# lnkloveating/MediQuery-RAG

Measured on AMD Instinct MI355X. Metric: queries/s (embed+top-k, k=5, b=256) over 1M×768 corpus; p50 single-query ms, higher is better.
Workload: dtype f32 (exact 3-way bf16 split, fp32 accumulate; exact fp32 top-k)

## Files before the change

### include/mq.h

```cpp
#ifndef MQ_H
#define MQ_H

#include <stdint.h>

#ifdef __cplusplus
extern "C" {
#endif

#define MQ_OK 0
#define MQ_EINVAL -1
#define MQ_ENOMEM -2
#define MQ_EHIP -3
#define MQ_EIO -4
#define MQ_ESTATE -5

#define MQ_DTYPE_F32 0
#define MQ_DTYPE_BF16 1
#define MQ_DTYPE_F32X6 2
#define MQ_DTYPE_F32_SCREEN 3

#define MQ_GELU_ERF 0
#define MQ_GELU_TANH 1
#define MQ_POOL_CLS 0
#define MQ_POOL_MEAN 1

#define MQ_MAX_K 64

typedef struct mq_index mq_index;
typedef struct mq_encoder mq_encoder;

const char* mq_last_error(void);
const char* mq_version(void);
const char* mq_build_source_hash(void);
int mq_device_count(void);

int mq_index_create(int device, int dim, int64_t capacity, int dtype, mq_index** out);
int mq_index_destroy(mq_index* ix);
int mq_index_size(const mq_index* ix, int64_t* n_rows);
int mq_index_dim(const mq_index* ix, int* dim);
int mq_index_add(mq_index* ix, const float* rows, int64_t n, int rows_on_device, void* stream);
int mq_index_reset(mq_index* ix);
int mq_index_search(mq_index* ix, const float* queries, int64_t nq, int k,
                    float* out_scores, int64_t* out_ids, int io_on_device, void* stream);
int mq_index_select(mq_index* src, const int64_t* rows, int64_t n, mq_index* dst);
int mq_index_get(mq_index* ix, int64_t row0, int64_t n, float* out, int out_on_device, void* stream);
int mq_index_set_precision(mq_index* ix, int dtype);
int mq_index_set_stream_threshold(mq_index* ix, int max_queries);
int mq_index_set_threshold_scan(mq_index* ix, int enabled);
int mq_index_set_int8_screen(mq_index* ix, int enabled);
int mq_index_set_async_screen(mq_index* ix, int enabled);
int mq_index_rescans(const mq_index* ix, int64_t* rescans, int64_t* remerges);
int mq_index_screen_fallbacks(const mq_index* ix, int64_t* to_direct, int64_t* to_split);
int mq_index_screen_skips(const mq_index* ix, int64_t* bf16_skips, int64_t* int8_skips);
int mq_index_data(mq_index* ix, void** device_rows);
int mq_index_set_timing(mq_index* ix, int enabled);
int mq_index_read_timing(mq_index* ix, float* ms, int n);
#define MQ_MASK_SET 0
#define MQ_MASK_AND 1
#define MQ_MASK_OR 2
#define MQ_MASK_CLEAR 3
int mq_mask_eval(const int32_t* codes, int64_t n, const uint8_t* lut, int n_lut, uint32_t* bits, int mode,
                 void* stream);
int mq_mask_eval_bits(const int32_t* codes, int64_t n, const uint64_t* lut_words, int n_lut, uint32_t* bits,
                      int mode, void* stream);
int mq_mask_combine(uint32_t* dst, const uint32_t* src, int64_t n_words, int mode, void* stream);
int mq_index_search_masked(mq_index* ix, const float* query, int k, const uint32_t* bits, float* out_scores,
                           int64_t* out_ids, int io_on_device, void* stream);
int mq_index_search_masked_batch(mq_index* ix, const float* queries, int64_t nq, int k, const uint32_t* bits,
                                 float* out_scores, int64_t* out_ids, int io_on_device, void* stream);
int mq_index_masked_gathers(const mq_index* ix, int64_t* count);
#define MQ_CONTAINS_MAX_BYTES 256
#define MQ_CONTAINS_SPAN_BYTES 16384
int mq_mask_contains(const uint8_t* text, int64_t text_bytes, const int64_t* offsets, int64_t n,
                     const uint8_t* pattern, int pattern_len, int negate, uint32_t* bits, int mode,
                     uint32_t* scratch, void* stream);

#define MQ_LEX_MAX_TERMS 128
#define MQ_LEX_NORM(fmul, fadd, c0, c1, dl) fadd((c0), fmul((c1), (dl)))
#define MQ_LEX_TERM(fmul, fadd, fdiv, w, tf, norm) fdiv(fmul((w), (tf)), fadd((tf), (norm)))
int64_t mq_lex_scratch_bytes(int64_t n, int k);
int mq_lex_df(const uint16_t* tokens, int64_t n_tokens, const int64_t* offsets, int64_t n, int ngram,
              const uint32_t* keys, int n_terms, int64_t* df, void* scratch, void* stream);
int mq_lex_topk(const uint16_t* tokens, int64_t n_tokens, const int64_t* offsets, int64_t n, int ngram,
                const uint32_t* keys, const float* w, int n_terms, float c0, float c1,
                const uint32_t* bits, int k, float* out_scores, int64_t* out_ids, int io_on_device,
                void* scratch, void* stream);

#define MQ_MMR_SCORE(fmul, fsub, lambda, s, red) \
  fsub(fmul((lambda), (s)), fmul(fsub(1.0f, (lambda)), (red)))
int mq_index_mmr_select(mq_index* ix, const float* cand_scores, const int64_t* cand_ids, int64_t nq,
                        int fetch_k, int k, float lambda, float* out_scores, int64_t* out_ids,
                        int io_on_device, void* stream);
int mq_index_search_mmr(mq_index* ix, const float* queries, int64_t nq, int k, int fetch_k,
                        float lambda, const uint32_t* bits, float* out_scores, int64_t* out_ids,
                        int io_on_device, void* stream);

int mq_index_save(mq_index* ix, const char* path);
int mq_index_load(mq_index* ix, const char* path);
int mq_index_save_rows(mq_index* ix, const char* path, int64_t row0, int64_t n);
int mq_index_load_append(mq_index* ix, const char* path);

int mq_topk_merge_host(const float* scores, const int64_t* ids, int n_lists, int64_t nq,
                       int k_in, int k_out, float* out_scores, int64_t* out_ids);
int mq_topk_merge_device(const float* scores, const int64_t* ids, int n_lists, int64_t nq,
                         int k_in, int k_out, float* out_scores, int64_t* out_ids, void* stream);

typedef struct mq_bert_config {
  int vocab_size;
  int hidden;
  int layers;
  int heads;
  int ffn;
  int max_positions;
  int type_vocab;
  float ln_eps;
  int gelu;
  int pooling;
} mq_bert_config;

int mq_encoder_create(int device, const mq_bert_config* cfg, mq_encoder** out);
int mq_encoder_destroy(mq_encoder* enc);
int64_t mq_encoder_weight_count(const mq_bert_config* cfg);
int mq_encoder_load_weights(mq_encoder* enc, const float* blob, int64_t n_floats);
int mq_encoder_set_precision(mq_encoder* enc, int dtype);
#define MQ_ENC_STAGES 8
int mq_encoder_set_graphs(mq_encoder* enc, int enabled);
#define MQ_ENC_OPT_ROWS_MAX 0
#define MQ_ENC_OPT_ROWS_SPLITS 1
#define MQ_ENC_OPT_SPLITK_MAX 2
#define MQ_ENC_OPT_FUSE_ATTN_OPROJ 4
#define MQ_ENC_OPT_SPLITK_TILES 6
#define MQ_ENC_OPT_RESIDENT_LAYERS 8
#define MQ_ENC_OPT_X6_PRESPLIT 9
#define MQ_ENC_OPT_ROWS_PLANES 10
#define MQ_ENC_OPT_LN_FOLD 11
#define MQ_ENC_OPT_CLS_KFREE 12
#define MQ_ENC_OPT_QKV_ATTN 13
#define MQ_ENC_OPT_EPI_SPLIT 14
int mq_encoder_set_option(mq_encoder* enc, int option, int value);
int mq_encoder_get_option(const mq_encoder* enc, int option, int* value);
int mq_encoder_set_timing(mq_encoder* enc, int enabled);
int mq_encoder_read_timing(mq_encoder* enc, float* ms, int n);
int mq_encoder_embed(mq_encoder* enc, const int32_t* ids, const int32_t* mask, int B, int L,
                     float* out, int io_on_device, void* stream);

#define MQ_HEAD_MAX_LABELS 8
int mq_encoder_load_head(mq_encoder* enc, const float* pooler_w, const float* pooler_b, const float* cls_w,
                         const float* cls_b, int n_labels);
int mq_encoder_score(mq_encoder* enc, const int32_t* ids, const int32_t* types, const int32_t* mask, int B,
                     int L, float* logits, int io_on_device, void* stream);

typedef struct mq_tokenizer mq_tokenizer;
int mq_tokenizer_create_wordpiece(const char* vocab_path, int lower_case, int max_length,
                                  mq_tokenizer** out);
int mq_tokenizer_create_wordpiece_tokens(const char* const* tokens, int n_tokens, int lower_case,
                                         int max_length, mq_tokenizer** out);
int mq_tokenizer_create_char(int vocab_size, int max_length, mq_tokenizer** out);
int mq_tokenizer_destroy(mq_tokenizer* tok);
int mq_tokenizer_encode_batch(mq_tokenizer* tok, const char* const* texts, int n, int pad_to,
                              int32_t* ids, int32_t* mask, int* out_len);

int mq_tokenizer_encode_pairs(mq_tokenizer* tok, const char* const* first, const char* const* second, int n,
                              int pad_to, int32_t* ids, int32_t* types, int32_t* mask, int* out_len);

int mq_debug_gemm_f32(const float* A, const float* W, const float* bias, const float* resid,
                      float* out, int M, int N, int K, int epi, int tile, void* stream);
int64_t mq_debug_w3_bytes(int N, int K);
int mq_debug_split_w3(const float* W, int N, int K, void* w3, void* stream);
int mq_debug_gemm_x6p(const float* A, const void* W3, const float* bias, const float* resid,
                      float* out, int M, int N, int K, int epi, int tile, void* stream);
int mq_debug_gemm_x6p_ln(const float* A, const void* W3, const float* bias, const float* resid,
                         float* out, int M, int N, int K, int epi, int tile, const float* stats_in,
                         float* stats_out, const float* g, const float* b, const float* s_fold,
                         float eps, void* stream);
int mq_debug_ln_fold_weight(const float* W, const float* bias, const float* g, const float* b, int N,
                            int K, float* Wg, float* s_out, float* c_out, void* stream);
int mq_debug_gemm_x6p_attn(const float* A, const void* W3, const float* bias, const int* mask,
                           float* ctx, int M, int K, int heads, float scale, int epi,
                           const float* stats_in, const float* s_fold, float eps, int max_workgroups,
                           void* stream);
int mq_debug_attention(const float* qkv, const int* mask, int B, int L, int H, int heads, float scale,
                       int variant, float* ctx, void* stream);
int mq_debug_cls_attention(const float* q, const float* x, const float* stats, const float* ln_g,
                           const float* ln_b, float eps, const int* mask, int B, int L, int H, int heads,
                           float scale, const float* Wk, const float* Wv, const float* bv, float* ctx,
                           void* stream);
int mq_debug_attn_oproj(const float* qkv, const int* mask, int B, int L, int H, int heads, float scale,
                        const float* Wo, const float* bo, const float* resid, int cls_only, int hg, int qf,
                        int acc, float* out, void* stream);
enum { MQ_ROWS_QKV = 0, MQ_ROWS_UP = 1, MQ_ROWS_OPROJ = 2, MQ_ROWS_DOWN = 3 };
int mq_debug_rows_gemm(int kind, int variant, const float* A, int lda, int64_t a_plane, int s_in, const float* W,
                       const float* bias, const float* resid, int ldr, float* out, int64_t o_plane, int M, int N,
                       int K, int splits, const float* ln_g, const float* ln_b, float eps, float* ln_out,
                       const int* ids, const int* types, int L, int vocab, const float* pos, const float* typ,
                       int type_vocab, int nt_w, float* zbuf, int64_t zn, void* stream);
int mq_debug_ln_pool(const float* hs, int planes, int64_t plane, const int* mask, int B, int L, int rows, int pooling,
                     const float* ln_g, const float* ln_b, float eps, int H, float* out, int raw, void* stream);

int mq_debug_cls_head(const float* cls, int B, int H, const float* pooler_w, const float* pooler_b,
                      const float* cls_w, const float* cls_b, int n_labels, float* logits, void* stream);

int mq_debug_int8_screen(mq_index* ix, const float* query, int kc, float* out_scores, int64_t* out_ids,
                         float* stats);

#ifdef __cplusplus
}
#endif
#endif
```

### mediquery-rag_amd/csrc/encoder.hip

```cpp
#include <algorithm>
#include <cmath>
#include <cstdlib>
#include <cstring>
#include <memory>
#include <vector>

#include "cls_head.hpp"
#include "common.hpp"
#include "gemm_epi.hpp"
#include "gemm_f32.hpp"
#include "gemm_x6p.hpp"

namespace mq {

__device__ __forceinline__ float wave_sum(float v) {
#pragma unroll
  for (int off = 32; off > 0; off >>= 1) v += __shfl_xor(v, off);
  return v;
}

template <class T, int EPI>
__global__ __launch_bounds__(T::THREADS, T::WG_PER_CU) void gemm_nt_kernel(const float* __restrict__ A, int lda,
                                                         const float* __restrict__ W,
                                                         const float* __restrict__ bias,
// ... 1297 lines not shown
  auto fetch = [&](int k0) {
    const int64_t row = row0 + min(k0 + lrow, L - 1);
#pragma unroll
    for (int j = 0; j < 4; ++j) xr[j] = *reinterpret_cast<const floatx4*>(x + row * H + (lc4 + TPR * j) * 4);
    if constexpr (FOLD) {
      const floatx4* sp = reinterpret_cast<const floatx4*>(stats + row * (2 * kLnMaxParts));
#pragma unroll
      for (int i = 0; i < kLnMaxParts / 2; ++i) sr[i] = sp[i];
    }
    mk = lane < CH && k0 + lane < L ? mask[row0 + k0 + lane] : 0;
  };
  float zacc[HEADS];
#pragma unroll
  for (int hh = 0; hh < HEADS; ++hh) zacc[hh] = 0.f;
  float m_run = -INFINITY, l_run = 0.f;
  fetch(0);
  for (int k0 = 0; k0 < L; k0 += CH) {
    if constexpr (FOLD) {
      float mu, rho;
      ln_merge(sr, eps, mu, rho);
#pragma unroll
      for (int j = 0; j < 4; ++j) xr[j] = (xr[j] - mu) * rho;
    }
#pragma unroll
    for (int j = 0; j < 4; ++j) *reinterpret_cast<floatx4*>(xs + lrow * H + (lc4 + TPR * j) * 4) = xr[j];
    const int live_key = mk;
    __syncthreads();
    if (k0 + CH < L) fetch(k0 + CH);
    float d[CH];
#pragma unroll
    for (int k = 0; k < CH; ++k) {
      float a = 0.f;
#pragma unroll
      for (int i = 0; i < VPL; ++i) {
        const floatx4 v = *reinterpret_cast<const floatx4*>(xs + k * H + (i * 64 + lane) * 4);
        a = fmaf(v.x, ur[i].x, fmaf(v.y, ur[i].y, fmaf(v.z, ur[i].z, fmaf(v.w, ur[i].w, a))));
      }
      d[k] = a;
    }
#pragma unroll
    for (int k = 0; k < CH; ++k) d[k] = wave_sum_fast(d[k]);
    float sc = -INFINITY;
#pragma unroll
    for (int k = 0; k < CH; ++k) sc = lane == k ? d[k] : sc;
    sc = live_key != 0 ? sc * scale : -INFINITY;
    float tmax = sc;
#pragma unroll
    for (int off = 8; off > 0; off >>= 1) tmax = fmaxf(tmax, __shfl_xor(tmax, off));
    tmax = __shfl(tmax, 0);
    const float m_new = fmaxf(m_run, tmax);
    const float alpha = m_new == -INFINITY ? 1.f : expf(m_run - m_new);
    const float p = sc == -INFINITY ? 0.f : expf(sc - m_new);
    float psum = p;
#pragma unroll
    for (int off = 8; off > 0; off >>= 1) psum += __shfl_xor(psum, off);
    psum = __shfl(psum, 0);
    l_run = l_run * alpha + psum;
    m_run = m_new;
    if (lane < CH) ps[lane * HEADS + h] = p;
    if (lane == 0) alpha_s[h] = alpha;
    __syncthreads();
#pragma unroll
    for (int q4 = 0; q4 < HEADS / 4; ++q4) {
      const floatx4 a = *reinterpret_cast<const floatx4*>(alpha_s + 4 * q4);
#pragma unroll
      for (int e = 0; e < 4; ++e) zacc[4 * q4 + e] *= a[e];
    }
#pragma unroll
    for (int k = 0; k < CH; ++k) {
      const float xv = xs[k * H + t];
#pragma unroll
      for (int q4 = 0; q4 < HEADS / 4; ++q4) {
        const floatx4 pp = *reinterpret_cast<const floatx4*>(ps + k * HEADS + 4 * q4);
#pragma unroll
        for (int e = 0; e < 4; ++e) zacc[4 * q4 + e] = fmaf(pp[e], xv, zacc[4 * q4 + e]);
      }
    }
    __syncthreads();
  }
  if (lane == 0) l_s[h] = l_run;
  __syncthreads();
#pragma unroll
  for (int hh = 0; hh < HEADS; ++hh) {
    const float l = l_s[hh];
    float v = l > 0.f ? zacc[hh] * (1.0f / l) : 0.f;
    if constexpr (FOLD) v = l > 0.f ? fmaf(v, g[t], be[t]) : 0.f;
    z[((int64_t)b * HEADS + hh) * H + t] = v;
  }
  if (t == 0) live[b] = l_s[0] > 0.f ? 1.f : 0.f;
}

}

using namespace mq;

namespace {

struct Buf {
  float* p = nullptr;
  size_t n = 0;
  int ensure(size_t need) {
    if (need <= n) return MQ_OK;
    if (p) (void)hipFree(p);
    p = nullptr;
    n = 0;
    if (hipMalloc((void**)&p, need * sizeof(float)) != hipSuccess)
      MQ_FAIL(MQ_ENOMEM, "hipMalloc(%zu floats) failed", need);
    n = need;
    return MQ_OK;
  }
  void release() {
    if (p) (void)hipFree(p);
    p = nullptr;
    n = 0;
  }
};

struct LayerW {
  const float *wqkv, *bqkv, *wo, *bo, *ln1g, *ln1b, *w1, *b1, *w2, *b2, *ln2g, *ln2b;
  const unsigned char *wqkv3 = nullptr, *wo3 = nullptr, *w13 = nullptr, *w23 = nullptr;
  const float *wqkvf = nullptr, *wof = nullptr, *w1f = nullptr, *w2f = nullptr;
  const unsigned char *w1g3 = nullptr, *wqkvg3 = nullptr;
  const float *w1gf = nullptr, *wqkvgf = nullptr;
  const float *w1s = nullptr, *w1c = nullptr, *wqkvs = nullptr, *wqkvc = nullptr;
};

int64_t weight_count(const mq_bert_config& c) {
  const int64_t H = c.hidden, F = c.ffn;
  const int64_t per_layer = 3 * H * H + 3 * H + H * H + H + 2 * H + F * H + F + H * F + H + 2 * H;
  return ((int64_t)c.vocab_size + c.max_positions + c.type_vocab) * H + 2 * H + c.layers * per_layer;
}

}


namespace {

struct GemmArgs {
  float* slab;
  size_t slab_floats;
  const float* A;
  int lda;
  const float* W;
  const float* bias;
  const float* resid;
  int ldr;
  float* out;
  int ldo;
  int M, N, K;
  int nt = 0;
  const void* W3 = nullptr;
  LnFold lf{};
  bool former_epi = false;
};

template <class T, int EPI>
void launch_gemm_t(const GemmArgs& g, int num_cus, hipStream_t s) {
  const int tiles = ((g.M + T::BM - 1) / T::BM) * ((g.N + T::BN - 1) / T::BN);
  const int grid = (std::min(tiles, T::WG_PER_CU * num_cus) + 7) / 8 * 8;
  const int tiles_m = (g.M + T::BM - 1) / T::BM, tiles_n = (g.N + T::BN - 1) / T::BN;
  const int rx = region_pick_rx(tiles_m, tiles_n, (double)T::BM * g.K * 4, (double)T::BN * g.K * 4, grid);
  hipLaunchKernelGGL((gemm_nt_kernel<T, EPI>), dim3(grid), dim3(T::THREADS), 0, s, g.A, g.lda, g.W,
                     g.bias, g.resid, g.ldr, g.out, g.ldo, g.M, g.N, g.K, rx, g.lf);
}

using GemmBig = F32Tile<2, 2, 2, 2>;
using GemmT96 = F32Tile<4, 1, 1, 3>;
using GemmMid = F32Tile<2, 2, 2, 1>;
using GemmSmall = F32Tile<1, 4, 1, 1>;

using X6Big = F32Tile<2, 2, 2, 2, true, 2, false, 0, false, true>;
using X6T96 = F32Tile<4, 1, 1, 3, true, 2, false, 0, false, true>;
using X6Mid = F32Tile<2, 2, 2, 1, true, 2, false, 0, false, true>;
using X6W192 = F32Tile<4, 2, 1, 3, true, 2, false, 0, false, true>;

template <int EPI>
void launch_gemm_tile(const GemmArgs& g, int tile, int num_cus, hipStream_t s) {
  switch (tile) {
    case 0: launch_gemm_t<GemmBig, EPI>(g, num_cus, s); return;
    case 1: launch_gemm_t<GemmT96, EPI>(g, num_cus, s); return;
    case 2: launch_gemm_t<GemmMid, EPI>(g, num_cus, s); return;
    case 5: launch_gemm_t<X6Big, EPI>(g, num_cus, s); return;
    case 6: launch_gemm_t<X6T96, EPI>(g, num_cus, s); return;
    case 7: launch_gemm_t<X6Mid, EPI>(g, num_cus, s); return;
    case 8: launch_gemm_t<F32Tile<4, 2, 1, 3>, EPI>(g, num_cus, s); return;
    case 9: launch_gemm_t<X6W192, EPI>(g, num_cus, s); return;
    default: launch_gemm_t<GemmSmall, EPI>(g, num_cus, s); return;
  }
}

int splitk_factor(const GemmArgs& g, int num_cus, int cap = 16, int tiles_max = 0) {
  if (!g.slab || g.N % 4 != 0) return 0;
  const int64_t tiles = (int64_t)((g.M + 31) / 32) * ((g.N + 127) / 128);
  const int64_t slots = 2 * (int64_t)num_cus;
  if (tiles > (tiles_max > 0 ? tiles_max : num_cus) || g.M > 256) return 0;
  const int slices = g.K / kBK;
  int best = 1;
  for (int s = 1; s <= slices && s <= cap; ++s)
    if (slices % s == 0 && tiles * s <= slots && (size_t)s * g.M * g.N <= g.slab_floats) best = s;
  return best >= 2 ? best : 0;
}

void launch_splitk_gemm(const GemmArgs& g, int S, hipStream_t s) {
  auto go = [&](auto tile) {
    using T = decltype(tile);
    const int tiles = ((g.M + T::BM - 1) / T::BM) * ((g.N + T::BN - 1) / T::BN);
    hipLaunchKernelGGL((gemm_splitk_kernel<T>), dim3(tiles * S), dim3(256), 0, s, g.A, g.lda, g.W, g.M, g.N, g.K,
                       S, g.slab);
  };
  if (g.nt)
    go(F32Tile<1, 4, 1, 1, false, 2, false, 0, true>{});
  else
    go(F32Tile<1, 4, 1, 1>{});
}

template <int EPI>
void launch_splitk(const GemmArgs& g, int S, hipStream_t s) {
  launch_splitk_gemm(g, S, s);
  const int64_t n4 = (int64_t)g.M * g.N / 4;
  hipLaunchKernelGGL((splitk_reduce_kernel<EPI>), dim3((unsigned)((n4 + 255) / 256)), dim3(256), 0,
                     s, g.slab, S, g.M, g.N, g.bias, g.resid, g.ldr, g.out, g.ldo);
}

int x6_tile_pick(const GemmArgs& g, int num_cus) {
  const int bns[3] = {128, 96, 64};
  const double effs[3] = {1.0, 0.96, 0.9};
  const int64_t slots = 2 * (int64_t)num_cus;
  int best = 0;
  double best_cost = 1e300;
  for (int i = 0; i < 3; ++i) {
    const int64_t tiles = (int64_t)((g.M + 127) / 128) * ((g.N + bns[i] - 1) / bns[i]);
    const double cost = (double)((tiles + slots - 1) / slots) * 128 * bns[i] / effs[i];
    if (cost < best_cost) {
      best_cost = cost;
      best = i;
    }
  }
  return best;
}

template <int EPI>
void launch_gemm_fold(const GemmArgs& g, int num_cus, hipStream_t s) {
  if (g.W3) {
    X6pArgs a{g.A, g.lda, g.W3, g.bias, g.resid, g.ldr, g.out, g.ldo, g.M, g.N, g.K};
    a.lf = g.lf;
    a.former_epi = g.former_epi;
    launch_gemm_x6p(a, EPI, -1, num_cus, s);
    return;
  }
  if constexpr (EPI == EPI_RESID_LN_STATS) {
    launch_gemm_t<X6T96, EPI>(g, num_cus, s);
  } else {
    switch (x6_tile_pick(g, num_cus)) {
      case 0: launch_gemm_t<X6Big, EPI>(g, num_cus, s); return;
      case 1: launch_gemm_t<X6T96, EPI>(g, num_cus, s); return;
      default: launch_gemm_t<X6Mid, EPI>(g, num_cus, s); return;
    }
  }
}

template <int EPI>
void launch_gemm(const GemmArgs& g, int num_cus, hipStream_t s, bool x6 = false, int splitk_cap = 16,
                 int splitk_tiles = 0) {
  const int S = splitk_factor(g, num_cus, splitk_cap, splitk_tiles);
  if (S) {
    launch_splitk<EPI>(g, S, s);
    return;
  }
  if (x6 && (int64_t)((g.M + 127) / 128) * ((g.N + 191) / 192) < num_cus) x6 = false;
  if (x6 && g.W3) {
    X6pArgs a{g.A, g.lda, g.W3, g.bias, g.resid, g.ldr, g.out, g.ldo, g.M, g.N, g.K};
    a.former_epi = g.former_epi;
    launch_gemm_x6p(a, EPI, -1, num_cus, s);
    return;
  }
  if (x6) {
    launch_gemm_tile<EPI>(g, 5 + x6_tile_pick(g, num_cus), num_cus, s);
    return;
  }
  struct Cand {
    int bm, bn;
    double eff;
  };
  const Cand cands[4] = {{128, 128, 1.0}, {128, 96, 0.96}, {128, 64, 0.9}, {32, 128, 0.55}};
  const int64_t slots = 2 * (int64_t)num_cus;
  int best = 0;
  double best_cost = 1e300;
  for (int i = 0; i < 4; ++i) {
    const int64_t tiles = (int64_t)((g.M + cands[i].bm - 1) / cands[i].bm) * ((g.N + cands[i].bn - 1) / cands[i].bn);
    const int64_t rounds = (tiles + slots - 1) / slots;
    const double cost = (double)rounds * cands[i].bm * cands[i].bn / cands[i].eff;
    if (cost < best_cost) {
      best_cost = cost;
      best = i;
    }
  }
  launch_gemm_tile<EPI>(g, best, num_cus, s);
}

#ifndef MQ_LN_FOLD_DEFAULT
#define MQ_LN_FOLD_DEFAULT 1
#endif
constexpr bool kLnFoldDefault = MQ_LN_FOLD_DEFAULT != 0;
#ifndef MQ_CLS_KFREE_DEFAULT
#define MQ_CLS_KFREE_DEFAULT 1
#endif
constexpr bool kClsKfreeDefault = MQ_CLS_KFREE_DEFAULT != 0;
#ifndef MQ_QKV_ATTN_DEFAULT
#define MQ_QKV_ATTN_DEFAULT 1
#endif
constexpr bool kQkvAttnDefault = MQ_QKV_ATTN_DEFAULT != 0;
#ifndef MQ_EPI_SPLIT_DEFAULT
#define MQ_EPI_SPLIT_DEFAULT 1
#endif
constexpr bool kEpiSplitDefault = MQ_EPI_SPLIT_DEFAULT != 0;

enum Stage { ST_EMBED = 0, ST_QKV, ST_ATTN, ST_OPROJ, ST_LN, ST_FFN_UP, ST_FFN_DOWN, ST_POOL, ST_N };


}

struct mq_encoder {
  int device = 0;
  PinBuf pin;
  mq_bert_config cfg{};
  int precision = MQ_DTYPE_F32;
  bool loaded = false;
  Buf weights;
  const float *word = nullptr, *pos = nullptr, *typ = nullptr, *eg = nullptr, *eb = nullptr;
  std::vector<LayerW> layers;
  Buf x, y, qkv, ctx, ffn, io_out, slab;
  Buf w3;
  Buf wfrag;
  int* io_ids = nullptr;
  int* io_mask = nullptr;
  size_t io_tokens = 0;
  Timeline tl;
  int num_cus = 256;
  struct Graph {
    int B = 0, L = 0, precision = 0;
    std::vector<const void*> bufs;
    hipGraphExec_t exec = nullptr;
    uint64_t last_use = 0;
  };
  std::vector<Graph> graphs;
  bool fuse_attn_oproj = true;
  int rows_max = kRowsDefault;
  int rows_splits = 0;
  int splitk_max = 16;
  int splitk_tiles = 0;
  int resident_layers = 8;
  bool x6_presplit = true;
  bool ln_fold = kLnFoldDefault;
  Buf lnst;
  Buf wfold3, wfoldf, sfold;
  bool rows_planes = false;
  bool cls_kfree = kClsKfreeDefault;
  bool qkv_attn = kQkvAttnDefault;
  bool epi_split = kEpiSplitDefault;
  Buf wkt;
  Buf cls;
  Buf head;
  int n_labels = 0;
  Buf cls_state;
  int* io_types = nullptr;
  size_t io_type_tokens = 0;
  bool use_graphs = false;
  uint64_t graph_clock = 0;
  hipStream_t cap_stream = nullptr;
  std::mutex mu;
};

namespace {

int build_w3(mq_encoder* e) {
  if (e->precision != MQ_DTYPE_F32X6 || !e->loaded || e->layers.empty() || e->layers[0].wqkv3) return MQ_OK;
  const mq_bert_config& c = e->cfg;
  const int H = c.hidden, F = c.ffn;
  const size_t per = w3_bytes(3 * H, H) + w3_bytes(H, H) + w3_bytes(F, H) + w3_bytes(H, F);
  DeviceGuard dg(e->device);
  int rc = e->w3.ensure((per * e->layers.size() + 3) / 4);
  if (rc) return rc;
  unsigned char* p = reinterpret_cast<unsigned char*>(e->w3.p);
  for (LayerW& w : e->layers) {
    auto one = [&](const float* W, int n, int k, const unsigned char*& dst) {
      launch_split_w3(W, n, k, p, nullptr);
      dst = p;
      p += w3_bytes(n, k);
    };
    one(w.wqkv, 3 * H, H, w.wqkv3);
    one(w.wo, H, H, w.wo3);
    one(w.w1, F, H, w.w13);
    one(w.w2, H, F, w.w23);
  }
  MQ_HIP(hipGetLastError());
  MQ_HIP(hipStreamSynchronize(nullptr));
  return MQ_OK;
}

int build_fold(mq_encoder* e) {
  const mq_bert_config& c = e->cfg;
  const int H = c.hidden, F = c.ffn;
  if (!e->ln_fold || e->precision != MQ_DTYPE_F32X6 || !e->loaded || e->layers.empty() ||
      H != kLnPartW * kLnMaxParts || F % 32 != 0)
    return MQ_OK;
  const bool img = e->x6_presplit;
  if (img ? e->layers[0].w1g3 != nullptr : e->layers[0].w1gf != nullptr) return MQ_OK;
  const size_t nl = e->layers.size();
  DeviceGuard dg(e->device);
  int rc = e->sfold.ensure(nl * 2 * ((size_t)F + 3 * H));
  if (rc) return rc;
  Buf tmp;
  if (img) {
    rc = e->wfold3.ensure((nl * w3_bytes(F, H) + (nl - 1) * w3_bytes(3 * H, H) + 3) / 4);
    if (!rc) rc = tmp.ensure((size_t)std::max(F, 3 * H) * H);
  } else {
    rc = e->wfoldf.ensure((nl * (size_t)F + (nl - 1) * (size_t)3 * H) * H);
  }
  if (rc) return rc;
  unsigned char* p3 = reinterpret_cast<unsigned char*>(e->wfold3.p);
  float* pf = e->wfoldf.p;
  float* ps = e->sfold.p;
  const LayerW* prev = nullptr;
  for (LayerW& w : e->layers) {
    auto one = [&](const float* W, const float* bias, const float* g, const float* b, int n, const unsigned char*& d3,
                   const float*& df, const float*& ds, const float*& dc) {
      float* wg = img ? tmp.p : pf;
      launch_ln_fold_weight(W, bias, g, b, n, H, wg, ps, ps + n, nullptr);
      ds = ps;
      dc = ps + n;
      ps += 2 * n;
      if (img) {
        launch_split_w3(wg, n, H, p3, nullptr);
        d3 = p3;
        p3 += w3_bytes(n, H);
      } else {
        df = pf;
        pf += (size_t)n * H;
      }
    };
    one(w.w1, w.b1, w.ln1g, w.ln1b, F, w.w1g3, w.w1gf, w.w1s, w.w1c);
    if (prev) one(w.wqkv, w.bqkv, prev->ln2g, prev->ln2b, 3 * H, w.wqkvg3, w.wqkvgf, w.wqkvs, w.wqkvc);
    prev = &w;
  }
  const hipError_t e1 = hipGetLastError(), e2 = hipStreamSynchronize(nullptr);
  tmp.release();
  MQ_HIP(e1);
  MQ_HIP(e2);
  return MQ_OK;
}

int build_frag16(mq_encoder* e) {
  const mq_bert_config& c = e->cfg;
  const int64_t H = c.hidden, F = c.ffn;
  const int64_t per = 3 * H * H + H * H + F * H + H * F;
  DeviceGuard dg(e->device);
  int rc = e->wfrag.ensure((size_t)(per * (int64_t)e->layers.size()));
  if (rc) return rc;
  float* p = e->wfrag.p;
  for (LayerW& w : e->layers) {
    auto one = [&](const float* W, int64_t r, int64_t k, const float*& dst) {
      const int64_t n4 = r * k / 4;
      hipLaunchKernelGGL(frag16_image_kernel, dim3((unsigned)((n4 + 255) / 256)), dim3(256), 0, nullptr, W, (int)r,
                         (int)k, reinterpret_cast<floatx4*>(p));
      dst = p;
      p += r * k;
    };
    one(w.wqkv, 3 * H, H, w.wqkvf);
    one(w.wo, H, H, w.wof);
    one(w.w1, F, H, w.w1f);
    one(w.w2, H, F, w.w2f);
  }
  MQ_HIP(hipGetLastError());
  MQ_HIP(hipStreamSynchronize(nullptr));
  return MQ_OK;
}

int build_wkt(mq_encoder* e) {
  const int H = e->cfg.hidden;
  if (e->cfg.pooling != MQ_POOL_CLS || e->layers.empty()) return MQ_OK;
  DeviceGuard dg(e->device);
  int rc = e->wkt.ensure((size_t)H * H);
  if (rc) return rc;
  hipLaunchKernelGGL(transpose_kernel, dim3(H / 32, H / 32), dim3(256), 0, nullptr,
                     e->layers.back().wqkv + (int64_t)H * H, H, H, e->wkt.p);
  MQ_HIP(hipGetLastError());
  MQ_HIP(hipStreamSynchronize(nullptr));
  return MQ_OK;
}

template <int EPI>
void gemm(mq_encoder* e, const GemmArgs& g, int stage, hipStream_t s) {
  e->tl.mark(s, stage);
  GemmArgs a = g;
  if (!e->x6_presplit) a.W3 = nullptr;
  a.former_epi = !e->epi_split;
  launch_gemm<EPI>(a, e->num_cus, s, e->precision == MQ_DTYPE_F32X6, e->splitk_max, e->splitk_tiles);
}

template <int VPL>
void gemm_resid_ln(mq_encoder* e, const GemmArgs& g, const float* lng, const float* lnb, float* x,
                   int stage, hipStream_t s) {
  const int H = VPL * 256;
  const int S = splitk_factor(g, e->num_cus, e->splitk_max, e->splitk_tiles);
  if (S && g.ldr == H && g.N == H) {
    e->tl.mark(s, stage);
    launch_splitk_gemm(g, S, s);
    e->tl.mark(s, ST_LN);
    hipLaunchKernelGGL((splitk_reduce_ln_kernel<VPL>), dim3((unsigned)g.M), dim3(256), 0, s, g.slab, S,
                       g.M, g.bias, g.resid, g.ldr, lng, lnb, e->cfg.ln_eps, x, 0);
    return;
  }
  gemm<EPI_RESID>(e, g, stage, s);
  e->tl.mark(s, ST_LN);
  constexpr int rows = 4 * kLnRowsPerWave;
  hipLaunchKernelGGL((ln_kernel<VPL, kLnRowsPerWave>), dim3((unsigned)((g.M + rows - 1) / rows)), dim3(256), 0, s,
                     g.out, g.M, lng, lnb, e->cfg.ln_eps, x);
}

struct ClsBufs {
  float *xc, *q, *u, *z, *part, *live;
  static size_t floats(int B, int H, int heads) {
    return (size_t)B * ((2 + kClsCtxSplits) * H + 2 * (size_t)heads * H + 1);
  }
  ClsBufs(float* p, int B, int H, int heads)
      : xc(p), q(xc + (size_t)B * H), u(q + (size_t)B * H), z(u + (size_t)B * heads * H),
        part(z + (size_t)B * heads * H), live(part + (size_t)kClsCtxSplits * B * H) {}
};

void launch_cls_u(int B, int H, int heads, const float* q, const float* wkt, float* u, hipStream_t s) {
  using T = F32Tile<1, 4, 1, 1>;
  const int tiles = ((B + T::BM - 1) / T::BM) * ((H + T::BN - 1) / T::BN);
  hipLaunchKernelGGL((gemm_heads_kernel<T>), dim3(tiles * heads), dim3(256), 0, s, q, H, kDh, wkt, H, kDh, nullptr,
                     nullptr, B, H, kDh, u, heads * H, H, 1, (int64_t)0);
}

void launch_cls_ctx(int B, int L, int H, int heads, float scale, const float* x, const float* stats,
                    const float* g, const float* be, float eps, const float* u, const int* mask, const float* wv,
                    const float* bv, float* z, float* part, float* live, float* ctx, hipStream_t s) {
  auto pass = [&](auto vpl) {
    constexpr int VPL = decltype(vpl)::value;
    if (stats)
      hipLaunchKernelGGL((cls_pass_kernel<VPL, true>), dim3(B), dim3(256 * VPL), 0, s, x, stats, g, be, eps, u, mask, L,
                         scale, z, live);
    else
      hipLaunchKernelGGL((cls_pass_kernel<VPL, false>), dim3(B), dim3(256 * VPL), 0, s, x, stats, g, be, eps, u, mask, L,
                         scale, z, live);
  };
  if (H == 256)
    pass(IC<1>{});
  else if (H == 512)
    pass(IC<2>{});
  else
    pass(IC<3>{});
  using T = F32Tile<2, 2, 1, 1>;
  const int tiles = (B + T::BM - 1) / T::BM;
  hipLaunchKernelGGL((gemm_heads_kernel<T>), dim3(tiles * heads * kClsCtxSplits), dim3(256), 0, s, z, heads * H, H, wv, H,
                     kDh * H, nullptr, nullptr, B, kDh, H, part, H, kDh, kClsCtxSplits, (int64_t)B * H);
  hipLaunchKernelGGL(cls_ctx_reduce_kernel, dim3((unsigned)(((int64_t)B * H / 4 + 255) / 256)), dim3(256), 0, s, part, B,
                     H, bv, live, ctx);
}

template <int VPL>
void gemm_resid_ln_pool(mq_encoder* e, const GemmArgs& g, const float* lng, const float* lnb, const int* mask,
                        float* out, int raw, int stage, hipStream_t s) {
  const int H = VPL * 256;
  const int S = splitk_factor(g, e->num_cus, e->splitk_max, e->splitk_tiles);
  if (S && g.ldr == H && g.N == H) {
    e->tl.mark(s, stage);
    launch_splitk_gemm(g, S, s);
    e->tl.mark(s, ST_POOL);
    hipLaunchKernelGGL((splitk_reduce_ln_kernel<VPL, true>), dim3((unsigned)g.M), dim3(256), 0, s, g.slab, S, g.M,
                       g.bias, g.resid, g.ldr, lng, lnb, e->cfg.ln_eps, out, raw);
    return;
  }
  gemm<EPI_RESID>(e, g, stage, s);
  e->tl.mark(s, ST_POOL);
  hipLaunchKernelGGL((ln_pool_kernel<VPL>), dim3((unsigned)((g.M + 3) / 4)), dim3(256), 0, s, g.out, 1, (int64_t)0, mask,
                     g.M, 1, 1, MQ_POOL_CLS, lng, lnb, e->cfg.ln_eps, out, raw);
}

template <int VPL>
int forward_vpl(mq_encoder* e, const int* ids, const int* types, const int* mask, int B, int L, float* out,
                int raw_cls, hipStream_t s) {
  const mq_bert_config& c = e->cfg;
  const int M = B * L, H = c.hidden, F = c.ffn;
  const unsigned row_blocks = (unsigned)((M + 3) / 4);
  const float scale = 1.0f / sqrtf((float)(H / c.heads));
  const int q_tiles = (L + 31) / 32;
  e->tl.mark(s, ST_EMBED);
  hipLaunchKernelGGL((embed_ln_kernel<VPL>), dim3(row_blocks), dim3(256), 0, s, ids, M, L,
                     c.vocab_size, e->word, e->pos, e->typ, types, c.type_vocab, e->eg, e->eb, c.ln_eps, e->x.p);
  const LayerW* prev = nullptr;
  const int nt = H / kLnPartW;
  const LayerW w0 = e->layers.empty() ? LayerW{} : e->layers[0];
  const bool fold = e->ln_fold && e->precision == MQ_DTYPE_F32X6 && M > 256 && H == kLnPartW * kLnMaxParts &&
                    F % 32 == 0 && (int64_t)((M + 127) / 128) * ((H + 191) / 192) >= e->num_cus &&
                    e->lnst.n >= (size_t)4 * M * nt && (e->x6_presplit ? w0.w1g3 != nullptr : w0.w1gf != nullptr);
  float* fst1 = e->lnst.p;
  float* fst2 = e->lnst.p + (size_t)2 * M * nt;
  bool raw = false;
  bool pooled = false;
  const bool attn_shape = e->qkv_attn && e->precision == MQ_DTYPE_F32X6 && L == 32 && H == 64 * c.heads &&
                          H % 192 == 0 && H % 32 == 0 && M > 256 &&
                          (int64_t)((M + 127) / 128) * ((3 * H + 191) / 192) >= e->num_cus &&
                          x6p_pick_tile(M, 3 * H, e->num_cus) == 0 && (int64_t)M * H < (1ll << 29);
  const bool qkv_attn = attn_shape && e->x6_presplit;
  auto fold_gemm = [&](auto epi, GemmArgs g, int stage) {
    e->tl.mark(s, stage);
    if (!e->x6_presplit) g.W3 = nullptr;
    g.former_epi = !e->epi_split;
    g.lf.eps = c.ln_eps;
    launch_gemm_fold<decltype(epi)::value>(g, e->num_cus, s);
  };
  for (size_t li = 0; li < e->layers.size(); ++li) {
    const LayerW& w = e->layers[li];
    const bool cls_only = c.pooling == MQ_POOL_CLS && li + 1 == e->layers.size();
    const int rows = cls_only ? B : M;
    int stride = cls_only ? L * H : H;
    const float* resid = e->x.p;
    int ldr = stride;
    const bool kfree = cls_only && L > 1 && e->cls_kfree && VPL <= 3 && e->wkt.p != nullptr &&
                       e->cls.n >= ClsBufs::floats(B, H, c.heads);
    const int lnt = M <= 256 && (int)li >= e->resident_layers ? 1 : 0;
    const bool fold_layer = fold && !(cls_only && L > 1);
    bool attn_done = false;
    bool attn_after = false;
    auto qkv_fold = [&](GemmArgs g, int row0) {
      g.W = w.wqkvgf ? w.wqkvgf + (int64_t)row0 * H : nullptr;
      g.W3 = w.wqkvg3 ? w.wqkvg3 + w3_row_offset(row0, H) : nullptr;
      g.bias = w.wqkvc + row0;
      g.lf.s = w.wqkvs + row0;
      g.lf.stats_in = fst2;
      fold_gemm(IC<EPI_BIAS_LNFOLD>{}, g, ST_QKV);
    };
    auto qkv_gemm = [&](GemmArgs g) {
      g.nt = lnt;
      if (raw)
        qkv_fold(g, (int)(g.W - w.wqkv) / H);
      else
        gemm<EPI_BIAS>(e, g, ST_QKV, s);
    };
    if (kfree) {
      const ClsBufs cb(e->cls.p, B, H, c.heads);
      const float* xin = e->x.p;
      const float* xst = raw ? fst2 : nullptr;
      if (xst) {
        e->tl.mark(s, ST_LN);
        hipLaunchKernelGGL((ln_rows_kernel<VPL>), dim3((unsigned)((B + 3) / 4)), dim3(256), 0, s, xin, B, (int64_t)L * H,
                           prev->ln2g, prev->ln2b, c.ln_eps, cb.xc);
        resid = cb.xc;
        ldr = H;
      }
      GemmArgs q{e->slab.p, e->slab.n, resid, ldr, w.wqkv, w.bqkv, nullptr, 0, cb.q, H, B, H, H, lnt};
      q.W3 = w.wqkv3;
      gemm<EPI_BIAS>(e, q, ST_QKV, s);
      launch_cls_u(B, H, c.heads, cb.q, e->wkt.p, cb.u, s);
      e->tl.mark(s, ST_ATTN);
      launch_cls_ctx(B, L, H, c.heads, scale, xin, xst, xst ? prev->ln2g : nullptr, xst ? prev->ln2b : nullptr,
                     c.ln_eps, cb.u, mask, w.wqkv + (int64_t)2 * H * H, w.bqkv + 2 * H, cb.z, cb.part, cb.live, e->ctx.p, s);
      stride = H;
    } else if (cls_only && L > 1) {
      GemmArgs kv{e->slab.p, e->slab.n, e->x.p, H, w.wqkv + (int64_t)H * H, w.bqkv + H, nullptr, 0, e->qkv.p + H,
                  3 * H, M, 2 * H, H};
      if (w.wqkv3) kv.W3 = w.wqkv3 + w3_row_offset(H, H);
      qkv_gemm(kv);
      if (raw) {
        e->tl.mark(s, ST_LN);
        hipLaunchKernelGGL((ln_rows_inplace_kernel<VPL>), dim3((unsigned)((B + 3) / 4)), dim3(256), 0, s, e->x.p, B,
                           (int64_t)L * H, prev->ln2g, prev->ln2b, c.ln_eps);
      }
      GemmArgs q{e->slab.p, e->slab.n, e->x.p, L * H, w.wqkv, w.bqkv, nullptr, 0, e->qkv.p, L * 3 * H, B, H, H, lnt};
      q.W3 = w.wqkv3;
      gemm<EPI_BIAS>(e, q, ST_QKV, s);
    } else if (qkv_attn && (raw ? w.wqkvg3 != nullptr : w.wqkv3 != nullptr)) {
      X6pArgs a{e->x.p, H, raw ? w.wqkvg3 : w.wqkv3, raw ? w.wqkvc : w.bqkv, nullptr, 0, e->ctx.p, H, M, 3 * H, H};
      if (raw) {
        a.lf.s = w.wqkvs;
        a.lf.stats_in = fst2;
        a.lf.eps = c.ln_eps;
      }
      a.at.mask = mask;
      a.at.scale = scale;
      e->tl.mark(s, ST_QKV);
      launch_gemm_x6p(a, raw ? EPI_ATTN_LNFOLD : EPI_ATTN_BIAS, 0, e->num_cus, s);
      attn_done = true;
    } else {
      GemmArgs qkv{e->slab.p, e->slab.n, e->x.p, H, w.wqkv, w.bqkv, nullptr, 0, e->qkv.p, 3 * H, M, 3 * H, H};
      qkv.W3 = w.wqkv3;
      qkv_gemm(qkv);
      attn_after = attn_shape;
    }
    const bool resid_raw = raw && fold_layer;
    raw = false;
    if (!kfree && !attn_done) {
      e->tl.mark(s, ST_ATTN);
      const int qt = cls_only ? 1 : q_tiles;
      if (attn_after)
        launch_attn32(e->qkv.p, mask, e->ctx.p, M, H, scale, s);
      else
        launch_attention(B, L, c.heads, qt, H, scale, e->qkv.p, mask, e->ctx.p, s);
    }
    GemmArgs oproj{e->slab.p, e->slab.n, e->ctx.p, stride, w.wo, w.bo, resid, ldr, e->y.p, H, rows, H, H, lnt};
    oproj.W3 = w.wo3;
    if (fold_layer) {
      oproj.lf.stats_out = fst1;
      if (resid_raw) {
        oproj.lf.stats_in = fst2;
        oproj.lf.g = prev->ln2g;
        oproj.lf.b = prev->ln2b;
      }
      fold_gemm(IC<EPI_RESID_LN_STATS>{}, oproj, ST_OPROJ);
    } else {
      gemm_resid_ln<VPL>(e, oproj, w.ln1g, w.ln1b, e->x.p, ST_OPROJ, s);
    }
    GemmArgs up{e->slab.p, e->slab.n, e->x.p, H, w.w1, w.b1, nullptr, 0, e->ffn.p, F, rows, F, H, lnt};
    up.W3 = w.w13;
    if (fold_layer) {
      up.A = e->y.p;
      up.W = w.w1gf;
      up.W3 = w.w1g3;
      up.bias = w.w1c;
      up.lf.s = w.w1s;
      up.lf.stats_in = fst1;
      if (c.gelu == MQ_GELU_TANH)
        fold_gemm(IC<EPI_GELU_TANH_LNFOLD>{}, up, ST_FFN_UP);
      else
        fold_gemm(IC<EPI_GELU_ERF_LNFOLD>{}, up, ST_FFN_UP);
    } else if (c.gelu == MQ_GELU_TANH) {
      gemm<EPI_GELU_TANH>(e, up, ST_FFN_UP, s);
    } else {
      gemm<EPI_GELU_ERF>(e, up, ST_FFN_UP, s);
    }
    GemmArgs down{e->slab.p, e->slab.n, e->ffn.p, F, w.w2, w.b2, e->x.p, H, e->y.p, H, rows, H, F, lnt};
    down.W3 = w.w23;
    if (fold_layer) {
      const bool last = li + 1 == e->layers.size();
      down.resid = e->y.p;
      down.lf.stats_in = fst1;
      down.lf.g = w.ln1g;
      down.lf.b = w.ln1b;
      down.lf.stats_out = fst2;
      down.out = last ? e->ctx.p : e->x.p;
      fold_gemm(IC<EPI_RESID_LN_STATS>{}, down, ST_FFN_DOWN);
      if (last) {
        e->tl.mark(s, ST_LN);
        constexpr int wg_rows = 4 * kLnRowsPerWave;
        hipLaunchKernelGGL((ln_kernel<VPL, kLnRowsPerWave>), dim3((unsigned)((M + wg_rows - 1) / wg_rows)), dim3(256),
                           0, s, e->ctx.p, M, w.ln2g, w.ln2b, c.ln_eps, e->x.p);
      } else {
        raw = true;
      }
    } else if (kfree) {
      gemm_resid_ln_pool<VPL>(e, down, w.ln2g, w.ln2b, mask, out, raw_cls, ST_FFN_DOWN, s);
      pooled = true;
    } else {
      gemm_resid_ln<VPL>(e, down, w.ln2g, w.ln2b, e->x.p, ST_FFN_DOWN, s);
    }
    prev = &w;
  }
  if (!pooled) {
    e->tl.mark(s, ST_POOL);
    const bool pruned = c.pooling == MQ_POOL_CLS;
    hipLaunchKernelGGL((pool_kernel<VPL>), dim3((B + 3) / 4), dim3(256), 0, s, e->x.p, mask, B,
                       pruned ? 1 : L, c.pooling, out, raw_cls);
  }
  e->tl.close(s);
  MQ_HIP(hipGetLastError());
  return MQ_OK;
}

struct RowsArgs {
  const float* A;
  int lda;
  int64_t a_plane;
  const float* W;
  int ldw;
  const float* bias;
  const float* resid;
  int ldr;
  float* out;
  int ldo;
  int64_t o_plane;
  int M, N, K;
  int splits;
  const int* ids = nullptr;
  int L = 1, vocab = 0;
  const float* pos = nullptr;
  const float* typ = nullptr;
  const int* types = nullptr;
  int type_vocab = 1;
  int nt_w = 0;
  float* zbuf = nullptr;
  int64_t zn = 0;
};

template <int EPI, bool LN_IN, int VPL, int NB, int S_IN, int RT, int FL>
void launch_rows_rt(const RowsArgs& g, const float* lng, const float* lnb, float eps, float* ln_out,
                    hipStream_t s) {
  hipLaunchKernelGGL((rows_gemm_kernel<EPI, LN_IN, VPL, NB, S_IN, RT, FL>),
                     dim3(g.N / kRT, (g.M + kRT * RT - 1) / (kRT * RT), g.splits), dim3(64 * kRWaves), 0, s,
                     g.A, g.lda, g.a_plane, g.M, lng, lnb, eps, ln_out, g.W, g.ldw, g.bias, g.resid, g.ldr,
                     g.out, g.ldo, g.o_plane, g.ids, g.L, g.vocab, g.pos, g.typ, g.types, g.type_vocab, g.nt_w, g.zbuf,
                     g.zn);
}

template <int EPI, bool LN_IN, int VPL, int NB, int S_IN, int FL = 0>
void launch_rows_nb(const RowsArgs& g, const float* lng, const float* lnb, float eps, float* ln_out,
                    hipStream_t s) {
  constexpr bool two_fit = LN_IN && (size_t)(2 * kRT * (NB * 256 + 4) + kRWaves * 2 * kRT * kRT) * 4 <= 160 * 1024;
  if constexpr (two_fit) {
    if (g.M > kRT) {
      launch_rows_rt<EPI, LN_IN, VPL, NB, S_IN, 2, FL>(g, lng, lnb, eps, ln_out, s);
      return;
    }
  }
  launch_rows_rt<EPI, LN_IN, VPL, NB, S_IN, 1, FL>(g, lng, lnb, eps, ln_out, s);
}

bool rows_nb_ok(int nb) { return nb >= 1 && (nb <= 4 || nb == 6 || nb == 8 || nb == 12 || nb == 16); }

int rows_splits(int K, int forced = 0) {
  const int nb = K / 256;
  if (forced >= 1 && forced <= 4 && nb % forced == 0 && rows_nb_ok(nb / forced)) return forced;
  for (int sp = 1; sp <= 4; ++sp)
    if (nb % sp == 0 && nb / sp <= 6 && rows_nb_ok(nb / sp)) return sp;
  return 1;
}

template <int EPI, int NB, int FL>
void launch_rows_plain(const RowsArgs& g, hipStream_t s) {
  launch_rows_nb<EPI, false, 1, NB, 1, FL>(g, nullptr, nullptr, 0.f, nullptr, s);
}

template <int EPI, int FL = 0>
void launch_rows(const RowsArgs& g, hipStream_t s) {
// ... 568 lines not shown
    g.zbuf = zn ? zbuf : nullptr;
    g.zn = zn;
    if (ln_kind && s_in == 0) {
      g.ids = ids;
      g.L = L;
      g.vocab = vocab;
      g.pos = pos;
      g.typ = typ;
      g.types = types;
      g.type_vocab = type_vocab;
    }
    if (ln_kind) {
      switch (K) {
        case 256: debug_rows_ln<1>(kind, variant, g, s_in, ln_g, ln_b, eps, ln_out, s); break;
        case 512: debug_rows_ln<2>(kind, variant, g, s_in, ln_g, ln_b, eps, ln_out, s); break;
        case 768: debug_rows_ln<3>(kind, variant, g, s_in, ln_g, ln_b, eps, ln_out, s); break;
        default: debug_rows_ln<4>(kind, variant, g, s_in, ln_g, ln_b, eps, ln_out, s); break;
      }
    } else if (kind == MQ_ROWS_OPROJ) {
      launch_rows<EPI_RESID>(g, s);
    } else if (acc) {
      launch_rows<EPI_RESID, FL_A | FL_ACC>(g, s);
    } else {
      launch_rows<EPI_RESID, FL_A>(g, s);
    }
    err = hipGetLastError();
  }
  const hipError_t serr = hipStreamSynchronize(s);
  (void)hipFree(wimg);
  if (err == hipSuccess) err = serr;
  if (err != hipSuccess) MQ_FAIL(MQ_EHIP, "few-row GEMM failed: %s", hipGetErrorString(err));
  return MQ_OK;
}

int mq_debug_ln_pool(const float* hs, int planes, int64_t plane, const int* mask, int B, int L, int rows, int pooling,
                     const float* ln_g, const float* ln_b, float eps, int H, float* out, int raw, void* stream) {
  clear_error();
  MQ_CHECK_ARG(hs && ln_g && ln_b && out, "NULL buffer");
  MQ_CHECK_ARG(H == 256 || H == 512 || H == 768 || H == 1024, "hidden must be 256/512/768/1024 (got %d)", H);
  MQ_CHECK_ARG(B >= 1 && L >= 1, "bad shape B=%d L=%d", B, L);
  MQ_CHECK_ARG(planes >= 1 && planes <= 4, "planes must be in [1, 4] (got %d)", planes);
  MQ_CHECK_ARG(planes == 1 || (plane > 0 && plane % 4 == 0), "plane must be a positive multiple of 4 (got %lld)",
               (long long)plane);
  MQ_CHECK_ARG(pooling == MQ_POOL_CLS || pooling == MQ_POOL_MEAN, "bad pooling %d", pooling);
  MQ_CHECK_ARG(rows == L || (rows == 1 && pooling == MQ_POOL_CLS),
               "rows per sequence must be L, or 1 with CLS pooling (rows %d, L %d)", rows, L);
  MQ_CHECK_ARG(pooling == MQ_POOL_CLS || mask, "mean pooling needs the mask");
  MQ_CHECK_ARG(raw == 0 || raw == 1, "raw must be 0 or 1 (got %d)", raw);
  MQ_CHECK_ARG(aligned16(hs) && aligned16(ln_g) && aligned16(ln_b) && aligned16(out), "buffers must be 16-byte aligned");
  hipStream_t s = (hipStream_t)stream;
  const dim3 grid((unsigned)((B + 3) / 4));
  auto go = [&](auto kern) {
    hipLaunchKernelGGL(kern, grid, dim3(256), 0, s, hs, planes, plane, mask, B, L, rows, pooling, ln_g, ln_b, eps, out,
                       raw);
  };
  switch (H) {
    case 256: go(ln_pool_kernel<1>); break;
    case 512: go(ln_pool_kernel<2>); break;
    case 768: go(ln_pool_kernel<3>); break;
    default: go(ln_pool_kernel<4>); break;
  }
  MQ_HIP(hipGetLastError());
  return MQ_OK;
}

int mq_debug_cls_attention(const float* q, const float* x, const float* stats, const float* ln_g,
                           const float* ln_b, float eps, const int* mask, int B, int L, int H, int heads,
                           float scale, const float* Wk, const float* Wv, const float* bv, float* ctx,
                           void* stream) {
  clear_error();
  MQ_CHECK_ARG(q && x && mask && Wk && Wv && bv && ctx, "NULL buffer");
  MQ_CHECK_ARG(B > 0 && L > 0 && heads > 0 && H == heads * kDh, "bad shape B=%d L=%d H=%d heads=%d", B, L, H, heads);
  MQ_CHECK_ARG(H == 256 || H == 512 || H == 768, "hidden must be 256 / 512 / 768 (got %d)", H);
  MQ_CHECK_ARG(!stats || (ln_g && ln_b && H == kLnPartW * kLnMaxParts), "stats need ln_g, ln_b and H = %d",
               kLnPartW * kLnMaxParts);
  hipStream_t s = (hipStream_t)stream;
  float* scratch = nullptr;
  const size_t wkt_floats = (size_t)H * H;
  if (hipMalloc((void**)&scratch, (wkt_floats + ClsBufs::floats(B, H, heads)) * 4) != hipSuccess)
    MQ_FAIL(MQ_ENOMEM, "scratch allocation failed");
  const ClsBufs cb(scratch + wkt_floats, B, H, heads);
  hipLaunchKernelGGL(transpose_kernel, dim3(H / 32, H / 32), dim3(256), 0, s, Wk, H, H, scratch);
  launch_cls_u(B, H, heads, q, scratch, cb.u, s);
  launch_cls_ctx(B, L, H, heads, scale, x, stats, ln_g, ln_b, eps, cb.u, mask, Wv, bv, cb.z, cb.part, cb.live, ctx, s);
  hipError_t err = hipGetLastError();
  const hipError_t serr = hipStreamSynchronize(s);
  (void)hipFree(scratch);
  if (err == hipSuccess) err = serr;
  if (err != hipSuccess) MQ_FAIL(MQ_EHIP, "CLS attention failed: %s", hipGetErrorString(err));
  return MQ_OK;
}

int mq_encoder_set_graphs(mq_encoder* e, int enabled) {
  clear_error();
  MQ_CHECK_ARG(e, "NULL encoder");
  std::lock_guard<std::mutex> lk(e->mu);
  e->use_graphs = enabled != 0;
  return MQ_OK;
}

int mq_encoder_set_option(mq_encoder* e, int option, int value) {
  clear_error();
  MQ_CHECK_ARG(e, "NULL encoder");
  std::lock_guard<std::mutex> lk(e->mu);
  switch (option) {
    case MQ_ENC_OPT_ROWS_MAX:
      MQ_CHECK_ARG(value >= 0 && value <= kRowsMax, "rows_max must be in [0, %d] (got %d)", kRowsMax, value);
      e->rows_max = value;
      break;
    case MQ_ENC_OPT_ROWS_SPLITS:
      MQ_CHECK_ARG(value >= 0 && value <= 4, "rows_splits must be in [0, 4] (got %d)", value);
      e->rows_splits = value;
      break;
    case MQ_ENC_OPT_SPLITK_MAX:
      MQ_CHECK_ARG(value >= 2 && value <= 64, "splitk_max must be in [2, 64] (got %d)", value);
      e->splitk_max = value;
      break;
    case MQ_ENC_OPT_FUSE_ATTN_OPROJ:
      MQ_CHECK_ARG(value == 0 || value == 1, "fuse_attn_oproj must be 0 or 1 (got %d)", value);
      e->fuse_attn_oproj = value != 0;
      break;
    case MQ_ENC_OPT_RESIDENT_LAYERS:
      MQ_CHECK_ARG(value >= 0 && value <= 1024, "resident_layers must be in [0, 1024] (got %d)", value);
      e->resident_layers = value;
      break;
    case MQ_ENC_OPT_SPLITK_TILES:
      MQ_CHECK_ARG(value >= 0 && value <= 4096, "splitk_tiles must be in [0, 4096] (got %d)", value);
      e->splitk_tiles = value;
      break;
    case MQ_ENC_OPT_X6_PRESPLIT:
      MQ_CHECK_ARG(value == 0 || value == 1, "x6_presplit must be 0 or 1 (got %d)", value);
      e->x6_presplit = value != 0;
      break;
    case MQ_ENC_OPT_ROWS_PLANES:
      MQ_CHECK_ARG(value == 0 || value == 1, "rows_planes must be 0 or 1 (got %d)", value);
      e->rows_planes = value != 0;
      break;
    case MQ_ENC_OPT_LN_FOLD:
      MQ_CHECK_ARG(value == 0 || value == 1, "ln_fold must be 0 or 1 (got %d)", value);
      e->ln_fold = value != 0;
      break;
    case MQ_ENC_OPT_CLS_KFREE:
      MQ_CHECK_ARG(value == 0 || value == 1, "cls_kfree must be 0 or 1 (got %d)", value);
      e->cls_kfree = value != 0;
      break;
    case MQ_ENC_OPT_QKV_ATTN:
      MQ_CHECK_ARG(value == 0 || value == 1, "qkv_attn must be 0 or 1 (got %d)", value);
      e->qkv_attn = value != 0;
      break;
    case MQ_ENC_OPT_EPI_SPLIT:
      MQ_CHECK_ARG(value == 0 || value == 1, "epi_split must be 0 or 1 (got %d)", value);
      e->epi_split = value != 0;
      break;
    default:
      MQ_FAIL(MQ_EINVAL, "unknown encoder option %d", option);
  }
  for (auto& g : e->graphs) (void)hipGraphExecDestroy(g.exec);
  e->graphs.clear();
  return MQ_OK;
}

int mq_encoder_get_option(const mq_encoder* e, int option, int* value) {
  clear_error();
  MQ_CHECK_ARG(e && value, "NULL argument");
  switch (option) {
    case MQ_ENC_OPT_ROWS_MAX: *value = e->rows_max; break;
    case MQ_ENC_OPT_ROWS_SPLITS: *value = e->rows_splits; break;
    case MQ_ENC_OPT_SPLITK_MAX: *value = e->splitk_max; break;
    case MQ_ENC_OPT_FUSE_ATTN_OPROJ: *value = e->fuse_attn_oproj ? 1 : 0; break;
    case MQ_ENC_OPT_RESIDENT_LAYERS: *value = e->resident_layers; break;
    case MQ_ENC_OPT_SPLITK_TILES: *value = e->splitk_tiles; break;
    case MQ_ENC_OPT_X6_PRESPLIT: *value = e->x6_presplit ? 1 : 0; break;
    case MQ_ENC_OPT_ROWS_PLANES: *value = e->rows_planes ? 1 : 0; break;
    case MQ_ENC_OPT_LN_FOLD: *value = e->ln_fold ? 1 : 0; break;
    case MQ_ENC_OPT_CLS_KFREE: *value = e->cls_kfree ? 1 : 0; break;
    case MQ_ENC_OPT_QKV_ATTN: *value = e->qkv_attn ? 1 : 0; break;
    case MQ_ENC_OPT_EPI_SPLIT: *value = e->epi_split ? 1 : 0; break;
    default: MQ_FAIL(MQ_EINVAL, "unknown encoder option %d", option);
  }
  return MQ_OK;
}

int mq_encoder_set_timing(mq_encoder* e, int enabled) {
  clear_error();
  MQ_CHECK_ARG(e, "NULL encoder");
  std::lock_guard<std::mutex> lk(e->mu);
  DeviceGuard dg(e->device);
  e->tl.drain();
  e->tl.on = enabled != 0;
  return MQ_OK;
}

int mq_encoder_read_timing(mq_encoder* e, float* ms, int n) {
  clear_error();
  MQ_CHECK_ARG(e && ms && n >= 0, "bad argument");
  std::lock_guard<std::mutex> lk(e->mu);
  DeviceGuard dg(e->device);
  e->tl.read(ms, n);
  return MQ_OK;
}

}

namespace {

int ensure_forward_bufs(mq_encoder* e, int B, int L) {
  const mq_bert_config& c = e->cfg;
  const size_t M = (size_t)B * L;
  if (e->tl.used > 4096) e->tl.drain();
  int rc = MQ_OK;
  rc = e->slab.ensure((size_t)2 * e->num_cus * 32 * 128);
  if (rc) return rc;
  rc = build_fold(e);
  if (rc) return rc;
  const size_t ln_parts = e->ln_fold && M > 256 ? (size_t)4 * M * std::max(1, c.hidden / kLnPartW) : 0;
  const size_t cls_floats = e->cls_kfree && c.pooling == MQ_POOL_CLS && L > 1 ? ClsBufs::floats(B, c.hidden, c.heads) : 0;
  for (auto bn : {std::make_pair(&e->x, M * c.hidden), std::make_pair(&e->y, (M <= (size_t)kRowsMax ? 4 : 1) * M * c.hidden),
                  std::make_pair(&e->ctx, M * c.hidden), std::make_pair(&e->qkv, M * 3 * c.hidden),
                  std::make_pair(&e->ffn, (M + 15) / 16 * 16 * c.ffn), std::make_pair(&e->lnst, ln_parts),
                  std::make_pair(&e->cls, cls_floats)}) {
    rc = bn.first->ensure(bn.second);
    if (rc) return rc;
  }
  return MQ_OK;
}

int ensure_io(mq_encoder* e, size_t M, int B) {
  if (e->io_tokens < M) {
    if (e->io_ids) (void)hipFree(e->io_ids);
    if (e->io_mask) (void)hipFree(e->io_mask);
    e->io_ids = e->io_mask = nullptr;
    e->io_tokens = 0;
    if (hipMalloc((void**)&e->io_ids, M * 4) != hipSuccess ||
        hipMalloc((void**)&e->io_mask, M * 4) != hipSuccess)
      MQ_FAIL(MQ_ENOMEM, "hipMalloc(io) failed");
    e->io_tokens = M;
  }
  return e->io_out.ensure((size_t)B * e->cfg.hidden);
}

}

extern "C" {

int mq_encoder_embed(mq_encoder* e, const int32_t* ids, const int32_t* mask, int B, int L,
                     float* out, int io_on_device, void* stream) {
  clear_error();
  MQ_CHECK_ARG(e, "NULL encoder");
  MQ_CHECK_ARG(B >= 0 && L >= 1, "bad shape B=%d L=%d", B, L);
  MQ_CHECK_ARG(L <= e->cfg.max_positions, "L=%d exceeds max_positions %d", L, e->cfg.max_positions);
  if (B == 0) return MQ_OK;
  MQ_CHECK_ARG(ids && mask && out, "NULL buffer");
  MQ_CHECK_ARG((int64_t)B * L < (1ll << 31) / 4096, "batch too large");
  if (!e->loaded) MQ_FAIL(MQ_ESTATE, "encoder weights not loaded");
  std::lock_guard<std::mutex> lk(e->mu);
  DeviceGuard dg(e->device);
  hipStream_t s = (hipStream_t)stream;
  const mq_bert_config& c = e->cfg;
  const size_t M = (size_t)B * L;
  int rc = ensure_forward_bufs(e, B, L);
  if (rc) return rc;
  const bool graph = e->use_graphs && !e->tl.on;
  const int* dids = ids;
  const int* dmask = mask;
  float* dout = out;
  if (!io_on_device || graph) {
    rc = ensure_io(e, M, B);
    if (rc) return rc;
    const hipMemcpyKind kind = io_on_device ? hipMemcpyDeviceToDevice : hipMemcpyHostToDevice;
    if (!io_on_device && M * 8 + (size_t)B * c.hidden * 4 <= (1u << 20)) {
      rc = e->pin.ensure(M * 8 + (size_t)B * c.hidden * 4);
      if (rc) return rc;
      memcpy(e->pin.as<unsigned char>(), ids, M * 4);
      memcpy(e->pin.as<unsigned char>() + M * 4, mask, M * 4);
      MQ_HIP(hipMemcpyAsync(e->io_ids, e->pin.p, M * 4, kind, s));
      MQ_HIP(hipMemcpyAsync(e->io_mask, e->pin.as<unsigned char>() + M * 4, M * 4, kind, s));
    } else {
      MQ_HIP(hipMemcpyAsync(e->io_ids, ids, M * 4, kind, s));
      MQ_HIP(hipMemcpyAsync(e->io_mask, mask, M * 4, kind, s));
    }
    dids = e->io_ids;
    dmask = e->io_mask;
    dout = e->io_out.p;
  }
  if (graph) {
    rc = launch_graph(e, B, L, s);
  } else {
    rc = forward(e, dids, nullptr, dmask, B, L, dout, 0, s);
  }
  if (rc) return rc;
  if (io_on_device && dout != out)
    MQ_HIP(hipMemcpyAsync(out, dout, (size_t)B * c.hidden * 4, hipMemcpyDeviceToDevice, s));
  if (!io_on_device) {
    const size_t ob = (size_t)B * c.hidden * 4;
    if (M * 8 + ob <= (1u << 20)) {
      unsigned char* hp = e->pin.as<unsigned char>() + M * 8;
      MQ_HIP(hipMemcpyAsync(hp, dout, ob, hipMemcpyDeviceToHost, s));
      MQ_HIP(hipStreamSynchronize(s));
      memcpy(out, hp, ob);
    } else {
      MQ_HIP(hipMemcpyAsync(out, dout, ob, hipMemcpyDeviceToHost, s));
      MQ_HIP(hipStreamSynchronize(s));
    }
  }
  return MQ_OK;
}

int mq_encoder_load_head(mq_encoder* e, const float* pooler_w, const float* pooler_b, const float* cls_w,
                         const float* cls_b, int n_labels) {
  clear_error();
  MQ_CHECK_ARG(n_labels >= 1 && n_labels <= MQ_HEAD_MAX_LABELS, "n_labels must be in [1, %d] (got %d)",
               MQ_HEAD_MAX_LABELS, n_labels);
  MQ_CHECK_ARG(e, "NULL encoder");
  MQ_CHECK_ARG(pooler_w && pooler_b && cls_w && cls_b, "NULL argument");
  if (!e->loaded) MQ_FAIL(MQ_ESTATE, "encoder weights not loaded");
  std::lock_guard<std::mutex> lk(e->mu);
  DeviceGuard dg(e->device);
  const size_t H = (size_t)e->cfg.hidden;
  e->n_labels = 0;
  const int rc = e->head.ensure(H * H + H + (size_t)MQ_HEAD_MAX_LABELS * (H + 1));
  if (rc) return rc;
  float* p = e->head.p;
  MQ_HIP(hipMemcpy(p, pooler_w, H * H * 4, hipMemcpyHostToDevice));
  MQ_HIP(hipMemcpy(p + H * H, pooler_b, H * 4, hipMemcpyHostToDevice));
  MQ_HIP(hipMemcpy(p + H * H + H, cls_w, (size_t)n_labels * H * 4, hipMemcpyHostToDevice));
  MQ_HIP(hipMemcpy(p + H * H + H + (size_t)MQ_HEAD_MAX_LABELS * H, cls_b, (size_t)n_labels * 4, hipMemcpyHostToDevice));
  e->n_labels = n_labels;
  return MQ_OK;
}

// ... 79 lines not shown
```

### mediquery-rag_amd/csrc/gemm_epi.hpp

```cpp
#pragma once

#include "gemm_f32.hpp"
#include "gemm_x6p.hpp"

namespace mq {

enum Epi {
  EPI_BIAS = 0,
  EPI_GELU_ERF = 1,
  EPI_GELU_TANH = 2,
  EPI_RESID = 3,
  EPI_RESID_LN_STATS = 5,
  EPI_BIAS_LNFOLD = 6,
  EPI_GELU_ERF_LNFOLD = 7,
  EPI_GELU_TANH_LNFOLD = 8,
  EPI_ATTN_BIAS = 9,
  EPI_ATTN_LNFOLD = 10
};
constexpr bool epi_is_lnfold(int epi) { return epi >= EPI_BIAS_LNFOLD && epi <= EPI_GELU_TANH_LNFOLD; }
constexpr bool epi_is_attn(int epi) { return epi == EPI_ATTN_BIAS || epi == EPI_ATTN_LNFOLD; }

__device__ __forceinline__ float gelu_erf(float x) {
  const float z = fabsf(x) * 0.70710678118654752f;
  const float t = __builtin_amdgcn_rcpf(fmaf(0.5f, z, 1.0f));
// ... 126 lines not shown
                                                           const LnFold& lf, const unsigned char* tl = nullptr) {
  static_assert(NB * 16 == kLnPartW && MB <= 4, "partials are per kLnPartW-column wave tile");
  static_assert(!HAND || ER == 1, "the hand-off form finishes a row at a time");
  const int c = lane & 15, g = lane >> 4;
  const bool ln_r = lf.stats_in != nullptr;
  float own_mu = 0.f, own_rho = 1.0f;
  if constexpr (!HAND) {
    if (ln_r) ln_row_own<MB>(lf.stats_in, wr0, M, lf.eps, lane, own_mu, own_rho);
  }
  float gv[NB];
#pragma unroll
  for (int n = 0; n < NB; ++n) {
    const int col = wc0 + n * 16 + c;
    const float bb = bias[col] + (ln_r ? lf.b[col] : 0.f);
    gv[n] = ln_r ? lf.g[col] : 1.0f;
#pragma unroll
    for (int m = 0; m < MB; ++m)
#pragma unroll
      for (int e = 0; e < 4; ++e) acc[m][n][e] += bb;
  }
  const __amdgpu_buffer_rsrc_t rr =
      __builtin_amdgcn_make_buffer_rsrc((void*)(resid + wc0), (short)0, 0x7fffffff, 0x00020000);
  const __amdgpu_buffer_rsrc_t ro =
      __builtin_amdgcn_make_buffer_rsrc((void*)(out + wc0), (short)0, 0x7fffffff, 0x00020000);
  const __amdgpu_buffer_rsrc_t rs = __builtin_amdgcn_make_buffer_rsrc(
      (void*)(lf.stats_out + 2 * (wc0 / kLnPartW)), (short)0, 0x7fffffff, 0x00020000);
#pragma unroll
  for (int m = 0; m < MB; ++m) {
    floatx4 tv[NB];
    if constexpr (HAND) {
#pragma unroll
      for (int n = 0; n < NB; ++n)
        tv[n] = *reinterpret_cast<const floatx4*>(tl + (m * NB + n) * 1024 + ln_t_slot(lane));
    }
#pragma unroll
    for (int eh = 0; eh < 4; eh += ER) {
      float v[ER][NB];
      if constexpr (!HAND) {
#pragma unroll
        for (int e2 = 0; e2 < ER; ++e2) {
          const int lo = (min(wr0 + m * 16 + 4 * g + eh + e2, M - 1) * ldr + c) * 4;
#pragma unroll
          for (int n = 0; n < NB; ++n)
            v[e2][n] = __uint_as_float(__builtin_amdgcn_raw_buffer_load_b32(rr, lo, n * 64, 0));
        }
      }
#pragma unroll
      for (int e2 = 0; e2 < ER; ++e2) {
        const int e = eh + e2, row = wr0 + m * 16 + 4 * g + e;
        float mu = 0.f, rho = 1.0f;
        if constexpr (!HAND) {
          mu = ln_row_bcast(own_mu, lane, m, e);
          rho = ln_row_bcast(own_rho, lane, m, e);
        }
        const int so = (row * ldo + c) * 4;
        float sum = 0.f;
#pragma unroll
        for (int n = 0; n < NB; ++n) {
          if constexpr (HAND)
            v[e2][n] = __fmaf_rn(tv[n][e], gv[n], acc[m][n][e]);
          else
            v[e2][n] = __fmaf_rn((v[e2][n] - mu) * rho, gv[n], acc[m][n][e]);
          sum += v[e2][n];
          if (row < M) __builtin_amdgcn_raw_buffer_store_b32(__float_as_uint(v[e2][n]), ro, so, n * 64, 0);
        }
        const float mean = row16_sum(sum) * (1.0f / (float)kLnPartW);
        float m2 = 0.f;
#pragma unroll
        for (int n = 0; n < NB; ++n) {
          const float d = v[e2][n] - mean;
          m2 = __fmaf_rn(d, d, m2);
        }
        m2 = row16_sum(m2);
        if (c == 0 && row < M) {
          uint2v_t pr;
          pr.x = __float_as_uint(mean);
          pr.y = __float_as_uint(m2);
          __builtin_amdgcn_raw_buffer_store_b64(pr, rs, row * (kLnMaxParts * 8), 0, 0);
        }
      }
    }
  }
}

template <int MB, int NB>
struct LnTileRegs {
  floatx4 r[MB][NB];
  floatx4 p[kLnMaxParts / 2];
};
template <int Q>
__device__ __forceinline__ float quad_bcast(float v) {
  return __int_as_float(__builtin_amdgcn_update_dpp(0, __float_as_int(v), Q * 0x55, 0xF, 0xF, false));
}
template <int MB, int NB>
__device__ __forceinline__ void ln_tile_load(LnTileRegs<MB, NB>& q, const float* __restrict__ resid, int ldr,
                                             int wr0, int wc0, int M, const LnFold& lf, int lane) {
  const __amdgpu_buffer_rsrc_t rr =
      __builtin_amdgcn_make_buffer_rsrc((void*)(resid + wc0), (short)0, 0x7fffffff, 0x00020000);
#pragma unroll
  for (int m = 0; m < MB; ++m) {
    const int row = min(wr0 + m * 16 + (lane >> 2), M - 1);
    const int lo = (row * ldr + 4 * (lane & 3)) * 4;
#pragma unroll
    for (int n = 0; n < NB; ++n)
      q.r[m][n] = __builtin_bit_cast(floatx4, __builtin_amdgcn_raw_buffer_load_b128(rr, lo, n * 64, 0));
  }
  if (lf.stats_in != nullptr) {
    const int row = min(wr0 + (lane & 3) * 16 + (lane >> 2), M - 1);
    const floatx4* src = reinterpret_cast<const floatx4*>(lf.stats_in + (int64_t)row * (2 * kLnMaxParts));
#pragma unroll
    for (int i = 0; i < kLnMaxParts / 2; ++i) q.p[i] = src[i];
  }
}
template <int MB, int NB>
__device__ __forceinline__ void ln_tile_write(const LnTileRegs<MB, NB>& q, unsigned char* tl, const LnFold& lf,
                                              int lane) {
  static_assert(MB == 4, "a quad's lanes share out the block rows");
  const int g = lane >> 4, e = (lane >> 2) & 3;
  unsigned off[4];
#pragma unroll
  for (int i = 0; i < 4; ++i) off[i] = (unsigned)(256 * g + 16 * ((4 * (lane & 3) + i) ^ g) + 4 * e);
  float own_mu = 0.f, own_rho = 1.0f;
  if (lf.stats_in != nullptr) ln_merge(q.p, lf.eps, own_mu, own_rho);
  const float mus[4] = {quad_bcast<0>(own_mu), quad_bcast<1>(own_mu), quad_bcast<2>(own_mu), quad_bcast<3>(own_mu)};
  const float rhos[4] = {quad_bcast<0>(own_rho), quad_bcast<1>(own_rho), quad_bcast<2>(own_rho),
                         quad_bcast<3>(own_rho)};
#pragma unroll
  for (int m = 0; m < MB; ++m) {
    const float mu = mus[m], rho = rhos[m];
#pragma unroll
    for (int n = 0; n < NB; ++n)
#pragma unroll
      for (int i = 0; i < 4; ++i)
        *reinterpret_cast<float*>(tl + (m * NB + n) * 1024 + off[i]) = (q.r[m][n][i] - mu) * rho;
  }
}

template <int NB>
struct EpiPre {
  float bv[NB], sv[NB];
  float own_mu = 0.f, own_rho = 0.f;
};
template <int EPI, int MB, int NB>
__device__ __forceinline__ void epi_pre_load(EpiPre<NB>& p, int wr0, int wc0, int M, int N,
                                             const float* __restrict__ bias, const LnFold& lf, int lane) {
#pragma unroll
  for (int n = 0; n < NB; ++n) {
    const int col = min(wc0 + n * 16 + (lane & 15), N - 1);
    p.bv[n] = bias[col];
    p.sv[n] = epi_is_lnfold(EPI) ? lf.s[col] : 0.f;
  }
  if constexpr (epi_is_lnfold(EPI)) ln_row_own<MB>(lf.stats_in, wr0, M, lf.eps, lane, p.own_mu, p.own_rho);
}
template <int EPI, int MB, int NB, int M_LO = 0, int M_HI = MB, bool PRE = false>
__device__ __forceinline__ void store_wave_tile16(floatx4 (&acc)[MB][NB], int wr0, int wc0, int M, int N,
                                                  const float* __restrict__ bias, const float* __restrict__ resid,
                                                  int ldr, float* __restrict__ out, int ldo, int lane,
                                                  const LnFold& lf = LnFold{}, const EpiPre<NB>* pre = nullptr) {
  static_assert(!PRE || (EPI != EPI_RESID && EPI != EPI_RESID_LN_STATS), "preloads: the kinds without a residual");
  static_assert(0 <= M_LO && M_LO < M_HI && M_HI <= MB, "block-row range");
  static_assert(EPI != EPI_RESID_LN_STATS || (M_LO == 0 && M_HI == MB), "the producer finishes whole wave tiles");
  const int c = lane & 15, g = lane >> 4;
  if constexpr (EPI == EPI_RESID_LN_STATS) {
    store_wave_tile16_ln_stats<1>(acc, wr0, wc0, M, bias, resid, ldr, out, ldo, lane, lf);
    return;
  }
  constexpr bool FOLD = epi_is_lnfold(EPI);
  static_assert(!FOLD || MB <= 4, "one lane of a 16-lane row group per row of the wave tile");
  float own_mu = 0.f, own_rho = 0.f;
  if constexpr (PRE) {
    own_mu = pre->own_mu;
    own_rho = pre->own_rho;
  } else if constexpr (FOLD) {
    ln_row_own<MB>(lf.stats_in, wr0, M, lf.eps, lane, own_mu, own_rho);
  }
  if (wr0 + MB * 16 <= M && wc0 + NB * 16 <= N) {
    float bv[NB], sv[NB];
#pragma unroll
    for (int n = 0; n < NB; ++n) {
      if constexpr (PRE)
        bv[n] = pre->bv[n];
      else
        bv[n] = bias[wc0 + n * 16 + c];
    }
    if constexpr (FOLD) {
#pragma unroll
      for (int n = 0; n < NB; ++n) {
        if constexpr (PRE)
          sv[n] = pre->sv[n];
        else
          sv[n] = lf.s[wc0 + n * 16 + c];
      }
    }
    const __amdgpu_buffer_rsrc_t rr = __builtin_amdgcn_make_buffer_rsrc(
        (void*)(resid + (EPI == EPI_RESID ? (int64_t)wr0 * ldr + wc0 : 0)), (short)0, 0x7fffffff, 0x00020000);
    const int rl = (4 * g * ldr + c) * 4;
    const __amdgpu_buffer_rsrc_t ro = __builtin_amdgcn_make_buffer_rsrc(
        (void*)(out + (int64_t)wr0 * ldo + wc0), (short)0, 0x7fffffff, 0x00020000);
    const int ol = (4 * g * ldo + c) * 4;
#pragma unroll
    for (int m = M_LO; m < M_HI; ++m) {
      float rv[NB][4];
      if constexpr (EPI == EPI_RESID) {
#pragma unroll
        for (int n = 0; n < NB; ++n)
#pragma unroll
          for (int e = 0; e < 4; ++e)
            rv[n][e] = __uint_as_float(
                __builtin_amdgcn_raw_buffer_load_b32(rr, rl, ((m * 16 + e) * ldr + n * 16) * 4, 0));
      }
      if constexpr (FOLD) {
#pragma unroll
        for (int e = 0; e < 4; ++e) {
          const float mu = ln_row_bcast(own_mu, lane, m, e), rho = ln_row_bcast(own_rho, lane, m, e);
#pragma unroll
          for (int n = 0; n < NB; ++n) {
            const float v = epi_apply<EPI>(__fmaf_rn(rho, __fmaf_rn(-mu, sv[n], acc[m][n][e]), bv[n]));
            __builtin_amdgcn_raw_buffer_store_b32(__float_as_uint(v), ro, ol, ((m * 16 + e) * ldo + n * 16) * 4, 0);
          }
        }
      } else {
#pragma unroll
        for (int n = 0; n < NB; ++n)
#pragma unroll
          for (int e = 0; e < 4; ++e) {
            float v = epi_apply<EPI>(acc[m][n][e] + bv[n]);
            if constexpr (EPI == EPI_RESID) v += rv[n][e];
            __builtin_amdgcn_raw_buffer_store_b32(__float_as_uint(v), ro, ol, ((m * 16 + e) * ldo + n * 16) * 4, 0);
          }
      }
    }
    return;
  }
  if constexpr (FOLD) {
#pragma unroll
    for (int m = M_LO; m < M_HI; ++m) {
      float mu[4], rho[4];
#pragma unroll
      for (int e = 0; e < 4; ++e) {
        mu[e] = ln_row_bcast(own_mu, lane, m, e);
        rho[e] = ln_row_bcast(own_rho, lane, m, e);
      }
#pragma unroll
      for (int n = 0; n < NB; ++n) {
        const int col = wc0 + n * 16 + c;
        if (col < N) {
          float b, sn;
          if constexpr (PRE) {
            b = pre->bv[n];
            sn = pre->sv[n];
          } else {
            b = bias[col];
            sn = lf.s[col];
          }
#pragma unroll
          for (int e = 0; e < 4; ++e) {
            const int row = wr0 + m * 16 + 4 * g + e;
            if (row < M)
              out[(int64_t)row * ldo + col] = epi_apply<EPI>(__fmaf_rn(rho[e], __fmaf_rn(-mu[e], sn, acc[m][n][e]), b));
          }
        }
      }
    }
    return;
  }
#pragma unroll
  for (int n = 0; n < NB; ++n) {
    const int col = wc0 + n * 16 + c;
    if (col >= N) continue;
    float b;
    if constexpr (PRE)
      b = pre->bv[n];
    else
      b = bias[col];
#pragma unroll
    for (int m = M_LO; m < M_HI; ++m)
#pragma unroll
      for (int e = 0; e < 4; ++e) {
        const int row = wr0 + m * 16 + 4 * g + e;
        if (row >= M) continue;
        float v = epi_apply<EPI>(acc[m][n][e] + b);
        if constexpr (EPI == EPI_RESID) v += resid[(int64_t)row * ldr + col];
        out[(int64_t)row * ldo + col] = v;
      }
  }
}

constexpr int kAttnSt = 36;
constexpr int kAttnStage = 64 * kAttnSt * 4;
template <bool FOLD, bool PRE = false>
__device__ __forceinline__ void attn_wave_tile(floatx4 (&acc)[4][6], int wr0, int head, int wn, int M, int H,
                                               const float* __restrict__ bias, const LnFold& lf,
                                               const int* __restrict__ mask, float scale,
                                               float* __restrict__ ctx, int lane, unsigned char* stg,
                                               const unsigned char* partner) {
  static_assert(kAttnStage >= 8 * 1024, "the partials of two sequences fit the staging");
  const int c = lane & 15, g = lane >> 4;
  const unsigned long long kbits = __ballot(mask[min(wr0 + lane, M - 1)] != 0);
  float own_mu = 0.f, own_rho = 0.f;
  if constexpr (FOLD) ln_row_own<4>(lf.stats_in, wr0, M, lf.eps, lane, own_mu, own_rho);
  if constexpr (PRE) {
#pragma unroll
    for (int m = 0; m < 4; ++m)
#pragma unroll
      for (int n = 0; n < 2; ++n)
#pragma unroll
        for (int e = 0; e < 4; ++e) acc[m][n][e] = acc[m][n][e] * scale;
  } else {
    float bv[6], sv[6];
#pragma unroll
    for (int n = 0; n < 6; ++n) {
      const int col = (n >> 1) * H + 64 * head + 32 * wn + 16 * (n & 1) + c;
      bv[n] = bias[col];
      if constexpr (FOLD) sv[n] = lf.s[col];
    }
#pragma unroll
    for (int m = 0; m < 4; ++m)
#pragma unroll
      for (int e = 0; e < 4; ++e) {
        float mu = 0.f, rho = 0.f;
        if constexpr (FOLD) {
          mu = ln_row_bcast(own_mu, lane, m, e);
          rho = ln_row_bcast(own_rho, lane, m, e);
        }
#pragma unroll
        for (int n = 0; n < 6; ++n) {
          float v;
          if constexpr (FOLD)
            v = __fmaf_rn(rho, __fmaf_rn(-mu, sv[n], acc[m][n][e]), bv[n]);
          else
            v = acc[m][n][e] + bv[n];
          acc[m][n][e] = n < 2 ? v * scale : v;
        }
      }
  }
  float* sf = reinterpret_cast<float*>(stg);
  floatx4 sp[2][2][2];
#pragma unroll
  for (int s = 0; s < 2; ++s) {
#pragma unroll
    for (int t = 0; t < 2; ++t)
#pragma unroll
      for (int mb = 0; mb < 2; ++mb)
#pragma unroll
        for (int nd = 0; nd < 2; ++nd)
#pragma unroll
          for (int e = 0; e < 4; ++e)
            sf[(32 * t + 16 * mb + 4 * g + e) * kAttnSt + 16 * nd + c] = acc[2 * s + mb][2 * t + nd][e];
    floatx4 qf[2][2], kf[2][2];
#pragma unroll
    for (int blk = 0; blk < 2; ++blk)
#pragma unroll
      for (int hf = 0; hf < 2; ++hf) {
        qf[blk][hf] = *reinterpret_cast<const floatx4*>(&sf[(16 * blk + c) * kAttnSt + 16 * hf + 4 * g]);
        kf[blk][hf] = *reinterpret_cast<const floatx4*>(&sf[(32 + 16 * blk + c) * kAttnSt + 16 * hf + 4 * g]);
      }
#pragma unroll
    for (int kb = 0; kb < 2; ++kb)
#pragma unroll
      for (int qb = 0; qb < 2; ++qb) {
        floatx4 st = {0.f, 0.f, 0.f, 0.f};
#pragma unroll
        for (int i = 0; i < 8; ++i)
          st = __builtin_amdgcn_mfma_f32_16x16x4f32(kf[kb][i >> 2][i & 3], qf[qb][i >> 2][i & 3], st, 0, 0, 0);
        sp[s][kb][qb] = st;
      }
  }
#pragma unroll
  for (int i = 0; i < 8; ++i)
    *reinterpret_cast<floatx4*>(stg + i * 1024 + lane * 16) = sp[i >> 2][(i >> 1) & 1][i & 1];
  asm volatile("s_waitcnt lgkmcnt(0)\n\ts_barrier" ::: "memory");
#pragma unroll
  for (int i = 0; i < 8; ++i)
    sp[i >> 2][(i >> 1) & 1][i & 1] += *reinterpret_cast<const floatx4*>(partner + i * 1024 + lane * 16);
#pragma unroll
  for (int s = 0; s < 2; ++s) {
    const unsigned kb32 = (unsigned)(kbits >> (32 * s));
    float inv[2];
#pragma unroll
    for (int qb = 0; qb < 2; ++qb) {
      float mx = -INFINITY;
#pragma unroll
      for (int kb = 0; kb < 2; ++kb)
#pragma unroll
        for (int e = 0; e < 4; ++e) {
          const bool live = (kb32 >> (16 * kb + 4 * g + e)) & 1u;
          sp[s][kb][qb][e] = live ? sp[s][kb][qb][e] : -INFINITY;
          mx = fmaxf(mx, sp[s][kb][qb][e]);
        }
      mx = fmaxf(mx, __shfl_xor(mx, 16));
      mx = fmaxf(mx, __shfl_xor(mx, 32));
      float l = 0.f;
#pragma unroll
      for (int kb = 0; kb < 2; ++kb)
#pragma unroll
        for (int e = 0; e < 4; ++e) {
          const float v = sp[s][kb][qb][e];
          const float p = v == -INFINITY ? 0.f : expf(v - mx);
          sp[s][kb][qb][e] = p;
          l += p;
        }
      l += __shfl_xor(l, 16);
      l += __shfl_xor(l, 32);
      inv[qb] = l > 0.f ? 1.0f / l : 0.f;
    }
#pragma unroll
    for (int qb = 0; qb < 2; ++qb) {
      floatx4 o[2] = {{0.f, 0.f, 0.f, 0.f}, {0.f, 0.f, 0.f, 0.f}};
#pragma unroll
      for (int kb = 0; kb < 2; ++kb)
#pragma unroll
        for (int e = 0; e < 4; ++e)
#pragma unroll
          for (int nd = 0; nd < 2; ++nd)
            o[nd] = __builtin_amdgcn_mfma_f32_16x16x4f32(sp[s][kb][qb][e], acc[2 * s + kb][4 + nd][e], o[nd], 0, 0, 0);
#pragma unroll
      for (int e = 0; e < 4; ++e) {
        const float iq = __shfl(inv[qb], 4 * g + e);
        const int row = wr0 + 32 * s + 16 * qb + 4 * g + e;
        if (row < M) {
          float* dst = ctx + (int64_t)row * H + 64 * head + 32 * wn + c;
          dst[0] = o[0][e] * iq;
          dst[16] = o[1][e] * iq;
        }
      }
    }
  }
}

}
```

### mediquery-rag_amd/csrc/gemm_x6p.hip

```cpp
#include <algorithm>

#include "gemm_epi.hpp"
#include "gemm_x6p.hpp"

namespace mq {
namespace {

typedef __attribute__((address_space(3))) void x6p_lds_t;

__device__ __forceinline__ void x6p_glds(const void* base, unsigned voff, unsigned lds_dst) {
  const uint64_t b64 = (uint64_t)(uintptr_t)base;
  base = (const void*)(uintptr_t)(((uint64_t)__builtin_amdgcn_readfirstlane((unsigned)(b64 >> 32)) << 32) |
                                  (unsigned)__builtin_amdgcn_readfirstlane((unsigned)b64));
  unsigned keep;
  asm volatile("s_mov_b32 %0, m0\n\ts_mov_b32 m0, %3\n\ts_nop 0\n\tglobal_load_lds_dwordx4 %1, %2\n\ts_mov_b32 m0, %0"
               : "=&s"(keep)
               : "v"(voff), "s"(base), "s"(__builtin_amdgcn_readfirstlane(lds_dst))
               : "memory");
}

__device__ __forceinline__ int a_swz(int q) { return q ^ (q >> 1); }

typedef __bf16 bf16x2_t __attribute__((ext_vector_type(2)));
typedef float float2_t __attribute__((ext_vector_type(2)));
__device__ __forceinline__ unsigned cvt_pk_bf16(float lo, float hi) {
  float2_t v;
  v.x = lo;
  v.y = hi;
  return __builtin_bit_cast(unsigned, __builtin_convertvector(v, bf16x2_t));
}
__device__ __forceinline__ void split3v(floatx4 x, uint2 (&pl)[3]) {
#pragma unroll
  for (int p = 0; p < 3; ++p) {
    const unsigned a = cvt_pk_bf16(x.x, x.y), b = cvt_pk_bf16(x.z, x.w);
    pl[p] = make_uint2(a, b);
    if (p < 2) {
      x.x -= bf16_lo(a);
      x.y -= bf16_hi(a);
      x.z -= bf16_lo(b);
      x.w -= bf16_hi(b);
    }
  }
}

#if defined(MQ_X6P_DBG) && !defined(MQ_MEASUREMENT_BUILD)
#error "MQ_X6P_DBG computes wrong results: only a measurement build (-DMQ_MEASUREMENT_BUILD) may set it"
#endif

template <int WAVES_M_, int WAVES_N_, int TM_, int TN_, int NBUF_, int KS_ = 1, int DMAW_ = 8, bool SCHED_ = false,
          int DBG_ = 0, int DSTEP_ = 1, int BR0_ = 0, int PS_ = 4, bool LDR_ = false, bool M16_ = false,
          bool DEEP_ = false>
struct X6pTile {
  static constexpr int WAVES_M = WAVES_M_, WAVES_N = WAVES_N_, TM = TM_, TN = TN_, NBUF = NBUF_;
  static constexpr int KS = KS_;
  static constexpr int DMAW = DMAW_;
  static constexpr bool SCHED = SCHED_;
  static constexpr int DSTEP = DSTEP_, BR0 = BR0_, PS = PS_;
  static constexpr int DBG = DBG_;
  static constexpr bool LDR = LDR_;
  static constexpr bool M16 = M16_, DEEP = DEEP_;
  static constexpr int NW = WAVES_M * WAVES_N, THREADS = (LDR ? 2 * NW : NW) * 64;
  static constexpr int WM = TM * 32, WN = TN * 32, BM = WAVES_M * WM, BN = WAVES_N * WN;
  static constexpr int A_SUB = BM * 64;
  static constexpr int B_SUB = BN * 96;
  static constexpr int STAGE = KS * (A_SUB + B_SUB);
  static constexpr int NA = BM / 16, NB = BN / 32 * 3;
  static constexpr int NI = KS * (NA + NB);
  static constexpr int CNT_LO = NI / DMAW, REM = NI % DMAW, CNT_HI = CNT_LO + (REM ? 1 : 0);
  static_assert(DMAW == 8 || DMAW == 4, "DMA waves");
  static_assert(!LDR || DMAW == 4, "loader mode: the 4 loader waves issue every DMA");
  static constexpr int AHEAD = KS == 1 || (M16 && DEEP) ? NBUF : NBUF - 1;
  static_assert(!M16 || (KS == 2 && SCHED), "16x16x32 body: slot-scheduled 32-deep stages");
  static_assert(!DEEP || M16, "DEEP is a 16x16x32 option");
#ifndef MQ_X6P_GM
#define MQ_X6P_GM 4
#endif
  static constexpr int GM = MQ_X6P_GM;
  static_assert(LDR ? NW == 4 : NW == 8, "8-wave workgroups");
  static_assert(!SCHED || (CNT_HI - 1) * DSTEP < TM * TN * 6 * (M16 ? 4 : 1), "DMAs per k-step slots");
  static_assert(AHEAD >= 2 && NBUF * STAGE <= 160 * 1024, "LDS ring");
};

#ifndef MQ_X6P_HS
#define MQ_X6P_HS 2
#endif
#ifndef MQ_X6P_SPLIT_BIAS
#define MQ_X6P_SPLIT_BIAS 0
#endif
constexpr bool epi_is_split(int epi) {
  return epi == EPI_GELU_ERF || epi == EPI_GELU_TANH || epi == EPI_GELU_ERF_LNFOLD || epi == EPI_GELU_TANH_LNFOLD ||
         (MQ_X6P_SPLIT_BIAS != 0 && (epi == EPI_BIAS || epi == EPI_BIAS_LNFOLD));
}

template <class T, int EPI, bool FORMER = false>
__global__ __launch_bounds__(T::THREADS, 1) void gemm_x6p_kernel(const float* __restrict__ A, int lda,
                                                             const unsigned char* __restrict__ W3,
                                                             const float* __restrict__ bias,
                                                             const float* __restrict__ resid, int ldr,
                                                             float* __restrict__ out, int ldo, int M, int N,
                                                             int K, int rx, LnFold lf, AttnEpi at) {
  __shared__ __attribute__((aligned(1024))) unsigned char lds[T::NBUF * T::STAGE];
  const unsigned lds0 = (unsigned)(uintptr_t)(x6p_lds_t*)lds;
  constexpr bool HAND = EPI == EPI_RESID_LN_STATS && T::LDR && T::M16 && !T::DEEP && T::NBUF == 3 && !FORMER;
  constexpr bool ATTN = epi_is_attn(EPI);
  static_assert(!ATTN || (T::LDR && T::M16 && !T::DEEP && T::NBUF == 3 && T::WAVES_M == 2 && T::WAVES_N == 2 &&
                          T::TM == 2 && T::TN == 3 && 4 * kAttnStage <= T::STAGE),
                "attention epilogue: the 128 x 192 loader-wave tile");
  static_assert(!HAND || (T::NW == 4 && 2 * T::WM * T::WN * 4 <= T::STAGE && T::WN == kLnPartW && T::STAGE % 1024 == 0),
                "hand-off: two wave tiles of t per ring slot");
  constexpr int HS = MQ_X6P_HS;
  constexpr bool SPLIT = epi_is_split(EPI) && !FORMER && T::LDR && T::M16 && !T::DEEP && T::NBUF == 3 && T::TM == 2 &&
                         T::TN == 3;
  static_assert(!SPLIT || ((HS == 1 || HS == 2) && 4 * HS * 2 * T::TN * 1024 <= T::STAGE),
                "split epilogue: the handed blocks of the four compute waves fit one ring slot");
  const int lane = threadIdx.x & 63;
  const int wave = __builtin_amdgcn_readfirstlane(threadIdx.x >> 6);
  const int cw = T::LDR ? wave % T::NW : wave;
  const int wm = cw / T::WAVES_N, wn = cw % T::WAVES_N;
  const int tiles_m = (M + T::BM - 1) / T::BM, tiles_n = (N + T::BN - 1) / T::BN;
  const int total = tiles_m * tiles_n;
  const int G = gridDim.x, per_xcd = G >> 3;
  const int xslot = (blockIdx.x & 7) * per_xcd + (blockIdx.x >> 3);
  int m_lo = 0, rm = tiles_m, n_lo = 0, rn = tiles_n, loc = xslot, wstep = G, rtiles = total;
  if (rx > 0) {
    const Region rg = region_of(rx, blockIdx.x & 7, tiles_m, tiles_n);
    m_lo = rg.m_lo;
    rm = rg.rm;
    n_lo = rg.n_lo;
    rn = rg.rn;
    loc = blockIdx.x >> 3;
    wstep = per_xcd;
    rtiles = rm * rn;
  }
  const int n_tiles = loc < rtiles ? (rtiles - loc + wstep - 1) / wstep : 0;
  if (n_tiles == 0) return;
  const int nk = K >> 4;
  const int nst = nk / T::KS;
  const int S = n_tiles * nst;
  const int nbw = (N + 31) >> 5;
  const int band_tiles = T::GM * rn;
  auto coords = [&](int i, int& m0, int& n0) {
    const int t = i * wstep + loc;
    const int band = t / band_tiles;
    const int gm = min(T::GM, rm - band * T::GM);
    const int w = t - band * band_tiles;
    const int tc = w / gm;
    m0 = (m_lo + band * T::GM + (w - tc * gm)) * T::BM;
    n0 = (n_lo + tc) * T::BN;
  };

  int is_j = 0, is_i = 0, is_kt = 0, is_m0, is_n0;
  coords(0, is_m0, is_n0);
  const unsigned a_chunk = (unsigned)(((lane & 3) ^ a_swz((lane >> 4) & 3)) * 16);
  auto issue_one = [&](int buf, int t) __attribute__((always_inline)) {
    if constexpr (T::DBG & 1) return;
    if constexpr (T::DBG & 64) {
      if (is_j >= T::AHEAD) return;
    }
    const int dw = T::LDR ? wave - T::NW : wave;
    if (dw < 0 || dw >= T::DMAW || (T::REM && t == T::CNT_HI - 1 && dw >= T::REM)) return;
    const unsigned dst = lds0 + (unsigned)(buf * T::STAGE);
    const int ins = dw + t * T::DMAW;
    const int ks = ins / (T::NA + T::NB), in = ins - ks * (T::NA + T::NB);
    const int kt = is_kt + ks;
    if (in < T::NA) {
      if constexpr (T::DBG & 16) return;
      const float* abase = A + (int64_t)is_m0 * lda + kt * 16;
      const unsigned voff = (unsigned)min(16 * in + (lane >> 2), M - 1 - is_m0) * (unsigned)lda * 4u + a_chunk;
      x6p_glds(abase, voff, dst + ks * T::A_SUB + in * 1024);
    } else {
      if constexpr (T::DBG & 32) return;
      const int b = in - T::NA, nbl = b / 3, p = b - nbl * 3;
      int nbg = min((is_n0 >> 5) + nbl, nbw - 1);
      if constexpr (ATTN) nbg = (nbl % 3) * (N / 96) + 2 * (is_n0 / T::BN) + nbl / 3;
      const unsigned char* wbase = W3 + ((size_t)(nbg * nk + kt) * 3 + p) * 1024;
      x6p_glds(wbase, (unsigned)lane * 16u, dst + T::KS * T::A_SUB + ks * T::B_SUB + b * 1024);
    }
  };
  auto advance = [&]() __attribute__((always_inline)) {
    if (is_j + 1 < S) {
      ++is_j;
      is_kt += T::KS;
      if (is_kt == nk) {
        is_kt = 0;
        ++is_i;
        coords(is_i, is_m0, is_n0);
      }
    }
  };
  auto issue = [&](int buf) __attribute__((always_inline)) {
#pragma unroll
    for (int t = 0; t < T::CNT_HI; ++t) issue_one(buf, t);
    advance();
  };

  const int r = lane & 31, h = lane >> 5, sw = a_swz((r >> 2) & 3);
  const unsigned a_lo = (unsigned)((((2 * h) ^ sw) * 16)), a_hi = (unsigned)((((2 * h + 1) ^ sw) * 16));
  struct Frags {
    floatx4 raw[T::TM][2];
    bf16x8 a[T::TM][3], b[T::TN][3];
  };
  auto read_frags = [&](int buf, int ks, Frags& f) __attribute__((always_inline)) {
    if constexpr (T::DBG & 8) return;
    const unsigned char* st = lds + buf * T::STAGE;
#pragma unroll
    for (int tm = 0; tm < T::TM; ++tm) {
      const unsigned char* ar = st + ks * T::A_SUB + (wm * T::WM + tm * 32 + r) * 64;
      f.raw[tm][0] = *reinterpret_cast<const floatx4*>(ar + a_lo);
      f.raw[tm][1] = *reinterpret_cast<const floatx4*>(ar + a_hi);
    }
    const unsigned char* bs = st + T::KS * T::A_SUB + ks * T::B_SUB + lane * 16;
#pragma unroll
    for (int tn = 0; tn < T::TN; ++tn)
#pragma unroll
      for (int p = 0; p < 3; ++p)
        f.b[tn][p] = __builtin_bit_cast(bf16x8, *reinterpret_cast<const uintx4*>(bs + ((wn * T::TN + tn) * 3 + p) * 1024));
  };
  auto split_frags = [&](Frags& f) __attribute__((always_inline)) {
#pragma unroll
    for (int tm = 0; tm < T::TM; ++tm) {
      if constexpr (T::DBG & 2) {
        f.a[tm][0] = __builtin_bit_cast(bf16x8, f.raw[tm][0]);
        f.a[tm][1] = __builtin_bit_cast(bf16x8, f.raw[tm][1]);
        f.a[tm][2] = f.a[tm][0];
        continue;
      }
      uint2 pl[3], ph[3];
      split3v(f.raw[tm][0], pl);
      split3v(f.raw[tm][1], ph);
#pragma unroll
      for (int p = 0; p < 3; ++p) {
        uintx4 v;
        v.x = pl[p].x;
        v.y = pl[p].y;
        v.z = ph[p].x;
        v.w = ph[p].y;
        f.a[tm][p] = __builtin_bit_cast(bf16x8, v);
      }
    }
  };
  floatx16 acc[T::TM][T::TN];
  auto mma = [&](const Frags& f, auto&& hook) __attribute__((always_inline)) {
#pragma unroll
    for (int tm = 0; tm < T::TM; ++tm)
#pragma unroll
      for (int tn = 0; tn < T::TN; ++tn) {
        acc[tm][tn] = __builtin_amdgcn_mfma_f32_32x32x16_bf16(f.a[tm][2], f.b[tn][0], acc[tm][tn], 0, 0, 0);
        acc[tm][tn] = __builtin_amdgcn_mfma_f32_32x32x16_bf16(f.a[tm][1], f.b[tn][1], acc[tm][tn], 0, 0, 0);
        acc[tm][tn] = __builtin_amdgcn_mfma_f32_32x32x16_bf16(f.a[tm][0], f.b[tn][2], acc[tm][tn], 0, 0, 0);
        acc[tm][tn] = __builtin_amdgcn_mfma_f32_32x32x16_bf16(f.a[tm][1], f.b[tn][0], acc[tm][tn], 0, 0, 0);
        acc[tm][tn] = __builtin_amdgcn_mfma_f32_32x32x16_bf16(f.a[tm][0], f.b[tn][1], acc[tm][tn], 0, 0, 0);
        acc[tm][tn] = __builtin_amdgcn_mfma_f32_32x32x16_bf16(f.a[tm][0], f.b[tn][0], acc[tm][tn], 0, 0, 0);
        hook(tm * T::TN + tn);
      }
  };
  auto mma_one = [&](const Frags& f, int i) __attribute__((always_inline)) {
    const int g = i / 6, tm = g / T::TN, tn = g % T::TN, term = i % 6;
    const int pa = term == 0 ? 2 : term == 1 || term == 3 ? 1 : 0;
    const int pb = term == 0 || term >= 3 ? (term == 4 ? 1 : 0) : term == 1 ? 1 : 2;
    acc[tm][tn] = __builtin_amdgcn_mfma_f32_32x32x16_bf16(f.a[tm][pa], f.b[tn][pb], acc[tm][tn], 0, 0, 0);
  };
  auto read_a = [&](int buf, int ks, Frags& f) __attribute__((always_inline)) {
    if constexpr ((T::DBG & 8) || (T::DBG & 512)) {
#pragma unroll
      for (int tm = 0; tm < T::TM; ++tm) asm volatile("" : "+v"(f.raw[tm][0]), "+v"(f.raw[tm][1]));
      return;
    }
    const unsigned char* st = lds + buf * T::STAGE;
#pragma unroll
    for (int tm = 0; tm < T::TM; ++tm) {
      const unsigned char* ar = st + ks * T::A_SUB + (wm * T::WM + tm * 32 + r) * 64;
      f.raw[tm][0] = *reinterpret_cast<const floatx4*>(ar + a_lo);
      f.raw[tm][1] = *reinterpret_cast<const floatx4*>(ar + a_hi);
    }
  };
  auto read_b = [&](int buf, int ks, Frags& f, int q) __attribute__((always_inline)) {
    if constexpr ((T::DBG & 8) || (T::DBG & 256)) {
      asm volatile("" : "+v"(f.b[q / 3][q % 3]));
      return;
    }
    const unsigned char* bs = lds + buf * T::STAGE + T::KS * T::A_SUB + ks * T::B_SUB + lane * 16;
    f.b[q / 3][q % 3] = __builtin_bit_cast(bf16x8, *reinterpret_cast<const uintx4*>(bs + ((wn * T::TN) * 3 + q) * 1024));
  };
  unsigned pk[T::TM][2][3][2];
  auto piece = [&](Frags& f, int q) __attribute__((always_inline)) {
    const int tm = q / 12, half = (q / 6) % 2, p = (q % 6) / 2, part = q % 2;
    floatx4& x = f.raw[tm][half];
    unsigned u;
    if (part == 0) {
      u = cvt_pk_bf16(x.x, x.y);
      if (p < 2) {
        x.x -= bf16_lo(u);
        x.y -= bf16_hi(u);
      }
    } else {
      u = cvt_pk_bf16(x.z, x.w);
      if (p < 2) {
        x.z -= bf16_lo(u);
        x.w -= bf16_hi(u);
      }
    }
    asm volatile("" : "+v"(u), "+v"(x));
    pk[tm][half][p][part] = u;
  };
  auto assemble = [&](Frags& f) __attribute__((always_inline)) {
#pragma unroll
    for (int tm = 0; tm < T::TM; ++tm)
#pragma unroll
      for (int p = 0; p < 3; ++p) {
        uintx4 v;
        v.x = pk[tm][0][p][0];
        v.y = pk[tm][0][p][1];
        v.z = pk[tm][1][p][0];
        v.w = pk[tm][1][p][1];
        f.a[tm][p] = __builtin_bit_cast(bf16x8, v);
        asm volatile("" : "+v"(f.a[tm][p]));
      }
  };
  int c_i = 0, c_st = 0;
  auto tile_end = [&]() __attribute__((always_inline)) {
    if (++c_st == nst) {
      c_st = 0;
      int m0, n0;
      coords(c_i, m0, n0);
      if constexpr (!(T::DBG & 4))
        store_wave_tile<EPI, T::TM, T::TN>(acc, m0 + wm * T::WM, n0 + wn * T::WN, M, N, bias, resid, ldr, out, ldo,
                                           lane);
      zero_acc<T>(acc);
      ++c_i;
    }
  };
  auto wait_stages = [&](auto stages) __attribute__((always_inline)) {
    constexpr int n = decltype(stages)::value;
    const int dwi = T::LDR ? wave - T::NW : wave;
    if constexpr (T::DBG & 128) {
      if (T::REM && dwi >= 0 && dwi < T::REM)
        asm volatile("s_waitcnt vmcnt(%0)\n\ts_waitcnt lgkmcnt(0)" ::"n"(T::CNT_HI * n) : "memory");
      else
        asm volatile("s_waitcnt vmcnt(%0)\n\ts_waitcnt lgkmcnt(0)" ::"n"(T::CNT_LO * n) : "memory");
      return;
    }
    if (T::REM && dwi >= 0 && dwi < T::REM)
      asm volatile("s_waitcnt vmcnt(%0)" ::"n"(T::CNT_HI * n) : "memory");
    else
      asm volatile("s_waitcnt vmcnt(%0)" ::"n"(T::CNT_LO * n) : "memory");
    __builtin_amdgcn_s_waitcnt(0xC07F);
    asm volatile("s_barrier" ::: "memory");
  };
  zero_acc<T>(acc);

  if constexpr (T::LDR) {
    if (wave >= T::NW) {
#pragma unroll
      for (int d = 0; d < T::AHEAD; ++d) issue(d);
      wait_stages(IC<T::AHEAD - 1>{});
      if constexpr (HAND) {
        static_assert(T::AHEAD == 2, "hand-off: the ring two stages ahead");
        for (int j = 0; j + 2 < S; ++j) {
          wait_stages(IC<0>{});
          issue((j + 2) % T::NBUF);
        }
        if (S >= 2) wait_stages(IC<0>{});
        int m0, n0;
        coords(n_tiles - 1, m0, n0);
        LnTileRegs<2 * T::TM, 2 * T::TN> q;
        ln_tile_load(q, resid, ldr, m0 + wm * T::WM, n0 + wn * T::WN, M, lf, lane);
        wait_stages(IC<0>{});
        const int ts = (S + (cw >> 1)) % T::NBUF;
        ln_tile_write(q, lds + ts * T::STAGE + (cw & 1) * (T::WM * T::WN * 4), lf, lane);
        __builtin_amdgcn_s_waitcnt(0xC07F);
        asm volatile("s_barrier" ::: "memory");
        return;
      }
      int l_st = 0;
      [[maybe_unused]] int l_i = 0;
      for (int j = 0; j < S; ++j) {
        wait_stages(IC<T::AHEAD - 2>{});
        issue((j + T::AHEAD) % T::NBUF);
        if constexpr (ATTN) {
          if (++l_st == nst) {
            l_st = 0;
            asm volatile("s_barrier" ::: "memory");
          }
        }
        if constexpr (SPLIT) {
          if (++l_st == nst) {
            l_st = 0;
            static_assert(T::AHEAD == 2, "split epilogue: the ring two stages ahead");
            constexpr int MB = 2 * T::TM, NB16 = 2 * T::TN;
            int m0, n0;
            coords(l_i++, m0, n0);
            const int wr0 = m0 + wm * T::WM, wc0 = n0 + wn * T::WN;
            EpiPre<NB16> pre;
            epi_pre_load<EPI, MB, NB16>(pre, wr0, wc0, M, N, bias, lf, lane);
            asm volatile("s_barrier" ::: "memory");
            const unsigned char* hs = lds + (j % T::NBUF) * T::STAGE + cw * (HS * NB16 * 1024) + lane * 16;
            floatx4 hacc[MB][NB16];
#pragma unroll
            for (int m = 0; m < HS; ++m)
#pragma unroll
              for (int n = 0; n < NB16; ++n)
                hacc[MB - HS + m][n] = *reinterpret_cast<const floatx4*>(hs + (m * NB16 + n) * 1024);
            store_wave_tile16<EPI, MB, NB16, MB - HS, MB, true>(hacc, wr0, wc0, M, N, bias, resid, ldr, out, ldo, lane,
                                                                lf, &pre);
          }
        }
      }
      asm volatile("s_waitcnt vmcnt(0)" ::: "memory");
      return;
    }
  } else {
#pragma unroll
    for (int d = 0; d < T::AHEAD; ++d) issue(d);
  }
  if constexpr (T::M16) {
    constexpr int MB = 2 * T::TM, NB16 = 2 * T::TN, RS = NB16 * 6, NM16 = MB * RS, NSUB = 28;
    static_assert(RS >= NSUB + 4, "a region holds one block's split and its raw reads");
    const int c = lane & 15, kq = lane >> 4, hq = kq & 1, sw16 = a_swz((c >> 2) & 3);
    const unsigned a_base = (unsigned)((kq >> 1) * T::A_SUB + (wm * T::WM + c) * 64);
    const unsigned a_lo16 = a_base + (unsigned)(((2 * hq) ^ sw16) * 16);
    const unsigned a_hi16 = a_base + (unsigned)(((2 * hq + 1) ^ sw16) * 16);
    const unsigned b_base =
        (unsigned)(T::KS * T::A_SUB + (kq >> 1) * T::B_SUB + wn * T::TN * 3 * 1024 + hq * 512 + c * 16);
    floatx4 acc4[MB][NB16];
    uintx4 au[MB][3];
    bf16x8 bw[NB16][3];
    floatx4 raw[2];
    auto rd_raw = [&](const unsigned char* st, int m, int half) __attribute__((always_inline)) {
      raw[half] = *reinterpret_cast<const floatx4*>(st + m * 1024 + (half ? a_hi16 : a_lo16));
    };
    auto rd_b = [&](const unsigned char* st, int n, int p) __attribute__((always_inline)) {
      bw[n][p] = __builtin_bit_cast(
          bf16x8, *reinterpret_cast<const uintx4*>(st + b_base + ((n >> 1) * 3 + p) * 1024 + (n & 1) * 256));
    };
    auto sub = [&](int m, int q) __attribute__((always_inline)) {
      const int half = q / 14, rq = q % 14;
      const int p = rq < 12 ? rq / 6 : 2, part = rq < 12 ? (rq % 6) / 3 : rq - 12, op = rq < 12 ? rq % 3 : 0;
      floatx4& x = raw[half];
      if (op == 0) {
        unsigned u = cvt_pk_bf16(x[2 * part], x[2 * part + 1]);
        asm volatile("" : "+v"(u));
        au[m][p][2 * half + part] = u;
      } else {
        const unsigned u = au[m][p][2 * half + part];
        if (op == 1)
          x[2 * part] -= bf16_lo(u);
        else
          x[2 * part + 1] -= bf16_hi(u);
        asm volatile("" : "+v"(x));
      }
    };
    auto zero4 = [&]() __attribute__((always_inline)) {
#pragma unroll
      for (int m = 0; m < MB; ++m)
#pragma unroll
        for (int n = 0; n < NB16; ++n) acc4[m][n] = floatx4{0.f, 0.f, 0.f, 0.f};
    };
    zero4();
    wait_stages(IC<T::AHEAD - 1>{});
    auto load_ops = [&](const unsigned char* st) __attribute__((always_inline)) {
#pragma unroll
      for (int m = 0; m < MB; ++m) {
        rd_raw(st, m, 0);
        rd_raw(st, m, 1);
        if (m < MB - 1) {
#pragma unroll
          for (int q = 0; q < NSUB; ++q) sub(m, q);
        }
      }
#pragma unroll
      for (int n = 0; n < NB16; ++n)
#pragma unroll
        for (int p = 0; p < 3; ++p) rd_b(st, n, p);
    };
    load_ops(lds);
    int rb = 1 % T::NBUF;
    int ib = T::AHEAD % T::NBUF;
    for (int j = 0; j < S; ++j) {
      if constexpr (!T::LDR) {
        wait_stages(IC<T::AHEAD - 2>{});
      } else {
        if constexpr (T::DEEP) __builtin_amdgcn_s_waitcnt(0xC07F);
        if constexpr (ATTN || SPLIT) {
          if (c_st == nst - 1) __builtin_amdgcn_s_waitcnt(0xC07F);
        }
        asm volatile("s_barrier" ::: "memory");
      }
      const unsigned char* st = lds + rb * T::STAGE;
      static_for<NM16>([&](auto ic) {
        constexpr int i = decltype(ic)::value;
        constexpr int m = i / RS, w = i % RS, n = w / 6, term = w % 6;
        constexpr int pa = term == 0 ? 2 : term == 1 || term == 3 ? 1 : 0;
        constexpr int pb = term == 0 || term >= 3 ? (term == 4 ? 1 : 0) : term == 1 ? 1 : 2;
        acc4[m][n] = __builtin_amdgcn_mfma_f32_16x16x32_bf16(__builtin_bit_cast(bf16x8, au[m][pa]), bw[n][pb],
                                                             acc4[m][n], 0, 0, 0);
        if constexpr (w >= 2 && w < 2 + NSUB) sub((m + MB - 1) % MB, w - 2);
        if constexpr (w == 2 + NSUB || w == 3 + NSUB) rd_raw(st, m, w - 2 - NSUB);
        if constexpr (m == MB - 1 && term == 2) rd_b(st, n, 2);
        if constexpr (m == MB - 1 && term == 4) rd_b(st, n, 1);
        if constexpr (m == MB - 1 && term == 5) rd_b(st, n, 0);
        if constexpr (!T::LDR && i % T::DSTEP == 0 && i / T::DSTEP < T::CNT_HI) issue_one(ib, i / T::DSTEP);
        __builtin_amdgcn_sched_barrier(0);
      });
      if constexpr (!T::LDR) {
        advance();
        ib = ib + 1 == T::NBUF ? 0 : ib + 1;
      }
      rb = rb + 1 == T::NBUF ? 0 : rb + 1;
      if (++c_st == nst) {
        if constexpr (HAND) {
          if (j == S - 1) break;
        }
        c_st = 0;
        int m0, n0;
        coords(c_i, m0, n0);
        if constexpr (ATTN) {
          unsigned char* fs = lds + (j % T::NBUF) * T::STAGE;
          attn_wave_tile<EPI == EPI_ATTN_LNFOLD>(acc4, m0 + wm * T::WM, n0 / T::BN, wn, M, N / 3, bias, lf, at.mask,
                                                 at.scale, out, lane, fs + cw * kAttnStage,
                                                 fs + (cw ^ 1) * kAttnStage);
          load_ops(st);
        } else if constexpr (SPLIT) {
          unsigned char* hs = lds + (j % T::NBUF) * T::STAGE + cw * (HS * NB16 * 1024) + lane * 16;
#pragma unroll
          for (int m = 0; m < HS; ++m)
#pragma unroll
            for (int n = 0; n < NB16; ++n)
              *reinterpret_cast<floatx4*>(hs + (m * NB16 + n) * 1024) = acc4[MB - HS + m][n];
          __builtin_amdgcn_s_waitcnt(0xC07F);
          asm volatile("s_barrier" ::: "memory");
          store_wave_tile16<EPI, MB, NB16, 0, MB - HS>(acc4, m0 + wm * T::WM, n0 + wn * T::WN, M, N, bias, resid, ldr,
                                                       out, ldo, lane, lf);
        } else {
          store_wave_tile16<EPI, MB, NB16>(acc4, m0 + wm * T::WM, n0 + wn * T::WN, M, N, bias, resid, ldr, out, ldo,
                                           lane, lf);
        }
        zero4();
        ++c_i;
      }
    }
    if constexpr (HAND) {
      asm volatile("s_barrier" ::: "memory");
      int m0, n0;
      coords(n_tiles - 1, m0, n0);
      const int ts = (S + (cw >> 1)) % T::NBUF;
      store_wave_tile16_ln_stats<1, MB, NB16, true>(acc4, m0 + wm * T::WM, n0 + wn * T::WN, M, bias, resid, ldr, out,
                                                    ldo, lane, lf,
                                                    lds + ts * T::STAGE + (cw & 1) * (T::WM * T::WN * 4));
      return;
    }
    if constexpr (!T::LDR) asm volatile("s_waitcnt vmcnt(0)" ::: "memory");
    return;
  }
  wait_stages(IC<T::AHEAD - 1>{});
  Frags f0 = {}, f1 = {};
  read_frags(0, 0, f0);
  split_frags(f0);
  auto step = [&](int j, Frags& fa, Frags& fb) __attribute__((always_inline)) {
    wait_stages(IC<T::AHEAD - 2>{});
    const int buf = (j + T::AHEAD) % T::NBUF;
    if constexpr (!T::SCHED && !T::LDR) issue(buf);
    static_for<T::KS>([&](auto kc) {
      constexpr int ks = decltype(kc)::value;
      Frags& cur = ks % 2 == 0 ? fa : fb;
      Frags& nxt = ks % 2 == 0 ? fb : fa;
      if constexpr (T::SCHED) {
        constexpr int NM = T::TM * T::TN * 6, NBR = 3 * T::TN, PS = T::PS, NP = 12 * T::TM;
        constexpr int PER = (NP + (NM - PS) - 1) / (NM - PS);
        const int rbuf = ks + 1 < T::KS ? j % T::NBUF : (j + 1) % T::NBUF;
        constexpr int rks = ks + 1 < T::KS ? ks + 1 : 0;
        read_a(rbuf, rks, nxt);
        __builtin_amdgcn_sched_barrier(0);
        static_for<NM>([&](auto ic) {
          constexpr int i = decltype(ic)::value;
          mma_one(cur, i);
          constexpr bool dma_slot = !T::LDR && ks == 0 && i % T::DSTEP == 0 && i / T::DSTEP < T::CNT_HI;
          constexpr int bslot = [] {
            int n = 0;
            for (int k = T::BR0; k < i; ++k)
              if (!(!T::LDR && ks == 0 && k % T::DSTEP == 0 && k / T::DSTEP < T::CNT_HI) || T::DSTEP == 1) ++n;
            return n;
          }();
          if constexpr (i >= T::BR0 && (!dma_slot || T::DSTEP == 1)) {
            if constexpr (2 * bslot < NBR) read_b(rbuf, rks, nxt, 2 * bslot);
            if constexpr (2 * bslot + 1 < NBR) read_b(rbuf, rks, nxt, 2 * bslot + 1);
          }
          if constexpr (dma_slot) issue_one(buf, i / T::DSTEP);
          if constexpr (i >= PS) {
            static_for<PER>([&](auto pc) {
              constexpr int q = (i - PS) * PER + decltype(pc)::value;
              if constexpr (q < NP) piece(nxt, q);
            });
          }
          __builtin_amdgcn_sched_barrier(0);
        });
        assemble(nxt);
      } else {
        if constexpr (ks + 1 < T::KS)
          read_frags(j % T::NBUF, ks + 1, nxt);
        else
          read_frags((j + 1) % T::NBUF, 0, nxt);
        mma(cur, [](int) {});
        split_frags(nxt);
      }
    });
    if constexpr (T::SCHED && !T::LDR) advance();
    tile_end();
  };
  if constexpr (T::KS % 2 == 0) {
    for (int j = 0; j < S; ++j) step(j, f0, f1);
  } else {
    for (int j = 0; j < S; j += 2) {
      step(j, f0, f1);
      if (j + 1 >= S) break;
      step(j + 1, f1, f0);
    }
  }
  asm volatile("s_waitcnt vmcnt(0)" ::: "memory");
}

__global__ __launch_bounds__(256) void attn32_kernel(const float* __restrict__ qkv, const int* __restrict__ mask,
                                                     float* __restrict__ ctx, int M, int H, float scale) {
  __shared__ __attribute__((aligned(16))) unsigned char stg[4 * kAttnStage];
  const int lane = threadIdx.x & 63, c = lane & 15, g = lane >> 4;
  const int cw = __builtin_amdgcn_readfirstlane(threadIdx.x >> 6), wm = cw >> 1, wn = cw & 1;
  const int heads = H / 64, head = blockIdx.x % heads, wr0 = (blockIdx.x / heads) * 128 + 64 * wm;
  floatx4 acc[4][6];
#pragma unroll
  for (int m = 0; m < 4; ++m)
#pragma unroll
    for (int e = 0; e < 4; ++e) {
      const float* row = qkv + (int64_t)min(wr0 + 16 * m + 4 * g + e, M - 1) * (3 * H) + 64 * head + 32 * wn + c;
#pragma unroll
      for (int n = 0; n < 6; ++n) acc[m][n][e] = row[(n >> 1) * H + 16 * (n & 1)];
    }
  attn_wave_tile<false, true>(acc, wr0, head, wn, M, H, nullptr, LnFold{}, mask, scale, ctx, lane,
                              stg + cw * kAttnStage, stg + (cw ^ 1) * kAttnStage);
}

__global__ __launch_bounds__(256) void split_w3_kernel(const float* __restrict__ W, int N, int K,
                                                       uintx4* __restrict__ w3) {
  const int k8n = K >> 3, np = (N + 31) & ~31;
  const int64_t idx = (int64_t)blockIdx.x * 256 + threadIdx.x;
  if (idx >= (int64_t)np * k8n) return;
  const int n = (int)(idx / k8n), k8 = (int)(idx - (int64_t)n * k8n);
  floatx4 lo = {0.f, 0.f, 0.f, 0.f}, hi = lo;
  if (n < N) {
    lo = *reinterpret_cast<const floatx4*>(W + (int64_t)n * K + 8 * k8);
    hi = *reinterpret_cast<const floatx4*>(W + (int64_t)n * K + 8 * k8 + 4);
  }
  uint2 pl[3], ph[3];
  split3(lo, pl);
  split3(hi, ph);
  const int kb = k8 >> 1, hh = k8 & 1, nb = n >> 5, rr = n & 31;
#pragma unroll
  for (int p = 0; p < 3; ++p) {
    uintx4 v;
    v.x = pl[p].x;
    v.y = pl[p].y;
    v.z = ph[p].x;
    v.w = ph[p].y;
    w3[((int64_t)(nb * (K >> 4) + kb) * 3 + p) * 64 + hh * 32 + rr] = v;
  }
}

using X6p0 = X6pTile<2, 2, 2, 3, 3, 2, 4, true, 0, 1, 0, 6, true, true>;
using X6p1 = X6pTile<4, 1, 2, 3, 3, 2, 4, true, 0, 1, 0, 6, true, true>;
using X6p2 = X6pTile<4, 2, 1, 3, 3, 2, 4, true, 0, 2, 1, 6, false, true>;
using X6p3 = X6pTile<4, 2, 2, 3, 2, 2, 8, true, 0, 6, 1, 8, false, true, true>;
using X6p4 = X6pTile<2, 2, 2, 3, 3, 2, 4, true, 0, 1, 0, 6, true, true, true>;
using X6p5 = X6pTile<2, 2, 1, 3, 3, 2, 4, true, 0, 1, 0, 6, true, true, true>;
using X6p6 = X6pTile<4, 1, 2, 3, 3, 2, 4, true, 0, 1, 0, 6, true, true, true>;
using X6p7 = X6pTile<2, 2, 1, 3, 3, 2, 4, true, 0, 1, 0, 6, true, true>;
using X6p16 = X6pTile<2, 2, 2, 3, 4, 1, 4, true, 0, 1, 0, 6, true>;
using X6p17 = X6pTile<2, 2, 1, 3, 4, 1, 4, true, 0, 1, 0, 6, true>;

template <class T, int EPI, bool FORMER = false>
void launch_t(const X6pArgs& g, int num_cus, hipStream_t s) {
  if constexpr (EPI < EPI_RESID_LN_STATS) {
    if (g.K % (16 * T::KS) != 0) {
      launch_t<X6pTile<4, 2, 1, 3, 4>, EPI>(g, num_cus, s);
      return;
    }
  }
  const int tiles = ((g.M + T::BM - 1) / T::BM) * ((g.N + T::BN - 1) / T::BN);
  int grid = (std::min(tiles, num_cus) + 7) / 8 * 8;
  if (g.max_wg > 0) grid = std::min(grid, g.max_wg);
  const int tiles_m = (g.M + T::BM - 1) / T::BM, tiles_n = (g.N + T::BN - 1) / T::BN;
  int rx = g.rx;
  if (rx < 0) rx = region_pick_rx(tiles_m, tiles_n, (double)T::BM * g.K * 4, (double)T::BN * g.K * 6, grid);
  if (rx > 0 && (8 % rx != 0 || rx > tiles_n || 8 / rx > tiles_m || grid < 8)) rx = 0;
  hipLaunchKernelGGL((gemm_x6p_kernel<T, EPI, FORMER>), dim3(grid), dim3(T::THREADS), 0, s, g.A, g.lda,
                     static_cast<const unsigned char*>(g.W3), g.bias, g.resid, g.ldr, g.out, g.ldo, g.M, g.N, g.K, rx,
                     g.lf, g.at);
}

template <int EPI>
void launch_tile(const X6pArgs& g, int tile, int num_cus, hipStream_t s) {
#ifdef MQ_X6P_DBG
  if (tile >= 8) {
    switch (tile) {
      case 8: launch_t<X6pTile<2, 2, 2, 3, 4, 1, 4, true, 64, 1, 0, 6, true>, EPI>(g, num_cus, s); return;
      case 9: launch_t<X6pTile<2, 2, 2, 3, 4, 1, 4, true, 66, 1, 0, 6, true>, EPI>(g, num_cus, s); return;
      case 10: launch_t<X6pTile<2, 2, 2, 3, 4, 1, 4, true, 8, 1, 0, 6, true>, EPI>(g, num_cus, s); return;
      case 11: launch_t<X6pTile<2, 2, 2, 3, 4, 1, 4, true, 74, 1, 0, 6, true>, EPI>(g, num_cus, s); return;
      case 12: launch_t<X6pTile<2, 2, 2, 3, 4, 1, 4, true, 2, 1, 0, 6, true>, EPI>(g, num_cus, s); return;
      case 13: launch_t<X6pTile<2, 2, 2, 3, 4, 1, 4, true, 256, 1, 0, 6, true>, EPI>(g, num_cus, s); return;
      case 14: launch_t<X6pTile<2, 2, 2, 3, 4, 1, 4, true, 512, 1, 0, 6, true>, EPI>(g, num_cus, s); return;
      default: launch_t<X6pTile<2, 2, 2, 3, 4, 1, 4, true, 128, 1, 0, 6, true>, EPI>(g, num_cus, s); return;
    }
  }
#endif
  switch (tile) {
    case 1: launch_t<X6p1, EPI>(g, num_cus, s); return;
    case 2: launch_t<X6p2, EPI>(g, num_cus, s); return;
    case 3: launch_t<X6p3, EPI>(g, num_cus, s); return;
    case 4: launch_t<X6p4, EPI>(g, num_cus, s); return;
    case 5: launch_t<X6p5, EPI>(g, num_cus, s); return;
    case 6: launch_t<X6p6, EPI>(g, num_cus, s); return;
    case 7: launch_t<X6p7, EPI>(g, num_cus, s); return;
    case 16: launch_t<X6p16, EPI>(g, num_cus, s); return;
    case 17: launch_t<X6p17, EPI>(g, num_cus, s); return;
    case 20: launch_t<X6p0, EPI, epi_is_split(EPI)>(g, num_cus, s); return;
    case 21: launch_t<X6p1, EPI, epi_is_split(EPI)>(g, num_cus, s); return;
    default: launch_t<X6p0, EPI>(g, num_cus, s); return;
  }
}

template <int EPI>
void launch_tile_fold(const X6pArgs& g, int tile, int num_cus, hipStream_t s) {
  constexpr bool HAS_FORMER = EPI == EPI_RESID_LN_STATS || epi_is_split(EPI);
  switch (tile) {
    case 1: launch_t<X6p1, EPI>(g, num_cus, s); return;
    case 20: launch_t<X6p0, EPI, HAS_FORMER>(g, num_cus, s); return;
    case 21: launch_t<X6p1, EPI, HAS_FORMER>(g, num_cus, s); return;
    default: launch_t<X6p0, EPI>(g, num_cus, s); return;
  }
}

__global__ __launch_bounds__(256) void ln_fold_weight_kernel(const float* __restrict__ W,
                                                             const float* __restrict__ bias,
                                                             const float* __restrict__ g,
                                                             const float* __restrict__ b, int N, int K,
                                                             float* __restrict__ Wg, float* __restrict__ s_out,
                                                             float* __restrict__ c_out) {
  const int lane = threadIdx.x & 63;
  const int n = blockIdx.x * 4 + (threadIdx.x >> 6);
  if (n >= N) return;
  double sg = 0.0, sb = 0.0;
  for (int k = lane; k < K; k += 64) {
    const float w = W[(int64_t)n * K + k];
    const float wg = g[k] * w;
    Wg[(int64_t)n * K + k] = wg;
    sg += (double)wg;
    sb += (double)b[k] * (double)w;
  }
#pragma unroll
  for (int off = 32; off > 0; off >>= 1) {
    sg += __shfl_xor(sg, off);
    sb += __shfl_xor(sb, off);
  }
  if (lane == 0) {
    s_out[n] = (float)sg;
    c_out[n] = (float)((double)bias[n] + sb);
  }
}

}

void launch_ln_fold_weight(const float* W, const float* bias, const float* g, const float* b, int N, int K, float* Wg,
                           float* s_out, float* c_out, hipStream_t s) {
  hipLaunchKernelGGL(ln_fold_weight_kernel, dim3((unsigned)((N + 3) / 4)), dim3(256), 0, s, W, bias, g, b, N, K, Wg,
                     s_out, c_out);
}

void launch_attn32(const float* qkv, const int* mask, float* ctx, int M, int H, float scale, hipStream_t s) {
  hipLaunchKernelGGL(attn32_kernel, dim3((unsigned)(((M + 127) / 128) * (H / 64))), dim3(256), 0, s, qkv, mask, ctx, M,
                     H, scale);
}

void launch_split_w3(const float* W, int N, int K, void* w3, hipStream_t s) {
  const int64_t n = (int64_t)((N + 31) & ~31) * (K >> 3);
  hipLaunchKernelGGL(split_w3_kernel, dim3((unsigned)((n + 255) / 256)), dim3(256), 0, s, W, N, K,
                     static_cast<uintx4*>(w3));
}

int x6p_pick_tile(int M, int N, int num_cus) {
  auto rounds = [&](int bm, int bn) {
    const int64_t tiles = (int64_t)((M + bm - 1) / bm) * ((N + bn - 1) / bn);
    return (tiles + num_cus - 1) / num_cus;
  };
  return rounds(256, 96) < rounds(128, 192) ? 1 : 0;
}

void launch_gemm_x6p(const X6pArgs& g, int epi, int tile, int num_cus, hipStream_t s) {
  if (tile < 0) {
    tile = x6p_pick_tile(g.M, g.N, num_cus);
  }
  if (g.former_epi && epi_is_split(epi) && (tile == 0 || tile == 1)) tile += 20;
  switch (epi) {
    case EPI_GELU_ERF: launch_tile<EPI_GELU_ERF>(g, tile, num_cus, s); return;
    case EPI_GELU_TANH: launch_tile<EPI_GELU_TANH>(g, tile, num_cus, s); return;
    case EPI_RESID: launch_tile<EPI_RESID>(g, tile, num_cus, s); return;
    case EPI_RESID_LN_STATS: launch_tile_fold<EPI_RESID_LN_STATS>(g, tile, num_cus, s); return;
    case EPI_BIAS_LNFOLD: launch_tile_fold<EPI_BIAS_LNFOLD>(g, tile, num_cus, s); return;
    case EPI_GELU_ERF_LNFOLD: launch_tile_fold<EPI_GELU_ERF_LNFOLD>(g, tile, num_cus, s); return;
    case EPI_GELU_TANH_LNFOLD: launch_tile_fold<EPI_GELU_TANH_LNFOLD>(g, tile, num_cus, s); return;
    case EPI_ATTN_BIAS: launch_t<X6p0, EPI_ATTN_BIAS>(g, num_cus, s); return;
    case EPI_ATTN_LNFOLD: launch_t<X6p0, EPI_ATTN_LNFOLD>(g, num_cus, s); return;
    default: launch_tile<EPI_BIAS>(g, tile, num_cus, s); return;
  }
}

}

extern "C" {

int64_t mq_debug_w3_bytes(int N, int K) { return N > 0 && K > 0 && K % 16 == 0 ? (int64_t)mq::w3_bytes(N, K) : -1; }

int mq_debug_split_w3(const float* W, int N, int K, void* w3, void* stream) {
  using namespace mq;
  clear_error();
  MQ_CHECK_ARG(W && w3, "NULL buffer");
  MQ_CHECK_ARG(N > 0 && K > 0 && K % 16 == 0, "bad shape N=%d K=%d", N, K);
  launch_split_w3(W, N, K, w3, (hipStream_t)stream);
  MQ_HIP(hipGetLastError());
  return MQ_OK;
}

int mq_debug_gemm_x6p(const float* A, const void* W3, const float* bias, const float* resid, float* out, int M,
                      int N, int K, int epi, int tile, void* stream) {
  using namespace mq;
  clear_error();
  MQ_CHECK_ARG(A && W3 && bias && out && (epi != EPI_RESID || resid), "NULL buffer");
  MQ_CHECK_ARG(M > 0 && N > 0 && K > 0 && K % 32 == 0, "bad shape M=%d N=%d K=%d", M, N, K);
  const int rx = tile >= 100 ? tile / 100 - 1 : -1;
  if (tile >= 100) tile %= 100;
  MQ_CHECK_ARG(epi >= 0 && epi <= 3 && tile >= -1 && (tile <= 17 || tile == 20 || tile == 21) && rx <= 8,
               "bad epi/tile");
  int dev = 0, cus = 256;
  (void)hipGetDevice(&dev);
  (void)hipDeviceGetAttribute(&cus, hipDeviceAttributeMultiprocessorCount, dev);
  X6pArgs g{A, K, W3, bias, resid, N, out, N, M, N, K};
  g.rx = rx;
  launch_gemm_x6p(g, epi, tile, cus, (hipStream_t)stream);
  MQ_HIP(hipGetLastError());
  return MQ_OK;
}

int mq_debug_ln_fold_weight(const float* W, const float* bias, const float* g, const float* b, int N, int K,
                            float* Wg, float* s_out, float* c_out, void* stream) {
  using namespace mq;
  clear_error();
  MQ_CHECK_ARG(W && bias && g && b && Wg && s_out && c_out, "NULL buffer");
  MQ_CHECK_ARG(N > 0 && K > 0, "bad shape N=%d K=%d", N, K);
  launch_ln_fold_weight(W, bias, g, b, N, K, Wg, s_out, c_out, (hipStream_t)stream);
  MQ_HIP(hipGetLastError());
  return MQ_OK;
}

int mq_debug_gemm_x6p_ln(const float* A, const void* W3, const float* bias, const float* resid, float* out, int M,
                         int N, int K, int epi, int tile, const float* stats_in, float* stats_out, const float* g,
                         const float* b, const float* s_fold, float eps, void* stream) {
  using namespace mq;
  clear_error();
  MQ_CHECK_ARG(A && W3 && bias && out, "NULL buffer");
  MQ_CHECK_ARG(M > 0 && N > 0 && K > 0 && K % 32 == 0, "bad shape M=%d N=%d K=%d", M, N, K);
  MQ_CHECK_ARG((tile >= -1 && tile <= 1) || tile == 20 || tile == 21,
               "the LayerNorm-fold epilogues run on tiles 0 and 1 (20 / 21: their former epilogues; got %d)", tile);
  if (epi == EPI_RESID_LN_STATS) {
    MQ_CHECK_ARG(resid && stats_out && (!stats_in || (g && b)), "producer: NULL buffer");
    MQ_CHECK_ARG(N == kLnPartW * kLnMaxParts, "producer: N must be %d (got %d)", kLnPartW * kLnMaxParts, N);
    MQ_CHECK_ARG((int64_t)M * N < (1ll << 29), "producer: M * N must stay below 2^29 (32-bit byte offsets)");
  } else {
    MQ_CHECK_ARG(epi_is_lnfold(epi), "epi must be a LayerNorm-fold kind (got %d)", epi);
    MQ_CHECK_ARG(stats_in && s_fold, "consumer: NULL buffer");
  }
  int dev = 0, cus = 256;
  (void)hipGetDevice(&dev);
  (void)hipDeviceGetAttribute(&cus, hipDeviceAttributeMultiprocessorCount, dev);
  X6pArgs a{A, K, W3, bias, resid, N, out, N, M, N, K};
  a.lf.stats_in = stats_in;
  a.lf.stats_out = stats_out;
  a.lf.g = g;
  a.lf.b = b;
  a.lf.s = s_fold;
  a.lf.eps = eps;
  launch_gemm_x6p(a, epi, tile, cus, (hipStream_t)stream);
  MQ_HIP(hipGetLastError());
  return MQ_OK;
}

int mq_debug_gemm_x6p_attn(const float* A, const void* W3, const float* bias, const int* mask, float* ctx, int M,
                           int K, int heads, float scale, int epi, const float* stats_in, const float* s_fold,
                           float eps, int max_workgroups, void* stream) {
  using namespace mq;
  clear_error();
  MQ_CHECK_ARG(A && W3 && bias && mask && ctx, "NULL buffer");
  MQ_CHECK_ARG(M > 0 && M % 32 == 0 && K > 0 && K % 32 == 0 && heads > 0 && heads <= 1024,
               "bad shape M=%d K=%d heads=%d (M and K must be multiples of 32)", M, K, heads);
  MQ_CHECK_ARG((int64_t)M * heads * 64 < (1ll << 31) && (int64_t)M * K < (1ll << 29), "M too large");
  MQ_CHECK_ARG(epi == EPI_ATTN_BIAS || epi == EPI_ATTN_LNFOLD, "epi must be an attention kind (got %d)", epi);
  MQ_CHECK_ARG(epi != EPI_ATTN_LNFOLD || (stats_in && s_fold), "fold: NULL buffer");
  MQ_CHECK_ARG(max_workgroups >= 0 && max_workgroups % 8 == 0,
               "max_workgroups must be 0 or a multiple of 8 (got %d)", max_workgroups);
  int dev = 0, cus = 256;
  (void)hipGetDevice(&dev);
  (void)hipDeviceGetAttribute(&cus, hipDeviceAttributeMultiprocessorCount, dev);
  const int H = 64 * heads;
  X6pArgs a{A, K, W3, bias, nullptr, 0, ctx, H, M, 3 * H, K};
  a.lf.stats_in = stats_in;
  a.lf.s = s_fold;
  a.lf.eps = eps;
  a.at.mask = mask;
  a.at.scale = scale;
  a.max_wg = max_workgroups;
  launch_gemm_x6p(a, epi, 0, cus, (hipStream_t)stream);
  MQ_HIP(hipGetLastError());
  return MQ_OK;
}

}
```

### mediquery-rag_amd/csrc/gemm_x6p.hpp

```cpp
#pragma once

#include <hip/hip_runtime.h>

#include <cstddef>
#include <cstdint>

namespace mq {

inline size_t w3_bytes(int64_t N, int64_t K) { return (size_t)((N + 31) / 32) * (size_t)(K / 16) * 3 * 1024; }
inline size_t w3_row_offset(int64_t row0, int64_t K) { return (size_t)(row0 / 32) * (size_t)(K / 16) * 3 * 1024; }

inline int region_pick_rx(int64_t tiles_m, int64_t tiles_n, double a_bytes_per_row_tile,
                          double w_bytes_per_col_tile, int64_t grid) {
  if (tiles_m * tiles_n <= grid || grid < 8) return 0;
  const double l2 = 4.0 * 1024 * 1024;
  const int64_t per_xcd = grid / 8;
  int best = 0;
  double best_b = 0;
  for (int rx = 1; rx <= 8; rx *= 2) {
    const int ry = 8 / rx;
    if (rx > tiles_n || ry > tiles_m) continue;
    const int64_t rm = (tiles_m + ry - 1) / ry, rn = (tiles_n + rx - 1) / rx;
    const int64_t rounds = (rm * rn + per_xcd - 1) / per_xcd;
    const double w = (double)rn * w_bytes_per_col_tile;
    const double b = (double)rm * a_bytes_per_row_tile + (w <= l2 ? w : w * (double)rounds);
    if (best == 0 || b < best_b) {
      best = rx;
      best_b = b;
    }
  }
  return best;
}
struct Region {
  int m_lo, rm, n_lo, rn;
};
__host__ __device__ inline Region region_of(int rx, int xc, int tiles_m, int tiles_n) {
  const int ry = 8 / rx, ri = xc / rx, rj = xc - ri * rx;
  Region r;
  r.m_lo = ri * tiles_m / ry;
  r.rm = (ri + 1) * tiles_m / ry - r.m_lo;
  r.n_lo = rj * tiles_n / rx;
  r.rn = (rj + 1) * tiles_n / rx - r.n_lo;
  return r;
}

void launch_split_w3(const float* W, int N, int K, void* w3, hipStream_t s);

constexpr int kLnPartW = 96;
constexpr int kLnMaxParts = 8;
struct LnFold {
  const float* stats_in = nullptr;
  float* stats_out = nullptr;
  const float* g = nullptr;
  const float* b = nullptr;
  const float* s = nullptr;
  float eps = 0.f;
};
void launch_ln_fold_weight(const float* W, const float* bias, const float* g, const float* b, int N, int K, float* Wg,
                           float* s_out, float* c_out, hipStream_t s);

struct AttnEpi {
  const int* mask = nullptr;
  float scale = 0.f;
};

struct X6pArgs {
  const float* A;
  int lda;
  const void* W3;
  const float* bias;
  const float* resid;
  int ldr;
  float* out;
  int ldo;
  int M, N, K;
  int rx = -1;
  LnFold lf{};
  AttnEpi at{};
  int max_wg = 0;
  bool former_epi = false;
};

void launch_attn32(const float* qkv, const int* mask, float* ctx, int M, int H, float scale, hipStream_t s);

int x6p_pick_tile(int M, int N, int num_cus);
void launch_gemm_x6p(const X6pArgs& g, int epi, int tile, int num_cus, hipStream_t s);

}
```

### mediquery-rag_amd/mediquery_hip/_lib.py

```python
import ctypes
import hashlib
import os

try:
    import torch
except Exception:
    torch = None

LIB_PATH = os.environ.get("MQ_LIB_PATH") or os.path.join(os.path.dirname(os.path.abspath(__file__)),
                                                          "libmqhip.so")

MQ_OK = 0
MQ_DTYPE_F32, MQ_DTYPE_BF16, MQ_DTYPE_F32X6, MQ_DTYPE_F32_SCREEN = 0, 1, 2, 3
MQ_GELU_ERF, MQ_GELU_TANH = 0, 1
MQ_POOL_CLS, MQ_POOL_MEAN = 0, 1
MQ_MAX_K = 64
MQ_HEAD_MAX_LABELS = 8
MQ_MASK_SET, MQ_MASK_AND, MQ_MASK_OR, MQ_MASK_CLEAR = 0, 1, 2, 3
MQ_CONTAINS_MAX_BYTES = 256
MQ_CONTAINS_SPAN_BYTES = 16384
MQ_LEX_MAX_TERMS = 128
MQ_ENC_OPT_ROWS_MAX, MQ_ENC_OPT_ROWS_SPLITS, MQ_ENC_OPT_SPLITK_MAX = 0, 1, 2
MQ_ENC_OPT_FUSE_ATTN_OPROJ = 4
MQ_ENC_OPT_SPLITK_TILES = 6
MQ_ENC_OPT_RESIDENT_LAYERS = 8
MQ_ENC_OPT_X6_PRESPLIT = 9
MQ_ENC_OPT_ROWS_PLANES = 10
MQ_ENC_OPT_LN_FOLD = 11
MQ_ENC_OPT_CLS_KFREE = 12
MQ_ENC_OPT_QKV_ATTN = 13
MQ_ENC_OPT_EPI_SPLIT = 14
MQ_ROWS_QKV, MQ_ROWS_UP, MQ_ROWS_OPROJ, MQ_ROWS_DOWN = 0, 1, 2, 3


class MQError(RuntimeError):

    def __init__(self, fn, code, msg):
        super().__init__("%s failed (status %d): %s" % (fn, code, msg))
        self.code = code


class BertConfigC(ctypes.Structure):
    _fields_ = [("vocab_size", ctypes.c_int), ("hidden", ctypes.c_int), ("layers", ctypes.c_int),
                ("heads", ctypes.c_int), ("ffn", ctypes.c_int), ("max_positions", ctypes.c_int),
                ("type_vocab", ctypes.c_int), ("ln_eps", ctypes.c_float), ("gelu", ctypes.c_int),
                ("pooling", ctypes.c_int)]

    @classmethod
    def from_config(cls, cfg):
        return cls(cfg.vocab_size, cfg.hidden, cfg.layers, cfg.heads, cfg.ffn, cfg.max_positions,
                   cfg.type_vocab, cfg.ln_eps, cfg.gelu, cfg.pooling)


_P = ctypes.c_void_p
_I = ctypes.c_int
_I64 = ctypes.c_int64
_PP = ctypes.POINTER(ctypes.c_void_p)

SIGNATURES = {
    "mq_last_error": (ctypes.c_char_p, []),
    "mq_version": (ctypes.c_char_p, []),
    "mq_build_source_hash": (ctypes.c_char_p, []),
    "mq_device_count": (_I, []),
    "mq_index_create": (_I, [_I, _I, _I64, _I, _PP]),
    "mq_index_destroy": (_I, [_P]),
    "mq_index_size": (_I, [_P, ctypes.POINTER(_I64)]),
    "mq_index_dim": (_I, [_P, ctypes.POINTER(_I)]),
    "mq_index_add": (_I, [_P, _P, _I64, _I, _P]),
    "mq_index_reset": (_I, [_P]),
    "mq_index_search": (_I, [_P, _P, _I64, _I, _P, _P, _I, _P]),
    "mq_index_get": (_I, [_P, _I64, _I64, _P, _I, _P]),
    "mq_index_select": (_I, [_P, _P, _I64, _P]),
    "mq_index_data": (_I, [_P, _PP]),
    "mq_index_set_precision": (_I, [_P, _I]),
    "mq_index_set_stream_threshold": (_I, [_P, _I]),
    "mq_index_set_threshold_scan": (_I, [_P, _I]),
    "mq_index_set_int8_screen": (_I, [_P, _I]),
    "mq_index_set_async_screen": (_I, [_P, _I]),
    "mq_index_rescans": (_I, [_P, _P, _P]),
    "mq_index_screen_fallbacks": (_I, [_P, _P, _P]),
    "mq_index_screen_skips": (_I, [_P, _P, _P]),
    "mq_index_set_timing": (_I, [_P, _I]),
    "mq_index_read_timing": (_I, [_P, _P, _I]),
    "mq_index_save": (_I, [_P, ctypes.c_char_p]),
    "mq_index_load": (_I, [_P, ctypes.c_char_p]),
    "mq_index_save_rows": (_I, [_P, ctypes.c_char_p, ctypes.c_int64, ctypes.c_int64]),
    "mq_index_load_append": (_I, [_P, ctypes.c_char_p]),
    "mq_mask_eval": (_I, [_P, _I64, _P, _I, _P, _I, _P]),
    "mq_mask_eval_bits": (_I, [_P, _I64, _P, _I, _P, _I, _P]),
    "mq_mask_combine": (_I, [_P, _P, _I64, _I, _P]),
    "mq_mask_contains": (_I, [_P, _I64, _P, _I64, _P, _I, _I, _P, _I, _P, _P]),
    "mq_lex_scratch_bytes": (_I64, [_I64, _I]),
    "mq_lex_df": (_I, [_P, _I64, _P, _I64, _I, _P, _I, _P, _P, _P]),
    "mq_lex_topk": (_I, [_P, _I64, _P, _I64, _I, _P, _P, _I, ctypes.c_float, ctypes.c_float, _P, _I, _P, _P, _I,
                         _P, _P]),
    "mq_index_search_masked": (_I, [_P, _P, _I, _P, _P, _P, _I, _P]),
    "mq_index_search_masked_batch": (_I, [_P, _P, _I64, _I, _P, _P, _P, _I, _P]),
    "mq_index_masked_gathers": (_I, [_P, ctypes.POINTER(_I64)]),
    "mq_index_mmr_select": (_I, [_P, _P, _P, _I64, _I, _I, ctypes.c_float, _P, _P, _I, _P]),
    "mq_index_search_mmr": (_I, [_P, _P, _I64, _I, _I, ctypes.c_float, _P, _P, _P, _I, _P]),
    "mq_topk_merge_host": (_I, [_P, _P, _I, _I64, _I, _I, _P, _P]),
    "mq_topk_merge_device": (_I, [_P, _P, _I, _I64, _I, _I, _P, _P, _P]),
    "mq_encoder_create": (_I, [_I, ctypes.POINTER(BertConfigC), _PP]),
    "mq_encoder_destroy": (_I, [_P]),
    "mq_encoder_weight_count": (_I64, [ctypes.POINTER(BertConfigC)]),
    "mq_encoder_load_weights": (_I, [_P, _P, _I64]),
    "mq_encoder_set_precision": (_I, [_P, _I]),
    "mq_encoder_set_graphs": (_I, [_P, _I]),
    "mq_encoder_set_option": (_I, [_P, _I, _I]),
    "mq_encoder_get_option": (_I, [_P, _I, ctypes.POINTER(ctypes.c_int)]),
    "mq_encoder_set_timing": (_I, [_P, _I]),
    "mq_encoder_read_timing": (_I, [_P, _P, _I]),
    "mq_encoder_embed": (_I, [_P, _P, _P, _I, _I, _P, _I, _P]),
    "mq_encoder_load_head": (_I, [_P, _P, _P, _P, _P, _I]),
    "mq_encoder_score": (_I, [_P, _P, _P, _P, _I, _I, _P, _I, _P]),
    "mq_tokenizer_create_wordpiece": (_I, [ctypes.c_char_p, _I, _I, _PP]),
    "mq_tokenizer_create_wordpiece_tokens": (_I, [ctypes.POINTER(ctypes.c_char_p), _I, _I, _I, _PP]),
    "mq_tokenizer_create_char": (_I, [_I, _I, _PP]),
    "mq_tokenizer_destroy": (_I, [_P]),
    "mq_tokenizer_encode_batch": (_I, [_P, ctypes.POINTER(ctypes.c_char_p), _I, _I, _P, _P,
                                       ctypes.POINTER(_I)]),
    "mq_tokenizer_encode_pairs": (_I, [_P, ctypes.POINTER(ctypes.c_char_p), ctypes.POINTER(ctypes.c_char_p), _I, _I,
                                       _P, _P, _P, ctypes.POINTER(_I)]),
    "mq_debug_cls_head": (_I, [_P, _I, _I, _P, _P, _P, _P, _I, _P, _P]),
    "mq_debug_gemm_f32": (_I, [_P, _P, _P, _P, _P, _I, _I, _I, _I, _I, _P]),
    "mq_debug_w3_bytes": (_I64, [_I, _I]),
    "mq_debug_split_w3": (_I, [_P, _I, _I, _P, _P]),
    "mq_debug_gemm_x6p": (_I, [_P, _P, _P, _P, _P, _I, _I, _I, _I, _I, _P]),
    "mq_debug_gemm_x6p_ln": (_I, [_P, _P, _P, _P, _P, _I, _I, _I, _I, _I, _P, _P, _P, _P, _P, ctypes.c_float, _P]),
    "mq_debug_ln_fold_weight": (_I, [_P, _P, _P, _P, _I, _I, _P, _P, _P, _P]),
    "mq_debug_gemm_x6p_attn": (_I, [_P, _P, _P, _P, _P, _I, _I, _I, ctypes.c_float, _I, _P, _P, ctypes.c_float, _I, _P]),
    "mq_debug_attention": (_I, [_P, _P, _I, _I, _I, _I, ctypes.c_float, _I, _P, _P]),
    "mq_debug_cls_attention": (_I, [_P, _P, _P, _P, _P, ctypes.c_float, _P, _I, _I, _I, _I, ctypes.c_float, _P, _P, _P,
                                    _P, _P]),
    "mq_debug_attn_oproj": (_I, [_P, _P, _I, _I, _I, _I, ctypes.c_float, _P, _P, _P, _I, _I, _I, _I, _P, _P]),
    "mq_debug_rows_gemm": (_I, [_I, _I, _P, _I, _I64, _I, _P, _P, _P, _I, _P, _I64, _I, _I, _I, _I, _P, _P,
                                ctypes.c_float, _P, _P, _P, _I, _I, _P, _P, _I, _I, _P, _I64, _P]),
    "mq_debug_ln_pool": (_I, [_P, _I, _I64, _P, _I, _I, _I, _I, _P, _P, ctypes.c_float, _I, _P, _I, _P]),
    "mq_debug_int8_screen":(_I, [_P, _P, _I, _P, _P, _P]),
}

_lib = None


def lib():
    global _lib
    if _lib is None:
        if not os.path.exists(LIB_PATH):
            raise ImportError("libmqhip.so not found at %s - build it with "
                              "`make -C mediquery-rag_amd/csrc` or __graft_entry__.build()" % LIB_PATH)
        h = ctypes.CDLL(LIB_PATH)
        allow_missing = os.environ.get("MQ_LIB_ALLOW_MISSING") == "1"
        for name, (res, args) in SIGNATURES.items():
            if allow_missing and not hasattr(h, name):
                continue
            fn = getattr(h, name)
            fn.restype = res
            fn.argtypes = args
        _lib = h
    return _lib


def check(fn_name, rc):
    if rc != MQ_OK:
        raise MQError(fn_name, rc, lib().mq_last_error().decode("utf-8", "replace"))
    return rc


def call(fn_name, *args):
    return check(fn_name, getattr(lib(), fn_name)(*args))


CSRC = os.path.join(os.path.dirname(os.path.dirname(os.path.abspath(__file__))), "csrc")
_STAMPED_EXT = (".hip", ".cpp", ".hpp", ".inc")


def tree_source_hash(csrc=CSRC):
    names = sorted(f for f in os.listdir(csrc) if f.endswith(_STAMPED_EXT))
    paths = [os.path.join(csrc, f) for f in names]
    paths += [os.path.join(csrc, "Makefile"), os.path.join(csrc, "..", "..", "include", "mq.h")]
    h = hashlib.sha256()
    for p in paths:
        with open(p, "rb") as f:
            h.update(f.read())
    return h.hexdigest()[:16]


def built_source_hash():
    return lib().mq_build_source_hash().decode()


def check_build_fresh():
    if not os.path.isdir(CSRC):
        return
    built, tree = built_source_hash(), tree_source_hash()
    if built != tree:
        raise ImportError("libmqhip.so at %s was built from sources %s, the tree holds %s: "
                          "rebuild with `make -C mediquery-rag_amd/csrc`" % (LIB_PATH, built, tree))


def device_count():
    return lib().mq_device_count()


def ptr(a):
    if a is None:
        return None
    if isinstance(a, int):
        return ctypes.c_void_p(a)
    if hasattr(a, "data_ptr"):
        return ctypes.c_void_p(a.data_ptr())
    return ctypes.c_void_p(a.ctypes.data)


class device_scope:

    def __init__(self, device):
        self._ctx = None
        if device is not None and torch is not None and torch.cuda.is_available():
            self._ctx = torch.cuda.device(int(device))

    def __enter__(self):
        if self._ctx is not None:
            self._ctx.__enter__()
        return self

    def __exit__(self, *exc):
        if self._ctx is not None:
            return self._ctx.__exit__(*exc)
        return False


def stream_handle(stream=None):
    if stream is None:
        if torch is None or not torch.cuda.is_available():
            return None
        stream = torch.cuda.current_stream()
    if isinstance(stream, int):
        return ctypes.c_void_p(stream)
    return ctypes.c_void_p(stream.cuda_stream)
```

### mediquery-rag_amd/mediquery_hip/native.py

```python
import ctypes

import numpy as np

from . import _lib
from .config import BertConfig
from .weights import head_from_state_dict, state_dict_to_blob, synthetic_state_dict


class FlatIndex:

    def __init__(self, dim=768, capacity=0, device=0, dtype=_lib.MQ_DTYPE_F32):
        h = ctypes.c_void_p()
        _lib.call("mq_index_create", device, dim, capacity, dtype, ctypes.byref(h))
        self._h = h
        self.dim = dim
        self.device = device

    def close(self):
        h, self._h = getattr(self, "_h", None), None
        if h:
            try:
                _lib.lib().mq_index_destroy(h)
            except Exception:
                pass
# ... 84 lines not shown
    @property
    def screen_passdowns(self):
        n = ctypes.c_int64()
        _lib.call("mq_index_screen_fallbacks", self._h, None, ctypes.byref(n))
        return n.value

    @property
    def screen_skips(self):
        n = ctypes.c_int64()
        _lib.call("mq_index_screen_skips", self._h, ctypes.byref(n), None)
        return n.value

    @property
    def int8_skips(self):
        n = ctypes.c_int64()
        _lib.call("mq_index_screen_skips", self._h, None, ctypes.byref(n))
        return n.value

    def set_timing(self, enabled=True):
        _lib.call("mq_index_set_timing", self._h, int(bool(enabled)))

    def read_timing(self):
        ms = np.zeros(len(self.STAGES), dtype=np.float32)
        _lib.call("mq_index_read_timing", self._h, _lib.ptr(ms), len(ms))
        return dict(zip(self.STAGES, ms.tolist()))

    def save(self, path):
        _lib.call("mq_index_save", self._h, str(path).encode())

    def load(self, path):
        _lib.call("mq_index_load", self._h, str(path).encode())

    def _check_bits(self, bits):
        check_mask_words(bits, len(self), self.device)

    def search_masked(self, queries, k, bits):
        q = np.ascontiguousarray(queries, dtype=np.float32).reshape(-1, self.dim)
        self._check_bits(bits)
        scores = np.empty((q.shape[0], k), dtype=np.float32)
        ids = np.empty((q.shape[0], k), dtype=np.int64)
        with _lib.device_scope(self.device):
            _lib.call("mq_index_search_masked_batch", self._h, _lib.ptr(q), q.shape[0], k, _lib.ptr(bits),
                      _lib.ptr(scores), _lib.ptr(ids), 0, _lib.stream_handle(None))
        return scores, ids

    def mmr_select(self, cand_scores, cand_ids, k, lambda_mult=0.5):
        s = np.ascontiguousarray(cand_scores, dtype=np.float32)
        i = np.ascontiguousarray(cand_ids, dtype=np.int64)
        s = s.reshape(1, -1) if s.ndim == 1 else s
        i = i.reshape(s.shape)
        scores = np.empty((s.shape[0], k), dtype=np.float32)
        ids = np.empty((s.shape[0], k), dtype=np.int64)
        with _lib.device_scope(self.device):
            _lib.call("mq_index_mmr_select", self._h, _lib.ptr(s), _lib.ptr(i), s.shape[0], s.shape[1], k,
                      float(lambda_mult), _lib.ptr(scores), _lib.ptr(ids), 0, _lib.stream_handle(None))
        return scores, ids

    def mmr_select_device(self, cand_scores, cand_ids, k, lambda_mult, out_scores, out_ids, stream=None):
        _lib.call("mq_index_mmr_select", self._h, _lib.ptr(cand_scores), _lib.ptr(cand_ids),
                  cand_scores.shape[0], cand_scores.shape[1], k, float(lambda_mult), _lib.ptr(out_scores),
                  _lib.ptr(out_ids), 1, _lib.stream_handle(stream))

    def search_mmr(self, queries, k, fetch_k, lambda_mult=0.5, bits=None):
        q = np.ascontiguousarray(queries, dtype=np.float32).reshape(-1, self.dim)
        if bits is not None:
            self._check_bits(bits)
        scores = np.empty((q.shape[0], k), dtype=np.float32)
        ids = np.empty((q.shape[0], k), dtype=np.int64)
        with _lib.device_scope(self.device):
            _lib.call("mq_index_search_mmr", self._h, _lib.ptr(q), q.shape[0], k, fetch_k, float(lambda_mult),
                      _lib.ptr(bits), _lib.ptr(scores), _lib.ptr(ids), 0, _lib.stream_handle(None))
        return scores, ids

    @property
    def masked_gathers(self):
        n = ctypes.c_int64()
        _lib.call("mq_index_masked_gathers", self._h, ctypes.byref(n))
        return n.value

    def save_rows(self, path, row0, n):
        _lib.call("mq_index_save_rows", self._h, str(path).encode(), int(row0), int(n))

    def load_append(self, path):
        _lib.call("mq_index_load_append", self._h, str(path).encode())


def merge_topk_host(scores, ids, k_out):
    scores = np.ascontiguousarray(scores, dtype=np.float32)
    ids = np.ascontiguousarray(ids, dtype=np.int64)
    n_lists, nq, k_in = scores.shape
    os_ = np.empty((nq, k_out), dtype=np.float32)
    oi = np.empty((nq, k_out), dtype=np.int64)
    _lib.call("mq_topk_merge_host", _lib.ptr(scores), _lib.ptr(ids), n_lists, nq, k_in, k_out,
              _lib.ptr(os_), _lib.ptr(oi))
    return os_, oi


def merge_topk_device(scores, ids, k_out, out_scores, out_ids, stream=None):
    n_lists, nq, k_in = scores.shape
    _lib.call("mq_topk_merge_device", _lib.ptr(scores), _lib.ptr(ids), n_lists, nq, k_in, k_out,
              _lib.ptr(out_scores), _lib.ptr(out_ids), _lib.stream_handle(stream))


class Encoder:

    def __init__(self, cfg: BertConfig, weights=None, seed=0, device=0):
        self.cfg = cfg
        self.device = device
        self._ccfg = _lib.BertConfigC.from_config(cfg)
        h = ctypes.c_void_p()
        _lib.call("mq_encoder_create", device, ctypes.byref(self._ccfg), ctypes.byref(h))
        self._h = h
        sd = weights if weights is not None else synthetic_state_dict(cfg, seed)
        blob = state_dict_to_blob(cfg, sd)
        n = _lib.lib().mq_encoder_weight_count(ctypes.byref(self._ccfg))
        if n != blob.size:
            raise ValueError("weight blob %d floats, library expects %d" % (blob.size, n))
        _lib.call("mq_encoder_load_weights", self._h, _lib.ptr(blob), blob.size)
        self.n_labels = 0

    def close(self):
        h, self._h = getattr(self, "_h", None), None
        if h:
            try:
                _lib.lib().mq_encoder_destroy(h)
            except Exception:
                pass

    __del__ = close

    STAGES = ("embed_ln", "qkv_gemm", "attention", "out_proj_gemm", "layernorm", "ffn_up_gemm",
              "ffn_down_gemm", "pool")

    def set_timing(self, enabled=True):
        _lib.call("mq_encoder_set_timing", self._h, int(bool(enabled)))

    def read_timing(self):
        ms = np.zeros(len(self.STAGES), dtype=np.float32)
        _lib.call("mq_encoder_read_timing", self._h, _lib.ptr(ms), len(ms))
        return dict(zip(self.STAGES, ms.tolist()))

    def set_precision(self, dtype):
        _lib.call("mq_encoder_set_precision", self._h, dtype)

    def set_graphs(self, enabled=True):
        _lib.call("mq_encoder_set_graphs", self._h, int(bool(enabled)))

    OPTIONS = {"rows_max": _lib.MQ_ENC_OPT_ROWS_MAX, "rows_splits": _lib.MQ_ENC_OPT_ROWS_SPLITS,
               "splitk_max": _lib.MQ_ENC_OPT_SPLITK_MAX, "fuse_attn_oproj": _lib.MQ_ENC_OPT_FUSE_ATTN_OPROJ,
               "splitk_tiles": _lib.MQ_ENC_OPT_SPLITK_TILES,
               "resident_layers": _lib.MQ_ENC_OPT_RESIDENT_LAYERS, "x6_presplit": _lib.MQ_ENC_OPT_X6_PRESPLIT,
               "rows_planes": _lib.MQ_ENC_OPT_ROWS_PLANES, "ln_fold": _lib.MQ_ENC_OPT_LN_FOLD,
               "cls_kfree": _lib.MQ_ENC_OPT_CLS_KFREE, "qkv_attn": _lib.MQ_ENC_OPT_QKV_ATTN,
               "epi_split": _lib.MQ_ENC_OPT_EPI_SPLIT}

    def set_option(self, name, value):
        _lib.call("mq_encoder_set_option", self._h, self.OPTIONS[name], int(value))

    def get_option(self, name):
        v = ctypes.c_int()
        _lib.call("mq_encoder_get_option", self._h, self.OPTIONS[name], ctypes.byref(v))
        return v.value

    def embed(self, ids, mask):
        ids = np.ascontiguousarray(ids, dtype=np.int32)
        mask = np.ascontiguousarray(mask, dtype=np.int32)
        B, L = ids.shape
        out = np.empty((B, self.cfg.hidden), dtype=np.float32)
        _lib.call("mq_encoder_embed", self._h, _lib.ptr(ids), _lib.ptr(mask), B, L, _lib.ptr(out),
                  0, None)
        return out

    def embed_device(self, ids, mask, out, stream=None):
        B, L = ids.shape
        _lib.call("mq_encoder_embed", self._h, _lib.ptr(ids), _lib.ptr(mask), B, L, _lib.ptr(out),
                  1, _lib.stream_handle(stream))

    def load_head(self, sd):
        pw, pb, cw, cb = head_from_state_dict(sd, self.cfg)
        n_labels = int(cw.shape[0])
        if not 1 <= n_labels <= _lib.MQ_HEAD_MAX_LABELS:
            raise ValueError("n_labels must be in [1, %d] (got %d)" % (_lib.MQ_HEAD_MAX_LABELS, n_labels))
        _lib.call("mq_encoder_load_head", self._h, _lib.ptr(pw), _lib.ptr(pb), _lib.ptr(cw), _lib.ptr(cb), n_labels)
        self.n_labels = n_labels

    def score(self, ids, types, mask):
        ids = np.ascontiguousarray(ids, dtype=np.int32)
        types = np.ascontiguousarray(types, dtype=np.int32)
        mask = np.ascontiguousarray(mask, dtype=np.int32)
        if types.shape != ids.shape or mask.shape != ids.shape or ids.ndim != 2:
            raise ValueError("ids, types and mask must share one [B, L] shape")
        B, L = ids.shape
        out = np.empty((B, max(1, self.n_labels)), dtype=np.float32)
        _lib.call("mq_encoder_score", self._h, _lib.ptr(ids), _lib.ptr(types), _lib.ptr(mask), B, L,
                  _lib.ptr(out), 0, None)
        return out

    def score_device(self, ids, types, mask, out, stream=None):
        if tuple(types.shape) != tuple(ids.shape) or tuple(mask.shape) != tuple(ids.shape):
            raise ValueError("ids, types and mask must share one [B, L] shape")
        B, L = ids.shape
        if out.numel() < B * max(1, self.n_labels):
            raise ValueError("out holds %d floats, needs B * n_labels = %d" % (out.numel(), B * self.n_labels))
        _lib.call("mq_encoder_score", self._h, _lib.ptr(ids), _lib.ptr(types), _lib.ptr(mask), B, L,
                  _lib.ptr(out), 1, _lib.stream_handle(stream))


def check_mask_words(bits, n, device=None):
    if not (getattr(bits, "is_cuda", False) and bits.element_size() == 4 and bits.is_contiguous()
            and bits.numel() >= (int(n) + 31) // 32):
        raise ValueError("bits must be a contiguous 32-bit device tensor of >= ceil(n / 32) = %d words"
                         % ((int(n) + 31) // 32))
    if device is not None and bits.device.index != int(device):
        raise ValueError("bits lives on cuda:%s, the index on cuda:%d" % (bits.device.index, int(device)))


def _check_codes(codes, bits):
    import torch
    if not (getattr(codes, "is_cuda", False) and codes.dtype == torch.int32 and codes.is_contiguous()):
        raise ValueError("codes must be a contiguous int32 device tensor")
    check_mask_words(bits, codes.numel(), codes.device.index)


def mask_eval(codes, lut, bits, mode, stream=None):
    import torch
    _check_codes(codes, bits)
    if not (getattr(lut, "is_cuda", False) and lut.dtype == torch.uint8 and lut.is_contiguous()
            and lut.device == codes.device and lut.numel() >= 1):
        raise ValueError("lut must be a non-empty contiguous uint8 tensor on the codes' device")
    with _lib.device_scope(codes.device.index):
        _lib.call("mq_mask_eval", _lib.ptr(codes), codes.numel(), _lib.ptr(lut), lut.numel(), _lib.ptr(bits),
                  mode, _lib.stream_handle(stream))


def mask_eval_bits(codes, lut, bits, mode, stream=None):
    _check_codes(codes, bits)
    lut = np.asarray(lut).astype(bool)
    if not 1 <= lut.size <= 256:
        raise ValueError("a by-value table holds 1..256 entries (got %d)" % lut.size)
    words = np.zeros(4, dtype=np.uint64)
    for i in np.flatnonzero(lut).tolist():
        words[i >> 6] |= np.uint64(1 << (i & 63))
    with _lib.device_scope(codes.device.index):
        _lib.call("mq_mask_eval_bits", _lib.ptr(codes), codes.numel(), _lib.ptr(words), len(lut), _lib.ptr(bits),
                  mode, _lib.stream_handle(stream))


def mask_contains(text, offsets, pattern, bits, mode, negate=False, stream=None, scratch=None):
    import torch
    if not (getattr(text, "is_cuda", False) and text.dtype == torch.uint8 and text.is_contiguous()
            and text.dim() == 1):
        raise ValueError("text must be a contiguous 1-d uint8 device tensor")
    if text.numel() and text.data_ptr() % 16:
        raise ValueError("text must start at a 16-byte aligned address")
    if not (getattr(offsets, "is_cuda", False) and offsets.dtype == torch.int64 and offsets.is_contiguous()
            and offsets.numel() >= 1 and offsets.device == text.device):
        raise ValueError("offsets must be a contiguous int64 tensor of n + 1 elements on the text's device")
    n = offsets.numel() - 1
    check_mask_words(bits, n, text.device.index)
    if not isinstance(pattern, (bytes, bytearray)) or not 1 <= len(pattern) <= _lib.MQ_CONTAINS_MAX_BYTES:
        raise ValueError("pattern must be 1..%d bytes" % _lib.MQ_CONTAINS_MAX_BYTES)
    with _lib.device_scope(text.device.index):
        if scratch is None:
            scratch = torch.empty(max(1, (n + 31) // 32), dtype=torch.int32, device=text.device)
        check_mask_words(scratch, n, text.device.index)
        if scratch.data_ptr() == bits.data_ptr():
            raise ValueError("scratch must not be bits")
        _lib.call("mq_mask_contains", _lib.ptr(text), text.numel(), _lib.ptr(offsets), n, bytes(pattern),
                  len(pattern), int(bool(negate)), _lib.ptr(bits), mode, _lib.ptr(scratch),
                  _lib.stream_handle(stream))


def lex_scratch_bytes(n, k=_lib.MQ_MAX_K):
    return int(_lib.lib().mq_lex_scratch_bytes(int(n), int(k)))


def _check_lex(tokens, offsets, ngram, keys, scratch, k):
    import torch
    if not (getattr(tokens, "is_cuda", False) and tokens.dtype == torch.uint16 and tokens.is_contiguous()
            and tokens.dim() == 1):
        raise ValueError("tokens must be a contiguous 1-d uint16 device tensor")
    if tokens.numel() and tokens.data_ptr() % 16:
        raise ValueError("tokens must start at a 16-byte aligned address")
    if not (getattr(offsets, "is_cuda", False) and offsets.dtype == torch.int64 and offsets.is_contiguous()
            and offsets.numel() >= 1 and offsets.device == tokens.device):
        raise ValueError("offsets must be a contiguous int64 tensor of n + 1 elements on the tokens' device")
    if ngram not in (1, 2):
        raise ValueError("ngram must be 1 or 2 (got %r)" % (ngram,))
    n = offsets.numel() - 1
    keys = np.ascontiguousarray(keys, dtype=np.uint32).reshape(-1)
    if not 1 <= keys.size <= _lib.MQ_LEX_MAX_TERMS:
        raise ValueError("a call takes 1..%d terms (got %d)" % (_lib.MQ_LEX_MAX_TERMS, keys.size))
    if np.unique(keys).size != keys.size:
        raise ValueError("keys must be distinct")
    need = lex_scratch_bytes(n, k)
    if scratch is None:
        scratch = torch.empty(need, dtype=torch.uint8, device=tokens.device)
    if not (getattr(scratch, "is_cuda", False) and scratch.is_contiguous() and scratch.device == tokens.device
            and scratch.numel() * scratch.element_size() >= need and scratch.data_ptr() % 16 == 0):
        raise ValueError("scratch must be a contiguous 16-byte aligned tensor of >= %d bytes on the tokens' device"
                         % need)
    return n, keys, scratch


def lex_df(tokens, offsets, ngram, keys, scratch=None, stream=None):
    n, keys, scratch = _check_lex(tokens, offsets, ngram, keys, scratch, 1)
    df = np.zeros(keys.size, dtype=np.int64)
# ... 42 lines not shown
```

Measured before the change: 40020.

## Add epilogue parameter prefetch option with staged LDS loads in x6p GEMM

Measured after the change: 40020. No clear change (-0.0%).

```diff
diff --git a/include/mq.h b/include/mq.h
--- a/include/mq.h
+++ b/include/mq.h
@@ -137,6 +137,7 @@
 #define MQ_ENC_OPT_CLS_KFREE 12
 #define MQ_ENC_OPT_QKV_ATTN 13
 #define MQ_ENC_OPT_EPI_SPLIT 14
+#define MQ_ENC_OPT_EPI_PREFETCH 15
 int mq_encoder_set_option(mq_encoder* enc, int option, int value);
 int mq_encoder_get_option(const mq_encoder* enc, int option, int* value);
 int mq_encoder_set_timing(mq_encoder* enc, int enabled);
@@ -179,6 +180,10 @@
                            float* ctx, int M, int K, int heads, float scale, int epi,
                            const float* stats_in, const float* s_fold, float eps, int max_workgroups,
                            void* stream);
+int mq_debug_gemm_x6p_attn_v(const float* A, const void* W3, const float* bias, const int* mask,
+                             float* ctx, int M, int K, int heads, float scale, int epi,
+                             const float* stats_in, const float* s_fold, float eps, int max_workgroups,
+                             int prefetch, void* stream);
 int mq_debug_attention(const float* qkv, const int* mask, int B, int L, int H, int heads, float scale,
                        int variant, float* ctx, void* stream);
 int mq_debug_cls_attention(const float* q, const float* x, const float* stats, const float* ln_g,
diff --git a/mediquery-rag_amd/csrc/encoder.hip b/mediquery-rag_amd/csrc/encoder.hip
--- a/mediquery-rag_amd/csrc/encoder.hip
+++ b/mediquery-rag_amd/csrc/encoder.hip
@@ -1473,6 +1473,7 @@
   const void* W3 = nullptr;
   LnFold lf{};
   bool former_epi = false;
+  bool no_prefetch = false;
 };
 
 template <class T, int EPI>
@@ -1566,6 +1567,7 @@
     X6pArgs a{g.A, g.lda, g.W3, g.bias, g.resid, g.ldr, g.out, g.ldo, g.M, g.N, g.K};
     a.lf = g.lf;
     a.former_epi = g.former_epi;
+    a.no_prefetch = g.no_prefetch;
     launch_gemm_x6p(a, EPI, -1, num_cus, s);
     return;
   }
@@ -1592,6 +1594,7 @@
   if (x6 && g.W3) {
     X6pArgs a{g.A, g.lda, g.W3, g.bias, g.resid, g.ldr, g.out, g.ldo, g.M, g.N, g.K};
     a.former_epi = g.former_epi;
+    a.no_prefetch = g.no_prefetch;
     launch_gemm_x6p(a, EPI, -1, num_cus, s);
     return;
   }
@@ -1635,6 +1638,10 @@
 #define MQ_EPI_SPLIT_DEFAULT 1
 #endif
 constexpr bool kEpiSplitDefault = MQ_EPI_SPLIT_DEFAULT != 0;
+#ifndef MQ_EPI_PREFETCH_DEFAULT
+#define MQ_EPI_PREFETCH_DEFAULT 0
+#endif
+constexpr bool kEpiPrefetchDefault = MQ_EPI_PREFETCH_DEFAULT != 0;
 
 enum Stage { ST_EMBED = 0, ST_QKV, ST_ATTN, ST_OPROJ, ST_LN, ST_FFN_UP, ST_FFN_DOWN, ST_POOL, ST_N };
 
@@ -1679,6 +1686,7 @@
   bool cls_kfree = kClsKfreeDefault;
   bool qkv_attn = kQkvAttnDefault;
   bool epi_split = kEpiSplitDefault;
+  bool epi_prefetch = kEpiPrefetchDefault;
   Buf wkt;
   Buf cls;
   Buf head;
@@ -1816,6 +1824,7 @@
   GemmArgs a = g;
   if (!e->x6_presplit) a.W3 = nullptr;
   a.former_epi = !e->epi_split;
+  a.no_prefetch = !e->epi_prefetch;
   launch_gemm<EPI>(a, e->num_cus, s, e->precision == MQ_DTYPE_F32X6, e->splitk_max, e->splitk_tiles);
 }
 
@@ -1931,6 +1940,7 @@
     e->tl.mark(s, stage);
     if (!e->x6_presplit) g.W3 = nullptr;
     g.former_epi = !e->epi_split;
+    g.no_prefetch = !e->epi_prefetch;
     g.lf.eps = c.ln_eps;
     launch_gemm_fold<decltype(epi)::value>(g, e->num_cus, s);
   };
@@ -2003,6 +2013,7 @@
       }
       a.at.mask = mask;
       a.at.scale = scale;
+      a.no_prefetch = !e->epi_prefetch;
       e->tl.mark(s, ST_QKV);
       launch_gemm_x6p(a, raw ? EPI_ATTN_LNFOLD : EPI_ATTN_BIAS, 0, e->num_cus, s);
       attn_done = true;
@@ -2877,6 +2888,10 @@
       MQ_CHECK_ARG(value == 0 || value == 1, "epi_split must be 0 or 1 (got %d)", value);
       e->epi_split = value != 0;
       break;
+    case MQ_ENC_OPT_EPI_PREFETCH:
+      MQ_CHECK_ARG(value == 0 || value == 1, "epi_prefetch must be 0 or 1 (got %d)", value);
+      e->epi_prefetch = value != 0;
+      break;
     default:
       MQ_FAIL(MQ_EINVAL, "unknown encoder option %d", option);
   }
@@ -2901,6 +2916,7 @@
     case MQ_ENC_OPT_CLS_KFREE: *value = e->cls_kfree ? 1 : 0; break;
     case MQ_ENC_OPT_QKV_ATTN: *value = e->qkv_attn ? 1 : 0; break;
     case MQ_ENC_OPT_EPI_SPLIT: *value = e->epi_split ? 1 : 0; break;
+    case MQ_ENC_OPT_EPI_PREFETCH: *value = e->epi_prefetch ? 1 : 0; break;
     default: MQ_FAIL(MQ_EINVAL, "unknown encoder option %d", option);
   }
   return MQ_OK;
diff --git a/mediquery-rag_amd/csrc/gemm_epi.hpp b/mediquery-rag_amd/csrc/gemm_epi.hpp
--- a/mediquery-rag_amd/csrc/gemm_epi.hpp
+++ b/mediquery-rag_amd/csrc/gemm_epi.hpp
@@ -302,6 +302,88 @@
   }
   if constexpr (epi_is_lnfold(EPI)) ln_row_own<MB>(lf.stats_in, wr0, M, lf.eps, lane, p.own_mu, p.own_rho);
 }
+template <int NB>
+struct EpiPreRaw {
+  float bv[NB], sv[NB];
+  floatx4 p[kLnMaxParts / 2];
+};
+__device__ __forceinline__ float pre_ld(const float* a) {
+  float v;
+  asm volatile("global_load_dword %0, %1, off" : "=&v"(v) : "v"(a) : "memory");
+  return v;
+}
+template <int EPI, int MB, int NB>
+__device__ __forceinline__ void epi_pre_issue(EpiPreRaw<NB>& q, int wr0, int wc0, int M, int N,
+                                              const float* __restrict__ bias, const LnFold& lf, int lane) {
+#pragma unroll
+  for (int n = 0; n < NB; ++n) {
+    const int col = min(wc0 + n * 16 + (lane & 15), N - 1);
+    q.bv[n] = pre_ld(bias + col);
+    q.sv[n] = epi_is_lnfold(EPI) ? pre_ld(lf.s + col) : 0.f;
+  }
+  if constexpr (epi_is_lnfold(EPI)) {
+    static_assert(kLnMaxParts == 8, "four 16-byte loads per row");
+    const int c = lane & 15;
+    const int row = min(wr0 + 16 * min(c >> 2, MB - 1) + 4 * (lane >> 4) + (c & 3), M - 1);
+    const float* src = lf.stats_in + (int64_t)row * (2 * kLnMaxParts);
+    asm volatile(
+        "global_load_dwordx4 %0, %4, off\n\tglobal_load_dwordx4 %1, %4, off offset:16\n\t"
+        "global_load_dwordx4 %2, %4, off offset:32\n\tglobal_load_dwordx4 %3, %4, off offset:48"
+        : "=&v"(q.p[0]), "=&v"(q.p[1]), "=&v"(q.p[2]), "=&v"(q.p[3])
+        : "v"(src)
+        : "memory");
+  }
+}
+template <int EPI, int NB, int BEHIND>
+__device__ __forceinline__ void epi_pre_wait(EpiPreRaw<NB>& q, EpiPre<NB>& p, float eps) {
+  static_assert(NB == 6, "the operand lists below");
+  asm volatile("s_waitcnt vmcnt(%12)"
+               : "+v"(q.bv[0]), "+v"(q.bv[1]), "+v"(q.bv[2]), "+v"(q.bv[3]), "+v"(q.bv[4]), "+v"(q.bv[5]),
+                 "+v"(q.sv[0]), "+v"(q.sv[1]), "+v"(q.sv[2]), "+v"(q.sv[3]), "+v"(q.sv[4]), "+v"(q.sv[5])
+               : "n"(BEHIND)
+               : "memory");
+#pragma unroll
+  for (int n = 0; n < NB; ++n) {
+    p.bv[n] = q.bv[n];
+    p.sv[n] = q.sv[n];
+  }
+  if constexpr (epi_is_lnfold(EPI)) {
+    asm volatile("" : "+v"(q.p[0]), "+v"(q.p[1]), "+v"(q.p[2]), "+v"(q.p[3])::"memory");
+    ln_merge(q.p, eps, p.own_mu, p.own_rho);
+  }
+}
+template <int NB, int R>
+constexpr int epi_pre_lds_bytes() {
+  return 8 * NB * 16 + 2 * 4 * (4 * R) * 4;
+}
+template <int NB, int R>
+__device__ __forceinline__ void epi_pre_lds_write(const EpiPre<NB>& p, unsigned char* z, int lane) {
+  static_assert(NB == 6, "three 16-byte pieces per column");
+  const int c = lane & 15, g = lane >> 4;
+  if (g == 0) {
+    floatx4* d = reinterpret_cast<floatx4*>(z + c * (8 * NB));
+    d[0] = floatx4{p.bv[0], p.bv[1], p.bv[2], p.bv[3]};
+    d[1] = floatx4{p.bv[4], p.bv[5], p.sv[0], p.sv[1]};
+    d[2] = floatx4{p.sv[2], p.sv[3], p.sv[4], p.sv[5]};
+  }
+  if (c < 4 * R) {
+    float* st = reinterpret_cast<float*>(z + 8 * NB * 16);
+    st[4 * R * g + c] = p.own_mu;
+    st[16 * R + 4 * R * g + c] = p.own_rho;
+  }
+}
+template <int NB, int R>
+__device__ __forceinline__ void epi_pre_lds_read(EpiPre<NB>& p, const unsigned char* z, int lane) {
+  static_assert(NB == 6, "three 16-byte pieces per column");
+  const int c = lane & 15, g = lane >> 4;
+  const floatx4* d = reinterpret_cast<const floatx4*>(z + c * (8 * NB));
+  const floatx4 d0 = d[0], d1 = d[1], d2 = d[2];
+  p.bv[0] = d0.x, p.bv[1] = d0.y, p.bv[2] = d0.z, p.bv[3] = d0.w, p.bv[4] = d1.x, p.bv[5] = d1.y;
+  p.sv[0] = d1.z, p.sv[1] = d1.w, p.sv[2] = d2.x, p.sv[3] = d2.y, p.sv[4] = d2.z, p.sv[5] = d2.w;
+  const float* st = reinterpret_cast<const float*>(z + 8 * NB * 16);
+  p.own_mu = st[4 * R * g + (c < 4 * R ? c : 0)];
+  p.own_rho = st[16 * R + 4 * R * g + (c < 4 * R ? c : 0)];
+}
 template <int EPI, int MB, int NB, int M_LO = 0, int M_HI = MB, bool PRE = false>
 __device__ __forceinline__ void store_wave_tile16(floatx4 (&acc)[MB][NB], int wr0, int wc0, int M, int N,
                                                   const float* __restrict__ bias, const float* __restrict__ resid,
@@ -438,17 +520,113 @@
 
 constexpr int kAttnSt = 36;
 constexpr int kAttnStage = 64 * kAttnSt * 4;
-template <bool FOLD, bool PRE = false>
+struct AttnPre {
+  unsigned long long kbits = 0;
+  float own_mu = 0.f, own_rho = 0.f;
+  float bv[6], sv[6];
+};
+template <bool FOLD>
+__device__ __forceinline__ void attn_pre_load(AttnPre& p, int wr0, int head, int wn, int M, int H,
+                                              const float* __restrict__ bias, const LnFold& lf,
+                                              const int* __restrict__ mask, int lane) {
+  p.kbits = __ballot(mask[min(wr0 + lane, M - 1)] != 0);
+  if constexpr (FOLD) ln_row_own<4>(lf.stats_in, wr0, M, lf.eps, lane, p.own_mu, p.own_rho);
+#pragma unroll
+  for (int n = 0; n < 6; ++n) {
+    const int col = (n >> 1) * H + 64 * head + 32 * wn + 16 * (n & 1) + (lane & 15);
+    p.bv[n] = bias[col];
+    p.sv[n] = FOLD ? lf.s[col] : 0.f;
+  }
+}
+constexpr int kAttnPreBytes = 1296;
+struct AttnPreRaw {
+  float mw;
+  float bv[6], sv[6];
+  floatx4 p[kLnMaxParts / 2];
+};
+template <bool FOLD>
+__device__ __forceinline__ void attn_pre_issue(AttnPreRaw& q, int wr0, int head, int wn, int M, int H,
+                                               const float* __restrict__ bias, const LnFold& lf,
+                                               const int* __restrict__ mask, int lane) {
+  q.mw = pre_ld(reinterpret_cast<const float*>(mask + min(wr0 + lane, M - 1)));
+  if constexpr (FOLD) {
+    static_assert(kLnMaxParts == 8, "four 16-byte loads per row");
+    const int c = lane & 15;
+    const int row = min(wr0 + 16 * (c >> 2) + 4 * (lane >> 4) + (c & 3), M - 1);
+    const float* src = lf.stats_in + (int64_t)row * (2 * kLnMaxParts);
+    asm volatile(
+        "global_load_dwordx4 %0, %4, off\n\tglobal_load_dwordx4 %1, %4, off offset:16\n\t"
+        "global_load_dwordx4 %2, %4, off offset:32\n\tglobal_load_dwordx4 %3, %4, off offset:48"
+        : "=&v"(q.p[0]), "=&v"(q.p[1]), "=&v"(q.p[2]), "=&v"(q.p[3])
+        : "v"(src)
+        : "memory");
+  }
+#pragma unroll
+  for (int n = 0; n < 6; ++n) {
+    const int col = (n >> 1) * H + 64 * head + 32 * wn + 16 * (n & 1) + (lane & 15);
+    q.bv[n] = pre_ld(bias + col);
+    q.sv[n] = FOLD ? pre_ld(lf.s + col) : 0.f;
+  }
+}
+template <bool FOLD, int BEHIND>
+__device__ __forceinline__ void attn_pre_wait(AttnPreRaw& q, AttnPre& p, float eps) {
+  asm volatile("s_waitcnt vmcnt(%13)"
+               : "+v"(q.bv[0]), "+v"(q.bv[1]), "+v"(q.bv[2]), "+v"(q.bv[3]), "+v"(q.bv[4]), "+v"(q.bv[5]),
+                 "+v"(q.sv[0]), "+v"(q.sv[1]), "+v"(q.sv[2]), "+v"(q.sv[3]), "+v"(q.sv[4]), "+v"(q.sv[5]), "+v"(q.mw)
+               : "n"(BEHIND)
+               : "memory");
+  p.kbits = __ballot(__float_as_int(q.mw) != 0);
+#pragma unroll
+  for (int n = 0; n < 6; ++n) {
+    p.bv[n] = q.bv[n];
+    p.sv[n] = q.sv[n];
+  }
+  if constexpr (FOLD) {
+    asm volatile("" : "+v"(q.p[0]), "+v"(q.p[1]), "+v"(q.p[2]), "+v"(q.p[3])::"memory");
+    ln_merge(q.p, eps, p.own_mu, p.own_rho);
+  }
+}
+__device__ __forceinline__ void attn_pre_lds_write(const AttnPre& p, unsigned char* z, int lane) {
+  if (lane < 16) {
+    floatx4* d = reinterpret_cast<floatx4*>(z + lane * 48);
+    d[0] = floatx4{p.bv[0], p.bv[1], p.bv[2], p.bv[3]};
+    d[1] = floatx4{p.bv[4], p.bv[5], p.sv[0], p.sv[1]};
+    d[2] = floatx4{p.sv[2], p.sv[3], p.sv[4], p.sv[5]};
+  }
+  reinterpret_cast<float*>(z + 768)[lane] = p.own_mu;
+  reinterpret_cast<float*>(z + 1024)[lane] = p.own_rho;
+  if (lane == 0) *reinterpret_cast<unsigned long long*>(z + 1280) = p.kbits;
+}
+__device__ __forceinline__ void attn_pre_lds_read(AttnPre& p, const unsigned char* z, int lane) {
+  const floatx4* d = reinterpret_cast<const floatx4*>(z + (lane & 15) * 48);
+  const floatx4 d0 = d[0], d1 = d[1], d2 = d[2];
+  p.bv[0] = d0.x, p.bv[1] = d0.y, p.bv[2] = d0.z, p.bv[3] = d0.w, p.bv[4] = d1.x, p.bv[5] = d1.y;
+  p.sv[0] = d1.z, p.sv[1] = d1.w, p.sv[2] = d2.x, p.sv[3] = d2.y, p.sv[4] = d2.z, p.sv[5] = d2.w;
+  p.own_mu = reinterpret_cast<const float*>(z + 768)[lane];
+  p.own_rho = reinterpret_cast<const float*>(z + 1024)[lane];
+  const uint2 kb = *reinterpret_cast<const uint2*>(z + 1280);
+  p.kbits = ((unsigned long long)(unsigned)__builtin_amdgcn_readfirstlane((int)kb.y) << 32) |
+            (unsigned)__builtin_amdgcn_readfirstlane((int)kb.x);
+}
+template <bool FOLD, bool PRE = false, bool STAGED = false>
 __device__ __forceinline__ void attn_wave_tile(floatx4 (&acc)[4][6], int wr0, int head, int wn, int M, int H,
                                                const float* __restrict__ bias, const LnFold& lf,
                                                const int* __restrict__ mask, float scale,
                                                float* __restrict__ ctx, int lane, unsigned char* stg,
-                                               const unsigned char* partner) {
+                                               const unsigned char* partner, const AttnPre* ap = nullptr) {
   static_assert(kAttnStage >= 8 * 1024, "the partials of two sequences fit the staging");
+  static_assert(!(PRE && STAGED), "staged preloads: the epilogue form");
   const int c = lane & 15, g = lane >> 4;
-  const unsigned long long kbits = __ballot(mask[min(wr0 + lane, M - 1)] != 0);
+  unsigned long long kbits;
   float own_mu = 0.f, own_rho = 0.f;
-  if constexpr (FOLD) ln_row_own<4>(lf.stats_in, wr0, M, lf.eps, lane, own_mu, own_rho);
+  if constexpr (STAGED) {
+    kbits = ap->kbits;
+    own_mu = ap->own_mu;
+    own_rho = ap->own_rho;
+  } else {
+    kbits = __ballot(mask[min(wr0 + lane, M - 1)] != 0);
+    if constexpr (FOLD) ln_row_own<4>(lf.stats_in, wr0, M, lf.eps, lane, own_mu, own_rho);
+  }
   if constexpr (PRE) {
 #pragma unroll
     for (int m = 0; m < 4; ++m)
@@ -460,6 +638,11 @@
     float bv[6], sv[6];
 #pragma unroll
     for (int n = 0; n < 6; ++n) {
+      if constexpr (STAGED) {
+        bv[n] = ap->bv[n];
+        sv[n] = ap->sv[n];
+        continue;
+      }
       const int col = (n >> 1) * H + 64 * head + 32 * wn + 16 * (n & 1) + c;
       bv[n] = bias[col];
       if constexpr (FOLD) sv[n] = lf.s[col];
diff --git a/mediquery-rag_amd/csrc/gemm_x6p.hip b/mediquery-rag_amd/csrc/gemm_x6p.hip
--- a/mediquery-rag_amd/csrc/gemm_x6p.hip
+++ b/mediquery-rag_amd/csrc/gemm_x6p.hip
@@ -45,6 +45,31 @@
 
 #if defined(MQ_X6P_DBG) && !defined(MQ_MEASUREMENT_BUILD)
 #error "MQ_X6P_DBG computes wrong results: only a measurement build (-DMQ_MEASUREMENT_BUILD) may set it"
+#endif
+
+#if defined(MQ_EPI_STAMPS) && !defined(MQ_MEASUREMENT_BUILD)
+#error "MQ_EPI_STAMPS fences the epilogues: only a measurement build (-DMQ_MEASUREMENT_BUILD) may set it"
+#endif
+#ifdef MQ_EPI_STAMPS
+constexpr int kStampWgs = 1024, kStampVals = 8;
+__device__ unsigned long long mq_epi_stamp_buf[kStampWgs][kStampVals];
+#define MQ_EPI_STAMP(i) (stamp_t[i] = __builtin_amdgcn_s_memtime())
+template <int NB>
+__device__ __forceinline__ void epi_pre_fence(EpiPre<NB>& p) {
+  static_assert(NB == 6, "the operand list below");
+  asm volatile("s_waitcnt vmcnt(0) lgkmcnt(0)"
+               : "+v"(p.bv[0]), "+v"(p.bv[1]), "+v"(p.bv[2]), "+v"(p.bv[3]), "+v"(p.bv[4]), "+v"(p.bv[5]),
+                 "+v"(p.sv[0]), "+v"(p.sv[1]), "+v"(p.sv[2]), "+v"(p.sv[3]), "+v"(p.sv[4]), "+v"(p.sv[5]),
+                 "+v"(p.own_mu), "+v"(p.own_rho)::"memory");
+}
+__device__ __forceinline__ void attn_pre_fence(AttnPre& p) {
+  asm volatile("s_waitcnt vmcnt(0) lgkmcnt(0)"
+               : "+v"(p.bv[0]), "+v"(p.bv[1]), "+v"(p.bv[2]), "+v"(p.bv[3]), "+v"(p.bv[4]), "+v"(p.bv[5]),
+                 "+v"(p.sv[0]), "+v"(p.sv[1]), "+v"(p.sv[2]), "+v"(p.sv[3]), "+v"(p.sv[4]), "+v"(p.sv[5]),
+                 "+v"(p.own_mu), "+v"(p.own_rho), "+s"(p.kbits)::"memory");
+}
+#else
+#define MQ_EPI_STAMP(i) ((void)0)
 #endif
 
 template <int WAVES_M_, int WAVES_N_, int TM_, int TN_, int NBUF_, int KS_ = 1, int DMAW_ = 8, bool SCHED_ = false,
@@ -92,7 +117,7 @@
          (MQ_X6P_SPLIT_BIAS != 0 && (epi == EPI_BIAS || epi == EPI_BIAS_LNFOLD));
 }
 
-template <class T, int EPI, bool FORMER = false>
+template <class T, int EPI, int FORM = 0>
 __global__ __launch_bounds__(T::THREADS, 1) void gemm_x6p_kernel(const float* __restrict__ A, int lda,
                                                              const unsigned char* __restrict__ W3,
                                                              const float* __restrict__ bias,
@@ -101,6 +126,7 @@
                                                              int K, int rx, LnFold lf, AttnEpi at) {
   __shared__ __attribute__((aligned(1024))) unsigned char lds[T::NBUF * T::STAGE];
   const unsigned lds0 = (unsigned)(uintptr_t)(x6p_lds_t*)lds;
+  constexpr bool FORMER = FORM == 1;
   constexpr bool HAND = EPI == EPI_RESID_LN_STATS && T::LDR && T::M16 && !T::DEEP && T::NBUF == 3 && !FORMER;
   constexpr bool ATTN = epi_is_attn(EPI);
   static_assert(!ATTN || (T::LDR && T::M16 && !T::DEEP && T::NBUF == 3 && T::WAVES_M == 2 && T::WAVES_N == 2 &&
@@ -113,6 +139,20 @@
                          T::TN == 3;
   static_assert(!SPLIT || ((HS == 1 || HS == 2) && 4 * HS * 2 * T::TN * 1024 <= T::STAGE),
                 "split epilogue: the handed blocks of the four compute waves fit one ring slot");
+  constexpr int PRE_B = epi_pre_lds_bytes<2 * T::TN, 2 * T::TM - HS>();
+  constexpr int PRE_OFF = 4 * HS * 2 * T::TN * 1024;
+  constexpr bool PREFETCH = SPLIT && FORM == 0 && T::DBG == 0 && T::REM == 0 && T::AHEAD == 2 && T::TN == 3 &&
+                            PRE_OFF + 4 * PRE_B <= T::STAGE;
+  static_assert(!PREFETCH || (PRE_OFF % 16 == 0 && PRE_B % 16 == 0), "16-byte pieces");
+#ifndef MQ_X6P_APRE_K1
+#define MQ_X6P_APRE_K1 6
+#endif
+  constexpr int APRE_K1 = MQ_X6P_APRE_K1;
+  constexpr int APRE_OFF = 4 * kAttnStage;
+  constexpr bool APREFETCH = ATTN && FORM == 0 && T::DBG == 0 && T::REM == 0 && T::AHEAD == 2 &&
+                             APRE_OFF + 4 * kAttnPreBytes <= T::STAGE;
+  static_assert(!APREFETCH || (APRE_OFF % 16 == 0 && kAttnPreBytes % 16 == 0), "16-byte pieces");
+  static_assert(!APREFETCH || (APRE_K1 >= 0 && APRE_K1 <= T::CNT_LO), "DMAs in front of P(j)");
   const int lane = threadIdx.x & 63;
   const int wave = __builtin_amdgcn_readfirstlane(threadIdx.x >> 6);
   const int cw = T::LDR ? wave % T::NW : wave;
@@ -374,8 +414,49 @@
       }
       int l_st = 0;
       [[maybe_unused]] int l_i = 0;
+      [[maybe_unused]] EpiPreRaw<2 * T::TN> praw;
+      [[maybe_unused]] int p_wr0 = 0, p_wc0 = 0;
+      [[maybe_unused]] bool l_landed = false;
       for (int j = 0; j < S; ++j) {
-        wait_stages(IC<T::AHEAD - 2>{});
+        if (PREFETCH && l_landed) {
+          l_landed = false;
+          __builtin_amdgcn_s_waitcnt(0xC07F);
+          asm volatile("s_barrier" ::: "memory");
+        } else {
+          wait_stages(IC<T::AHEAD - 2>{});
+        }
+        if constexpr (PREFETCH) {
+          if (l_st + 1 == nst) {
+            int m0, n0;
+            coords(l_i, m0, n0);
+            p_wr0 = m0 + wm * T::WM;
+            p_wc0 = n0 + wn * T::WN;
+            epi_pre_issue<EPI, 2 * T::TM, 2 * T::TN>(praw, p_wr0, p_wc0, M, N, bias, lf, lane);
+          }
+        }
+        if constexpr (APREFETCH) {
+          if (l_st + 1 == nst) {
+            l_st = 0;
+            int m0, n0;
+            coords(l_i++, m0, n0);
+            AttnPreRaw araw;
+            attn_pre_issue<EPI == EPI_ATTN_LNFOLD>(araw, m0 + wm * T::WM, n0 / T::BN, wn, M, N / 3, bias, lf, at.mask,
+                                                   lane);
+            const int ibuf = (j + T::AHEAD) % T::NBUF;
+#pragma unroll
+            for (int t = 0; t < APRE_K1; ++t) issue_one(ibuf, t);
+            AttnPre ap;
+            attn_pre_wait<EPI == EPI_ATTN_LNFOLD, APRE_K1>(araw, ap, lf.eps);
+            attn_pre_lds_write(ap, lds + (j % T::NBUF) * T::STAGE + APRE_OFF + cw * kAttnPreBytes, lane);
+            __builtin_amdgcn_s_waitcnt(0xC07F);
+            asm volatile("s_barrier" ::: "memory");
+            asm volatile("s_barrier" ::: "memory");
+#pragma unroll
+            for (int t = APRE_K1; t < T::CNT_HI; ++t) issue_one(ibuf, t);
+            advance();
+            continue;
+          }
+        }
         issue((j + T::AHEAD) % T::NBUF);
         if constexpr (ATTN) {
           if (++l_st == nst) {
@@ -392,7 +473,13 @@
             coords(l_i++, m0, n0);
             const int wr0 = m0 + wm * T::WM, wc0 = n0 + wn * T::WN;
             EpiPre<NB16> pre;
-            epi_pre_load<EPI, MB, NB16>(pre, wr0, wc0, M, N, bias, lf, lane);
+            if constexpr (PREFETCH) {
+              epi_pre_wait<EPI, NB16, T::CNT_LO>(praw, pre, lf.eps);
+              epi_pre_lds_write<NB16, MB - HS>(pre, lds + (j % T::NBUF) * T::STAGE + PRE_OFF + cw * PRE_B, lane);
+              __builtin_amdgcn_s_waitcnt(0xC07F);
+            } else {
+              epi_pre_load<EPI, MB, NB16>(pre, wr0, wc0, M, N, bias, lf, lane);
+            }
             asm volatile("s_barrier" ::: "memory");
             const unsigned char* hs = lds + (j % T::NBUF) * T::STAGE + cw * (HS * NB16 * 1024) + lane * 16;
             floatx4 hacc[MB][NB16];
@@ -401,6 +488,10 @@
 #pragma unroll
               for (int n = 0; n < NB16; ++n)
                 hacc[MB - HS + m][n] = *reinterpret_cast<const floatx4*>(hs + (m * NB16 + n) * 1024);
+            if constexpr (PREFETCH) {
+              asm volatile("s_waitcnt vmcnt(0)" ::: "memory");
+              l_landed = true;
+            }
             store_wave_tile16<EPI, MB, NB16, MB - HS, MB, true>(hacc, wr0, wc0, M, N, bias, resid, ldr, out, ldo, lane,
                                                                 lf, &pre);
           }
@@ -474,6 +565,11 @@
         for (int p = 0; p < 3; ++p) rd_b(st, n, p);
     };
     load_ops(lds);
+#ifdef MQ_EPI_STAMPS
+    unsigned long long stamp_t[5] = {}, stamp_s[6] = {};
+    bool stamp_open = false;
+    const unsigned long long stamp_k0 = __builtin_amdgcn_s_memtime(), stamp_r0 = __builtin_amdgcn_s_memrealtime();
+#endif
     int rb = 1 % T::NBUF;
     int ib = T::AHEAD % T::NBUF;
     for (int j = 0; j < S; ++j) {
@@ -487,6 +583,13 @@
         asm volatile("s_barrier" ::: "memory");
       }
       const unsigned char* st = lds + rb * T::STAGE;
+#ifdef MQ_EPI_STAMPS
+      if (stamp_open) {
+        stamp_open = false;
+        stamp_s[4] += __builtin_amdgcn_s_memtime() - stamp_t[3];
+        ++stamp_s[5];
+      }
+#endif
       static_for<NM16>([&](auto ic) {
         constexpr int i = decltype(ic)::value;
         constexpr int m = i / RS, w = i % RS, n = w / 6, term = w % 6;
@@ -514,11 +617,37 @@
         c_st = 0;
         int m0, n0;
         coords(c_i, m0, n0);
+        MQ_EPI_STAMP(0);
         if constexpr (ATTN) {
           unsigned char* fs = lds + (j % T::NBUF) * T::STAGE;
-          attn_wave_tile<EPI == EPI_ATTN_LNFOLD>(acc4, m0 + wm * T::WM, n0 / T::BN, wn, M, N / 3, bias, lf, at.mask,
-                                                 at.scale, out, lane, fs + cw * kAttnStage,
-                                                 fs + (cw ^ 1) * kAttnStage);
+#ifdef MQ_EPI_STAMPS
+          if constexpr (APREFETCH) asm volatile("s_barrier" ::: "memory");
+          MQ_EPI_STAMP(1);
+          AttnPre ap;
+          if constexpr (APREFETCH)
+            attn_pre_lds_read(ap, fs + APRE_OFF + cw * kAttnPreBytes, lane);
+          else
+            attn_pre_load<EPI == EPI_ATTN_LNFOLD>(ap, m0 + wm * T::WM, n0 / T::BN, wn, M, N / 3, bias, lf, at.mask,
+                                                  lane);
+          attn_pre_fence(ap);
+          MQ_EPI_STAMP(2);
+          attn_wave_tile<EPI == EPI_ATTN_LNFOLD, false, true>(acc4, m0 + wm * T::WM, n0 / T::BN, wn, M, N / 3, bias, lf,
+                                                              at.mask, at.scale, out, lane, fs + cw * kAttnStage,
+                                                              fs + (cw ^ 1) * kAttnStage, &ap);
+#else
+          if constexpr (APREFETCH) {
+            asm volatile("s_barrier" ::: "memory");
+            AttnPre ap;
+            attn_pre_lds_read(ap, fs + APRE_OFF + cw * kAttnPreBytes, lane);
+            attn_wave_tile<EPI == EPI_ATTN_LNFOLD, false, true>(acc4, m0 + wm * T::WM, n0 / T::BN, wn, M, N / 3, bias,
+                                                                lf, at.mask, at.scale, out, lane,
+                                                                fs + cw * kAttnStage, fs + (cw ^ 1) * kAttnStage, &ap);
+          } else {
+            attn_wave_tile<EPI == EPI_ATTN_LNFOLD>(acc4, m0 + wm * T::WM, n0 / T::BN, wn, M, N / 3, bias, lf, at.mask,
+                                                   at.scale, out, lane, fs + cw * kAttnStage,
+                                                   fs + (cw ^ 1) * kAttnStage);
+          }
+#endif
           load_ops(st);
         } else if constexpr (SPLIT) {
           unsigned char* hs = lds + (j % T::NBUF) * T::STAGE + cw * (HS * NB16 * 1024) + lane * 16;
@@ -529,16 +658,52 @@
               *reinterpret_cast<floatx4*>(hs + (m * NB16 + n) * 1024) = acc4[MB - HS + m][n];
           __builtin_amdgcn_s_waitcnt(0xC07F);
           asm volatile("s_barrier" ::: "memory");
-          store_wave_tile16<EPI, MB, NB16, 0, MB - HS>(acc4, m0 + wm * T::WM, n0 + wn * T::WN, M, N, bias, resid, ldr,
-                                                       out, ldo, lane, lf);
+          MQ_EPI_STAMP(1);
+          if constexpr (PREFETCH) {
+            EpiPre<NB16> pre;
+            epi_pre_lds_read<NB16, MB - HS>(pre, lds + (j % T::NBUF) * T::STAGE + PRE_OFF + cw * PRE_B, lane);
+#ifdef MQ_EPI_STAMPS
+            epi_pre_fence(pre);
+            MQ_EPI_STAMP(2);
+#endif
+            store_wave_tile16<EPI, MB, NB16, 0, MB - HS, true>(acc4, m0 + wm * T::WM, n0 + wn * T::WN, M, N, bias,
+                                                               resid, ldr, out, ldo, lane, lf, &pre);
+          } else {
+#ifdef MQ_EPI_STAMPS
+            EpiPre<NB16> pre;
+            epi_pre_load<EPI, MB, NB16>(pre, m0 + wm * T::WM, n0 + wn * T::WN, M, N, bias, lf, lane);
+            epi_pre_fence(pre);
+            MQ_EPI_STAMP(2);
+            store_wave_tile16<EPI, MB, NB16, 0, MB - HS, true>(acc4, m0 + wm * T::WM, n0 + wn * T::WN, M, N, bias,
+                                                               resid, ldr, out, ldo, lane, lf, &pre);
+#else
+            store_wave_tile16<EPI, MB, NB16, 0, MB - HS>(acc4, m0 + wm * T::WM, n0 + wn * T::WN, M, N, bias, resid,
+                                                         ldr, out, ldo, lane, lf);
+#endif
+          }
         } else {
           store_wave_tile16<EPI, MB, NB16>(acc4, m0 + wm * T::WM, n0 + wn * T::WN, M, N, bias, resid, ldr, out, ldo,
                                            lane, lf);
         }
+#ifdef MQ_EPI_STAMPS
+        if constexpr (ATTN || SPLIT) {
+          MQ_EPI_STAMP(3);
+          ++stamp_s[0];
+          for (int i = 1; i < 4; ++i) stamp_s[i] += stamp_t[i] - stamp_t[i - 1];
+          stamp_open = true;
+        }
+#endif
         zero4();
         ++c_i;
       }
     }
+#ifdef MQ_EPI_STAMPS
+    if (wave == 0 && lane == 0 && blockIdx.x < kStampWgs) {
+      for (int i = 0; i < 6; ++i) mq_epi_stamp_buf[blockIdx.x][i] = stamp_s[i];
+      mq_epi_stamp_buf[blockIdx.x][6] = __builtin_amdgcn_s_memtime() - stamp_k0;
+      mq_epi_stamp_buf[blockIdx.x][7] = __builtin_amdgcn_s_memrealtime() - stamp_r0;
+    }
+#endif
     if constexpr (HAND) {
       asm volatile("s_barrier" ::: "memory");
       int m0, n0;
@@ -675,7 +840,7 @@
 using X6p16 = X6pTile<2, 2, 2, 3, 4, 1, 4, true, 0, 1, 0, 6, true>;
 using X6p17 = X6pTile<2, 2, 1, 3, 4, 1, 4, true, 0, 1, 0, 6, true>;
 
-template <class T, int EPI, bool FORMER = false>
+template <class T, int EPI, int FORM = 0>
 void launch_t(const X6pArgs& g, int num_cus, hipStream_t s) {
   if constexpr (EPI < EPI_RESID_LN_STATS) {
     if (g.K % (16 * T::KS) != 0) {
@@ -690,7 +855,7 @@
   int rx = g.rx;
   if (rx < 0) rx = region_pick_rx(tiles_m, tiles_n, (double)T::BM * g.K * 4, (double)T::BN * g.K * 6, grid);
   if (rx > 0 && (8 % rx != 0 || rx > tiles_n || 8 / rx > tiles_m || grid < 8)) rx = 0;
-  hipLaunchKernelGGL((gemm_x6p_kernel<T, EPI, FORMER>), dim3(grid), dim3(T::THREADS), 0, s, g.A, g.lda,
+  hipLaunchKernelGGL((gemm_x6p_kernel<T, EPI, FORM>), dim3(grid), dim3(T::THREADS), 0, s, g.A, g.lda,
                      static_cast<const unsigned char*>(g.W3), g.bias, g.resid, g.ldr, g.out, g.ldo, g.M, g.N, g.K, rx,
                      g.lf, g.at);
 }
@@ -721,8 +886,9 @@
     case 7: launch_t<X6p7, EPI>(g, num_cus, s); return;
     case 16: launch_t<X6p16, EPI>(g, num_cus, s); return;
     case 17: launch_t<X6p17, EPI>(g, num_cus, s); return;
-    case 20: launch_t<X6p0, EPI, epi_is_split(EPI)>(g, num_cus, s); return;
-    case 21: launch_t<X6p1, EPI, epi_is_split(EPI)>(g, num_cus, s); return;
+    case 20: launch_t<X6p0, EPI, epi_is_split(EPI) ? 1 : 0>(g, num_cus, s); return;
+    case 21: launch_t<X6p1, EPI, epi_is_split(EPI) ? 1 : 0>(g, num_cus, s); return;
+    case 22: launch_t<X6p0, EPI, epi_is_split(EPI) ? 2 : 0>(g, num_cus, s); return;
     default: launch_t<X6p0, EPI>(g, num_cus, s); return;
   }
 }
@@ -732,8 +898,9 @@
   constexpr bool HAS_FORMER = EPI == EPI_RESID_LN_STATS || epi_is_split(EPI);
   switch (tile) {
     case 1: launch_t<X6p1, EPI>(g, num_cus, s); return;
-    case 20: launch_t<X6p0, EPI, HAS_FORMER>(g, num_cus, s); return;
-    case 21: launch_t<X6p1, EPI, HAS_FORMER>(g, num_cus, s); return;
+    case 20: launch_t<X6p0, EPI, HAS_FORMER ? 1 : 0>(g, num_cus, s); return;
+    case 21: launch_t<X6p1, EPI, HAS_FORMER ? 1 : 0>(g, num_cus, s); return;
+    case 22: launch_t<X6p0, EPI, epi_is_split(EPI) ? 2 : 0>(g, num_cus, s); return;
     default: launch_t<X6p0, EPI>(g, num_cus, s); return;
   }
 }
@@ -798,6 +965,7 @@
     tile = x6p_pick_tile(g.M, g.N, num_cus);
   }
   if (g.former_epi && epi_is_split(epi) && (tile == 0 || tile == 1)) tile += 20;
+  if (g.no_prefetch && epi_is_split(epi) && tile == 0) tile = 22;
   switch (epi) {
     case EPI_GELU_ERF: launch_tile<EPI_GELU_ERF>(g, tile, num_cus, s); return;
     case EPI_GELU_TANH: launch_tile<EPI_GELU_TANH>(g, tile, num_cus, s); return;
@@ -806,8 +974,18 @@
     case EPI_BIAS_LNFOLD: launch_tile_fold<EPI_BIAS_LNFOLD>(g, tile, num_cus, s); return;
     case EPI_GELU_ERF_LNFOLD: launch_tile_fold<EPI_GELU_ERF_LNFOLD>(g, tile, num_cus, s); return;
     case EPI_GELU_TANH_LNFOLD: launch_tile_fold<EPI_GELU_TANH_LNFOLD>(g, tile, num_cus, s); return;
-    case EPI_ATTN_BIAS: launch_t<X6p0, EPI_ATTN_BIAS>(g, num_cus, s); return;
-    case EPI_ATTN_LNFOLD: launch_t<X6p0, EPI_ATTN_LNFOLD>(g, num_cus, s); return;
+    case EPI_ATTN_BIAS:
+      if (g.no_prefetch)
+        launch_t<X6p0, EPI_ATTN_BIAS, 2>(g, num_cus, s);
+      else
+        launch_t<X6p0, EPI_ATTN_BIAS>(g, num_cus, s);
+      return;
+    case EPI_ATTN_LNFOLD:
+      if (g.no_prefetch)
+        launch_t<X6p0, EPI_ATTN_LNFOLD, 2>(g, num_cus, s);
+      else
+        launch_t<X6p0, EPI_ATTN_LNFOLD>(g, num_cus, s);
+      return;
     default: launch_tile<EPI_BIAS>(g, tile, num_cus, s); return;
   }
 }
@@ -836,7 +1014,7 @@
   MQ_CHECK_ARG(M > 0 && N > 0 && K > 0 && K % 32 == 0, "bad shape M=%d N=%d K=%d", M, N, K);
   const int rx = tile >= 100 ? tile / 100 - 1 : -1;
   if (tile >= 100) tile %= 100;
-  MQ_CHECK_ARG(epi >= 0 && epi <= 3 && tile >= -1 && (tile <= 17 || tile == 20 || tile == 21) && rx <= 8,
+  MQ_CHECK_ARG(epi >= 0 && epi <= 3 && tile >= -1 && (tile <= 17 || (tile >= 20 && tile <= 22)) && rx <= 8,
                "bad epi/tile");
   int dev = 0, cus = 256;
   (void)hipGetDevice(&dev);
@@ -866,8 +1044,10 @@
   clear_error();
   MQ_CHECK_ARG(A && W3 && bias && out, "NULL buffer");
   MQ_CHECK_ARG(M > 0 && N > 0 && K > 0 && K % 32 == 0, "bad shape M=%d N=%d K=%d", M, N, K);
-  MQ_CHECK_ARG((tile >= -1 && tile <= 1) || tile == 20 || tile == 21,
-               "the LayerNorm-fold epilogues run on tiles 0 and 1 (20 / 21: their former epilogues; got %d)", tile);
+  MQ_CHECK_ARG((tile >= -1 && tile <= 1) || (tile >= 20 && tile <= 22),
+               "the LayerNorm-fold epilogues run on tiles 0 and 1 (20 / 21: their former epilogues, 22: tile 0 "
+               "without the prefetch; got %d)",
+               tile);
   if (epi == EPI_RESID_LN_STATS) {
     MQ_CHECK_ARG(resid && stats_out && (!stats_in || (g && b)), "producer: NULL buffer");
     MQ_CHECK_ARG(N == kLnPartW * kLnMaxParts, "producer: N must be %d (got %d)", kLnPartW * kLnMaxParts, N);
@@ -891,11 +1071,31 @@
   return MQ_OK;
 }
 
+#ifdef MQ_EPI_STAMPS
+int mq_debug_epi_stamps(unsigned long long* dst, int workgroups) {
+  using namespace mq;
+  clear_error();
+  MQ_CHECK_ARG(dst && workgroups > 0 && workgroups <= kStampWgs, "bad arguments");
+  MQ_HIP(hipDeviceSynchronize());
+  MQ_HIP(hipMemcpyFromSymbol(dst, HIP_SYMBOL(mq_epi_stamp_buf), (size_t)workgroups * kStampVals * 8, 0,
+                             hipMemcpyDeviceToHost));
+  return MQ_OK;
+}
+#endif
+
 int mq_debug_gemm_x6p_attn(const float* A, const void* W3, const float* bias, const int* mask, float* ctx, int M,
                            int K, int heads, float scale, int epi, const float* stats_in, const float* s_fold,
                            float eps, int max_workgroups, void* stream) {
+  return mq_debug_gemm_x6p_attn_v(A, W3, bias, mask, ctx, M, K, heads, scale, epi, stats_in, s_fold, eps,
+                                  max_workgroups, 0, stream);
+}
+
+int mq_debug_gemm_x6p_attn_v(const float* A, const void* W3, const float* bias, const int* mask, float* ctx, int M,
+                             int K, int heads, float scale, int epi, const float* stats_in, const float* s_fold,
+                             float eps, int max_workgroups, int prefetch, void* stream) {
   using namespace mq;
   clear_error();
+  MQ_CHECK_ARG(prefetch == 0 || prefetch == 1, "prefetch must be 0 or 1 (got %d)", prefetch);
   MQ_CHECK_ARG(A && W3 && bias && mask && ctx, "NULL buffer");
   MQ_CHECK_ARG(M > 0 && M % 32 == 0 && K > 0 && K % 32 == 0 && heads > 0 && heads <= 1024,
                "bad shape M=%d K=%d heads=%d (M and K must be multiples of 32)", M, K, heads);
@@ -915,6 +1115,7 @@
   a.at.mask = mask;
   a.at.scale = scale;
   a.max_wg = max_workgroups;
+  a.no_prefetch = prefetch == 0;
   launch_gemm_x6p(a, epi, 0, cus, (hipStream_t)stream);
   MQ_HIP(hipGetLastError());
   return MQ_OK;
diff --git a/mediquery-rag_amd/csrc/gemm_x6p.hpp b/mediquery-rag_amd/csrc/gemm_x6p.hpp
--- a/mediquery-rag_amd/csrc/gemm_x6p.hpp
+++ b/mediquery-rag_amd/csrc/gemm_x6p.hpp
@@ -79,6 +79,7 @@
   AttnEpi at{};
   int max_wg = 0;
   bool former_epi = false;
+  bool no_prefetch = false;
 };
 
 void launch_attn32(const float* qkv, const int* mask, float* ctx, int M, int H, float scale, hipStream_t s);
diff --git a/mediquery-rag_amd/mediquery_hip/_lib.py b/mediquery-rag_amd/mediquery_hip/_lib.py
--- a/mediquery-rag_amd/mediquery_hip/_lib.py
+++ b/mediquery-rag_amd/mediquery_hip/_lib.py
@@ -30,6 +30,7 @@
 MQ_ENC_OPT_CLS_KFREE = 12
 MQ_ENC_OPT_QKV_ATTN = 13
 MQ_ENC_OPT_EPI_SPLIT = 14
+MQ_ENC_OPT_EPI_PREFETCH = 15
 MQ_ROWS_QKV, MQ_ROWS_UP, MQ_ROWS_OPROJ, MQ_ROWS_DOWN = 0, 1, 2, 3
 
 
@@ -130,6 +131,8 @@
     "mq_debug_gemm_x6p_ln": (_I, [_P, _P, _P, _P, _P, _I, _I, _I, _I, _I, _P, _P, _P, _P, _P, ctypes.c_float, _P]),
     "mq_debug_ln_fold_weight": (_I, [_P, _P, _P, _P, _I, _I, _P, _P, _P, _P]),
     "mq_debug_gemm_x6p_attn": (_I, [_P, _P, _P, _P, _P, _I, _I, _I, ctypes.c_float, _I, _P, _P, ctypes.c_float, _I, _P]),
+    "mq_debug_gemm_x6p_attn_v": (_I, [_P, _P, _P, _P, _P, _I, _I, _I, ctypes.c_float, _I, _P, _P, ctypes.c_float, _I, _I,
+                                      _P]),
     "mq_debug_attention": (_I, [_P, _P, _I, _I, _I, _I, ctypes.c_float, _I, _P, _P]),
     "mq_debug_cls_attention": (_I, [_P, _P, _P, _P, _P, ctypes.c_float, _P, _I, _I, _I, _I, ctypes.c_float, _P, _P, _P,
                                     _P, _P]),
diff --git a/mediquery-rag_amd/mediquery_hip/native.py b/mediquery-rag_amd/mediquery_hip/native.py
--- a/mediquery-rag_amd/mediquery_hip/native.py
+++ b/mediquery-rag_amd/mediquery_hip/native.py
@@ -260,7 +260,7 @@
                "resident_layers": _lib.MQ_ENC_OPT_RESIDENT_LAYERS, "x6_presplit": _lib.MQ_ENC_OPT_X6_PRESPLIT,
                "rows_planes": _lib.MQ_ENC_OPT_ROWS_PLANES, "ln_fold": _lib.MQ_ENC_OPT_LN_FOLD,
                "cls_kfree": _lib.MQ_ENC_OPT_CLS_KFREE, "qkv_attn": _lib.MQ_ENC_OPT_QKV_ATTN,
-               "epi_split": _lib.MQ_ENC_OPT_EPI_SPLIT}
+               "epi_split": _lib.MQ_ENC_OPT_EPI_SPLIT, "epi_prefetch": _lib.MQ_ENC_OPT_EPI_PREFETCH}
 
     def set_option(self, name, value):
         _lib.call("mq_encoder_set_option", self._h, self.OPTIONS[name], int(value))
```
